# lmb-freiburg/understanding_flow_robustness

Hardware: AMD Instinct MI355X
Metric: attack-iters/s (higher is better)
Workload: dtype f32

## Files before the change

include/ufr_hip.h:

```cpp
#ifndef UFR_HIP_H_
#define UFR_HIP_H_

#include <stdint.h>

#ifdef __cplusplus
extern "C" {
#endif

#define UFR_ABI_VERSION 9

enum { UFR_F32 = 0, UFR_F64 = 1, UFR_F16 = 2 };
enum {
  UFR_OK = 0,
  UFR_EINVAL = -1,
  UFR_EUNSUPPORTED = -2,
  UFR_ELAUNCH = -3
};

typedef void* ufr_stream_t;

int ufr_abi_version(void);
const char* ufr_last_error(void);
int ufr_device_count(void);
const char* ufr_build_manifest(void);
// ... 277 lines not shown
int ufr_resample_u8_vertical(const unsigned char* src, unsigned char* dst, int Hs, int Hd, int W, int C,
                             const int* bounds, const int* kk, int ksize, ufr_stream_t stream);
int ufr_u8_to_tensor(const unsigned char* src, float* dst, int H, int W, int C, int crop_y, int crop_x, int crop_h,
                     int crop_w, float divisor, ufr_stream_t stream);
int ufr_kitti_flow_decode(const unsigned short* src, float* dst, int H, int W, ufr_stream_t stream);

int ufr_host_png_unfilter(const unsigned char* data, unsigned char* out, int rows, int stride, int bpp);

#define UFR_IGEMM_MAX_TAPS 25
typedef struct {
  int ntaps, oy0, ox0;
  long w_off;
  signed char dy[UFR_IGEMM_MAX_TAPS], dx[UFR_IGEMM_MAX_TAPS];
} ufr_igemm_phase;
typedef struct {
  const void* x; long x_plane_stride; int in_chunk0, KC;
  int B, Hi, Wi, in_sy, in_sx;
  const int* in_x0; int in_x0_stride, in_x0_div, in_xw;
  const void* w; long w_plane_stride; int Npad, N;
  int Hr, Wr;
  const int* row_x0; int row_x0_stride, row_x0_div;
  int Ho, Wo, out_sy, out_sx;
  int nphase;
  ufr_igemm_phase phase[4];
  int act; const float* bias; float slope;
  const float* add; int add_chunk0;
  const void* mask; int mask_chunk0;
  void* out_planes; long out_plane_stride; int out_chunk0;
  float* out_f32; int out_f32_chunk0;
  float* tail; int tail_n0, tail_accumulate;
  int splitk; float* ws;
  int products;
  int variant;
  int k_order;
  float* out_rowmajor; long out_ld;
  int planes_chunks, f32_first_chunk;
  int no_reduce;
  int* tickets;
} ufr_igemm_desc;
int ufr_igemm(const ufr_igemm_desc* d, ufr_stream_t stream);
typedef struct {
  int on;
  int row_tiles, col_tiles;
  int full_row_tiles, tail_row_tiles;
  int tail_row0, tail_rows;
  int slices, slice_ktiles, ktiles;
  int workgroups;
  long ws_floats;
  int steps_before, steps_after;
} ufr_igemm_tail_plan_t;
int ufr_igemm_tail_plan(const ufr_igemm_desc* d, int resident_workgroups, ufr_igemm_tail_plan_t* plan);
int ufr_igemm_balanced(const ufr_igemm_desc* d, int resident_workgroups, float* ws, long ws_floats, ufr_stream_t stream);
typedef struct {
  const void* x; long x_plane_stride; int in_chunk0, C;
  const void* gy; long gy_plane_stride; int g_chunk0, N;
  int B, Hi, Wi, Ho, Wo, kh, kw, sy, sx, py, px;
  float* dw;
  float* db;
  int accumulate;
  int splitm; float* ws; long ws_elems;
  int products;
} ufr_igemm_wgrad_desc;
int ufr_igemm_wgrad(const ufr_igemm_wgrad_desc* d, ufr_stream_t stream);
int ufr_igemm_wgrad_dilated(const ufr_igemm_wgrad_desc* d, int dy, int dx, ufr_stream_t stream);
int ufr_igemm_variant_fallbacks(void);
int ufr_igemm_clock_probe(unsigned long long* buf, int capacity_workgroups);
int ufr_rowmajor_to_planes(const float* src, long ld, long rows, int cols, float scale, void* planes, long plane_stride, int chunk0,
                           long plane_rows, ufr_stream_t stream);
int ufr_nchw_to_planes(const float* x, void* planes, long plane_stride, int chunk0, int B, int C, int H, int W,
                       float scale, float slope, const float* bias, ufr_stream_t stream);
int ufr_window_scatter_planes(const float* src, void* planes, long plane_stride, int chunk0, const int* win, int n_win,
                              int N, int C, int Hd, int Wd, int wh, int ww, int level_stride, int margin,
                              ufr_stream_t stream);
int ufr_window_features_planes(const void* c2w, long c2w_stride, const void* c3w, long c3w_stride, void* cat2, long cat2_stride,
                               void* c3a, long c3a_stride, void* c3b, long c3b_stride, float* c3_nchw, float* c3w_nchw,
                               const int* win, int B, int H, int W, int wh, int ww, int m2, int m3, ufr_stream_t stream);
int ufr_chunks_to_nchw(const void* planes, long plane_stride, const float* f32, int chunk0, const void* mask,
                       int mask_chunk0, float* out, int B, int C, int H, int W, float scale, float slope,
                       ufr_stream_t stream);
int ufr_nchw_cat_to_planes(const float* const* srcs, const int* channels, const int* dst_channel0, int nseg, void* planes,
                           long plane_stride, int chunk0, int chunks, int B, int H, int W, ufr_stream_t stream);
int ufr_chunks_to_nchw_cat(const float* g, int chunk0, int chunks, float* const* dsts, const int* channels, const int* src_channel0,
                           int nseg, const float* act0, float pos0, float neg0, int B, int H, int W, ufr_stream_t stream);
int ufr_grad_finalize(const float* g, int g_chunk0, const void* mask, int mask_chunk0, void* out, long out_plane_stride,
                      int out_chunk0, long M, int chunks, float slope, ufr_stream_t stream);

int ufr_conv1_direct(const float* frames_a, const float* frames_b, int Ba, int Bb, int H, int W, const double* mean,
                     const void* wimg, const float* bias, float slope, void* out_planes, long plane_stride, int out_chunk0,
                     ufr_stream_t stream);
int ufr_conv1_pack_planes(const float* frames_a, const float* frames_b, void* planes, long plane_stride, int Ba, int Bb, int H,
                          int W, const double* mean, ufr_stream_t stream);
int ufr_conv1_unpack_grad(const float* G, float* grad_frames, int N, int H, int W, ufr_stream_t stream);
int ufr_unshuffle_pack_planes(const float* x, void* planes, long plane_stride, int N, int C, int H, int W, ufr_stream_t stream);
int ufr_unshuffle_unpack_grad(const float* G, float* grad_x, int N, int C, int H, int W, ufr_stream_t stream);
int ufr_nchw_grad_to_planes(const float* grad, const float* act, void* planes, long plane_stride, int chunk0, int B, int C, int H,
                            int W, float slope, ufr_stream_t stream);
int ufr_window_gather_chunks(const float* src, float* dst, const int* win, int n_win, int N, int N_dst, int chunks, int Hs, int Ws,
                             int wh, int ww, int level_stride, int margin, ufr_stream_t stream);

int ufr_normalize_frames(const float* frames_a, const float* frames_b, float* out, int Ba, int Bb, int C, int H, int W,
                         const double* mean, ufr_stream_t stream);

int ufr_corr_forward_planes_window(const void* f1_planes, const void* f2_planes, long in_plane_stride, void* out_planes,
                                   long out_plane_stride, int out_chunk0, int B, int C, int H, int W, int patch,
                                   int dilation_patch, float scale, float slope, const int* win, int level_stride,
                                   int win_cells, ufr_stream_t stream);

int ufr_corr_forward_planes_changed(const void* f1_planes, const void* f2_planes, long in_plane_stride, void* out_planes,
                                    long out_plane_stride, int out_chunk0, int B, int C, int H, int W, int patch,
                                    int dilation_patch, float scale, float slope, const int* win, int level_stride,
                                    int win_cells_h, int win_cells_w, int margin, ufr_stream_t stream);

int ufr_corr_backward_window_fused(const float* f1, const float* f2, const float* G, int g_chunk0, float g_scale,
                                   const float* G_redir, float* grad_window, int B, int C, int H, int W, int patch,
                                   int dilation_patch, const int* win, int level_stride, int wh, int ww, int margin,
                                   ufr_stream_t stream);

int ufr_corr_forward_planes(const void* f1_planes, const void* f2_planes, long in_plane_stride, void* out_planes,
                            long out_plane_stride, int out_chunk0, int B, int C, int H, int W, int patch,
                            int dilation_patch, float scale, float slope, ufr_stream_t stream);
int ufr_flow_head_planes_forward(const void* planes, long plane_stride, int chunk0, int chunks, const float* wpk, int w_chunks,
                                 const float* bias, float* out, int B, int H, int W, ufr_stream_t stream);
int ufr_flow_head_planes_forward_mfma(const void* planes, long plane_stride, int chunk0, int chunks, const void* wmf, int w_chunks,
                                      const float* bias, float* out, int B, int H, int W, ufr_stream_t stream);
int ufr_flow_head_split_plan(int B, int H, int W, int chunks, int* slices, int* starved, long* partial_floats);
int ufr_flow_head_planes_forward_split(const void* planes, long plane_stride, int chunk0, int chunks, const void* wmf, int w_chunks,
                                       float* partials, long partial_floats, int slices, int B, int H, int W, ufr_stream_t stream);
int ufr_flow_head_split_finish(const float* partials, long partial_floats, int slices, const float* bias, float* flow,
                               const float* up_w, const float* up_bias, void* up_planes, long up_plane_stride, int up_chunk, int B,
                               int H, int W, ufr_stream_t stream);
int ufr_deconv_flow_tail_backward_mfma(const void* grad_planes, long plane_stride, int chunk0, int chunks, const void* wmf,
                                       int w_chunks, float* G, int g_chunks, int out_chunk, int B, int H, int W, ufr_stream_t stream);
int ufr_flow_head_planes_backward(const float* grad_y, const float* wpk, int w_chunks, float* G, int g_chunks, int chunk0, int chunks,
                                  int B, int H, int W, int accumulate, ufr_stream_t stream);
int ufr_flow_head_planes_backward_finalize(const float* grad_y, const float* wpk, int w_chunks, float* G, int g_chunks, int chunk0,
                                           int chunks, int B, int H, int W, int accumulate, const void* mask_planes, void* out_planes,
                                           long out_plane_stride, int fin_chunk0, int fin_chunks, float slope, ufr_stream_t stream);
#define UFR_PF_REGION_BAND 1
#define UFR_PF_REGION_WINDOW 2
int ufr_flow_head_planes_backward_regions(const float* grad_y, const float* wpk, int w_chunks, float* G, int g_chunks, int chunk0,
                                          int chunks, int B, int H, int W, int accumulate, int head_chunks, int region,
                                          const int* origin, int origin_stride, int origin_div, int reg_h, int reg_w, int margin,
// ... 134 lines not shown
```

understanding_flow_robustness_amd/_lib.py:

```python
from __future__ import annotations

import ctypes as C
import os

import torch

_HERE = os.path.dirname(os.path.abspath(__file__))
LIB_PATH = os.environ.get("UFR_HIP_LIB") or os.path.join(_HERE, "lib", "libufr_hip.so")
UFR_F32, UFR_F64, UFR_F16 = 0, 1, 2
ABI_VERSION = 9
_lib = None


class CorrParams(C.Structure):
    _fields_ = [(n, C.c_int) for n in (
        "kH", "kW", "patchH", "patchW", "padH", "padW", "dilationH", "dilationW",
        "dilation_patchH", "dilation_patchW", "dH", "dW")]


UFR_MAX_LEVELS = 8


class Pyramid(C.Structure):
    _fields_ = [("num_levels", C.c_int),
                ("vol", C.c_void_p * UFR_MAX_LEVELS),
                ("grad_vol", C.c_void_p * UFR_MAX_LEVELS),
                ("Hl", C.c_int * UFR_MAX_LEVELS),
                ("Wl", C.c_int * UFR_MAX_LEVELS)]


class AltCorrLevels(C.Structure):
    _fields_ = [("num_levels", C.c_int), ("fmap2", C.c_void_p * 4), ("fmap2_grad", C.c_void_p * 4),
                ("H2", C.c_int * 4), ("W2", C.c_int * 4), ("coord_scale", C.c_float * 4)]


class AltCorrPlaneLevels(C.Structure):
    _fields_ = [("num_levels", C.c_int), ("planes", C.c_void_p * 4), ("plane_stride", C.c_long * 4),
                ("H2", C.c_int * 4), ("W2", C.c_int * 4), ("coord_scale", C.c_float * 4)]


UFR_IGEMM_MAX_TAPS = 25


class IgemmPhase(C.Structure):
    _fields_ = [("ntaps", C.c_int), ("oy0", C.c_int), ("ox0", C.c_int), ("w_off", C.c_long),
                ("dy", C.c_byte * UFR_IGEMM_MAX_TAPS), ("dx", C.c_byte * UFR_IGEMM_MAX_TAPS)]


class IgemmDesc(C.Structure):
    _fields_ = [("x", C.c_void_p), ("x_plane_stride", C.c_long), ("in_chunk0", C.c_int), ("KC", C.c_int),
                ("B", C.c_int), ("Hi", C.c_int), ("Wi", C.c_int), ("in_sy", C.c_int), ("in_sx", C.c_int),
                ("in_x0", C.c_void_p), ("in_x0_stride", C.c_int), ("in_x0_div", C.c_int), ("in_xw", C.c_int),
                ("w", C.c_void_p), ("w_plane_stride", C.c_long), ("Npad", C.c_int), ("N", C.c_int),
                ("Hr", C.c_int), ("Wr", C.c_int),
                ("row_x0", C.c_void_p), ("row_x0_stride", C.c_int), ("row_x0_div", C.c_int),
                ("Ho", C.c_int), ("Wo", C.c_int), ("out_sy", C.c_int), ("out_sx", C.c_int),
                ("nphase", C.c_int),
                ("phase", IgemmPhase * 4),
                ("act", C.c_int), ("bias", C.c_void_p), ("slope", C.c_float),
                ("add", C.c_void_p), ("add_chunk0", C.c_int),
                ("mask", C.c_void_p), ("mask_chunk0", C.c_int),
                ("out_planes", C.c_void_p), ("out_plane_stride", C.c_long), ("out_chunk0", C.c_int),
                ("out_f32", C.c_void_p), ("out_f32_chunk0", C.c_int),
                ("tail", C.c_void_p), ("tail_n0", C.c_int), ("tail_accumulate", C.c_int),
                ("splitk", C.c_int), ("ws", C.c_void_p),
                ("products", C.c_int), ("variant", C.c_int), ("k_order", C.c_int),
                ("out_rowmajor", C.c_void_p), ("out_ld", C.c_long),
                ("planes_chunks", C.c_int), ("f32_first_chunk", C.c_int), ("no_reduce", C.c_int),
                ("tickets", C.c_void_p)]


class IgemmTailPlan(C.Structure):
    _fields_ = [("on", C.c_int), ("row_tiles", C.c_int), ("col_tiles", C.c_int), ("full_row_tiles", C.c_int), ("tail_row_tiles", C.c_int),
                ("tail_row0", C.c_int), ("tail_rows", C.c_int), ("slices", C.c_int), ("slice_ktiles", C.c_int), ("ktiles", C.c_int),
                ("workgroups", C.c_int), ("ws_floats", C.c_long), ("steps_before", C.c_int), ("steps_after", C.c_int)]


UFR_IGEMM_WGRAD_MAX_TAPS = 49


class IgemmWgradDesc(C.Structure):
    _fields_ = [("x", C.c_void_p), ("x_plane_stride", C.c_long), ("in_chunk0", C.c_int), ("C", C.c_int),
                ("gy", C.c_void_p), ("gy_plane_stride", C.c_long), ("g_chunk0", C.c_int), ("N", C.c_int),
                ("B", C.c_int), ("Hi", C.c_int), ("Wi", C.c_int), ("Ho", C.c_int), ("Wo", C.c_int),
                ("kh", C.c_int), ("kw", C.c_int), ("sy", C.c_int), ("sx", C.c_int), ("py", C.c_int), ("px", C.c_int),
                ("dw", C.c_void_p), ("db", C.c_void_p), ("accumulate", C.c_int),
                ("splitm", C.c_int), ("ws", C.c_void_p), ("ws_elems", C.c_long),
                ("products", C.c_int)]


UFR_TRAIN_LOSS_MAX_SCALES = 8


class TrainLossDesc(C.Structure):
    _fields_ = [("gt", C.c_void_p), ("B", C.c_int), ("H", C.c_int), ("W", C.c_int), ("nscale", C.c_int),
                ("pred", C.c_void_p * UFR_TRAIN_LOSS_MAX_SCALES), ("grad", C.c_void_p * UFR_TRAIN_LOSS_MAX_SCALES),
                ("h", C.c_int * UFR_TRAIN_LOSS_MAX_SCALES), ("w", C.c_int * UFR_TRAIN_LOSS_MAX_SCALES),
                ("weight", C.c_double * UFR_TRAIN_LOSS_MAX_SCALES),
                ("kind", C.c_int), ("div_flow", C.c_double),
                ("ws", C.c_void_p), ("ws_elems", C.c_long), ("out", C.c_void_p)]


UFR_RAFT_LOSS_MAX_PREDS = 32


class RaftSequenceLossDesc(C.Structure):
    _fields_ = [("gt", C.c_void_p), ("valid", C.c_void_p), ("B", C.c_int), ("H", C.c_int), ("W", C.c_int), ("npred", C.c_int),
                ("flow", C.c_void_p * UFR_RAFT_LOSS_MAX_PREDS), ("mask", C.c_void_p * UFR_RAFT_LOSS_MAX_PREDS),
                ("grad_flow", C.c_void_p * UFR_RAFT_LOSS_MAX_PREDS), ("grad_mask", C.c_void_p * UFR_RAFT_LOSS_MAX_PREDS),
                ("weight", C.c_double * UFR_RAFT_LOSS_MAX_PREDS),
                ("div_flow", C.c_double), ("max_flow", C.c_double), ("exclude_large", C.c_int),
                ("ws", C.c_void_p), ("ws_elems", C.c_long), ("out", C.c_void_p)]


class AdamwSeg(C.Structure):
    _fields_ = [("p", C.c_void_p), ("g", C.c_void_p), ("m", C.c_void_p), ("v", C.c_void_p), ("n", C.c_long)]


class AdamwHyper(C.Structure):
    _fields_ = [(n, C.c_double) for n in ("lr", "beta1", "beta2", "eps", "weight_decay", "bias1", "bias2")]


class FeatureStatsSeg(C.Structure):
    _fields_ = [("src", C.c_void_p), ("plane_stride", C.c_long), ("pixels", C.c_long), ("kind", C.c_int), ("images", C.c_int),
                ("image0", C.c_int), ("B", C.c_int), ("chunk0", C.c_int), ("channels", C.c_int), ("unleaky", C.c_double),
                ("out_col", C.c_long)]


# ... 29 lines not shown
    "ufr_patch_update": [_vp, _vp, _vp, _vp, _vp, _vp, _vp, _vp, _i, _i, _l, _l, _f, _f, _f, _f, _vp, _vp],
    "ufr_attack_gate": [_vp, _vp, _f, _vp],
    "ufr_gru_gates_forward": [_vp, _vp, _vp, _vp, _i, _i, _i, _l, _vp],
    "ufr_gru_gates_backward": [_vp, _vp, _vp, _vp, _vp, _vp, _i, _i, _i, _l, _vp],
    "ufr_gru_blend_forward": [_vp, _vp, _vp, _vp, _l, _vp],
    "ufr_gru_blend_backward": [_vp, _vp, _vp, _vp, _vp, _vp, _vp, _l, _vp],
    "ufr_flow_loss_ex": [_vp, _vp, _vp, _vp, _i, _i, _i, _i, _f, _vp, _vp, _vp],
    "ufr_universal_update": [_vp, _vp, _vp, _vp, _vp, _vp, _vp, _vp, _i, _i, _f, _f, _f, _f, _i, _i, _i, _i,
                             _i, _vp],
    "ufr_flow_loss": [_vp, _vp, _vp, _vp, _i, _i, _i, _f, _vp, _vp],
    "ufr_flow2_upsampled_loss": [_vp, _f, _vp, _vp, _vp, _i, _i, _i, _i, _f, _vp, _vp],
    "ufr_flow2_upsampled_loss_fast": [_vp, _f, _vp, _vp, _vp, _i, _i, _i, _i, _f, _vp, _vp],
    "ufr_patch_grad_crop": [_vp, _vp, _vp, _vp, _vp, _vp, _vp, _i, _i, _i, _i, _i, _i, _vp],
    "ufr_patch_apply": [_vp, _i, _vp, _vp, _i, _i, _f, _f, _vp, _vp],
    "ufr_patch_grad_crop_window": [_vp, _vp, _vp, _vp, _vp, _vp, _i, _i, _i, _i, _i, _i, _i, _i, _vp],
    "ufr_patch_paste_placed_rect": [_vp, _vp, _vp, _vp, _vp, _vp, _vp, _i, _i, _i, _i, _i, _i, _f, _f, _vp, _vp],
    "ufr_patch_paste_placed": [_vp, _vp, _vp, _vp, _vp, _vp, _vp, _vp, _vp, _i, _i, _i, _i, _i, _i, _f, _f, _vp, _vp],
    "ufr_cone_window": [_vp, _i, _l, _i, _i, _i, C.POINTER(ConeChain), _i, _i, _vp, _vp, _vp],
    "ufr_attack_place": [_vp, _vp, _vp, _vp, _vp, _vp, _vp, _vp, _vp, _vp, _vp, _i, _i, _i, _i, _i, C.POINTER(ConeChain), _i, _i,
                         _vp, _vp, _i, _i, _i, _i, _vp],
    "ufr_attack_load_frames": [_vp, _vp, _vp, _vp, _vp, _vp, _vp, _vp, _vp, _i, _i, _i, _i, _i, _vp],
    "ufr_patch_mask_placed": [_vp, _vp, _vp, _i, _i, _i, _i, _i, _vp],
    "ufr_patch_grad_crop_packed": [_vp, _vp, _vp, _vp, _vp, _vp, _i, _i, _i, _i, _i, _i, _i, _i, _vp],
    "ufr_patch_apply_paste_rect": [_vp, _i, _vp, _vp, _vp, _vp, _vp, _vp, _vp, _vp, _i, _i, _i, _i, _i, _f, _f, _i, _f, _f, _vp, _vp],
    "ufr_window_gather_pair": [_vp, _vp, _vp, _vp, _vp, _i, _i, _i, _i, _i, _i, _vp],
    "ufr_window_features_planes": [_vp, _l, _vp, _l, _vp, _l, _vp, _l, _vp, _l, _vp, _vp, _vp, _i, _i, _i, _i, _i, _i, _i, _vp],
    "ufr_window_gather": [_vp, _vp, _vp, _i, _i, _i, _i, _i, _i, _i, _i, _i, _vp],
    "ufr_window_scatter": [_vp, _vp, _vp, _i, _i, _i, _i, _i, _i, _i, _i, _i, _vp],
    "ufr_conv1_pack_planes": [_vp, _vp, _vp, _l, _i, _i, _i, _i, _vp, _vp],
    "ufr_conv1_unpack_grad": [_vp, _vp, _i, _i, _i, _vp],
    "ufr_nchw_grad_to_planes": [_vp, _vp, _vp, _l, _i, _i, _i, _i, _i, _f, _vp],
    "ufr_window_gather_chunks": [_vp, _vp, _vp, _i, _i, _i, _i, _i, _i, _i, _i, _i, _i, _vp],
    "ufr_normalize_frames": [_vp, _vp, _vp, _i, _i, _i, _i, _i, _vp, _vp],
    "ufr_corr_backward_window_fused": [_vp, _vp, _vp, _i, _f, _vp, _vp, _i, _i, _i, _i, _i, _i, _vp, _i, _i, _i, _i, _vp],
    "ufr_corr_backward_window": [_vp, _vp, _vp, _vp, _vp, _i, _i, _i, _i, _i, _i, _vp, _i, _i, _i, _vp],
    "ufr_bias_leaky_forward": [_vp, _vp, _i, _i, _l, _f, _vp],
    "ufr_leaky_backward": [_vp, _vp, _vp, _l, _f, _vp],
    "ufr_conv3x3_c2_forward": [_vp, _vp, _vp, _vp, _vp, _i, _i, _i, _i, _vp],
    "ufr_conv3x3_c2_backward_data": [_vp, _vp, _vp, _i, _i, _i, _i, _vp],
    "ufr_deconv4x4s2_c2_forward": [_vp, _vp, _vp, _vp, _i, _i, _i, _vp],
    "ufr_deconv4x4s2_c2_backward_data": [_vp, _vp, _vp, _i, _i, _i, _vp],
    "ufr_pwc_warp_forward": [_vp, _vp, _vp, _i, _i, _i, _i, _vp],
    "ufr_pwc_warp_backward": [_vp, _vp, _vp, _vp, _vp, _i, _i, _i, _i, _vp],
    "ufr_pwc_warp_backward_owner": [_vp, _vp, _vp, _vp, _vp, _vp, _l, _i, _i, _i, _i, _vp],
    "ufr_raft_normalize_pair": [_vp, _vp, _vp, _l, _vp],
    "ufr_raft_normalize_pair_backward": [_vp, _vp, _vp, _l, _vp],
    "ufr_raft_fmap_pyramid_forward": [_vp, _vp, _i, _i, _i, _i, _i, _vp],
    "ufr_raft_fmap_pyramid_backward": [_vp, _i, _vp, _i, _i, _i, _i, _vp],
    "ufr_raft_context_split_forward": [_vp, _vp, _vp, _i, _i, _i, _l, _vp],
    "ufr_raft_context_split_backward": [_vp, _vp, _vp, _vp, _vp, _i, _i, _i, _l, _vp],
    "ufr_igemm": [C.POINTER(IgemmDesc), _vp],
    "ufr_igemm_tail_plan": [C.POINTER(IgemmDesc), _i, C.POINTER(IgemmTailPlan)],
    "ufr_igemm_balanced": [C.POINTER(IgemmDesc), _i, _vp, _l, _vp],
    "ufr_igemm_wgrad": [C.POINTER(IgemmWgradDesc), _vp],
    "ufr_igemm_wgrad_dilated": [C.POINTER(IgemmWgradDesc), _i, _i, _vp],
    "ufr_flow_upscale4_forward": [_vp, _vp, _i, _i, _i, _i, _f, _i, _vp],
    "ufr_flow_upscale4_backward": [_vp, _vp, _i, _i, _i, _i, _f, _i, _vp],
    "ufr_fn2_stage_pack": [_vp, _vp, _vp, _vp, _i, _i, _i, _f, _vp],
    "ufr_fn2_stage_unpack_grad": [_vp, _vp, _vp, _vp, _i, _i, _i, _vp],
    "ufr_fn2_stage_finish_grad": [_vp, _vp, _vp, _vp, _vp, _i, _i, _i, _f, _vp],
    "ufr_fn2_fusion_pack": [_vp, _vp, _vp, _vp, _vp, _vp, _i, _i, _i, _vp],
    "ufr_fn2_fusion_unpack_grad": [_vp, _vp, _vp, _vp, _vp, _vp, _vp, _vp, _vp, _i, _i, _i, _vp],
    "ufr_fn2_fusion_finish_grad": [_vp, _vp, _vp, _vp, _vp, _vp, _vp, _i, _i, _i, _vp],
    "ufr_rowmajor_to_planes": [_vp, _l, _l, _i, _f, _vp, _l, _i, _l, _vp],
    "ufr_nchw_to_planes": [_vp, _vp, _l, _i, _i, _i, _i, _i, _f, _f, _vp, _vp],
    "ufr_window_scatter_planes": [_vp, _vp, _l, _i, _vp, _i, _i, _i, _i, _i, _i, _i, _i, _i, _vp],
    "ufr_chunks_to_nchw": [_vp, _l, _vp, _i, _vp, _i, _vp, _i, _i, _i, _i, _f, _f, _vp],
    "ufr_nchw_cat_to_planes": [_vp, _vp, _vp, _i, _vp, _l, _i, _i, _i, _i, _i, _vp],
    "ufr_chunks_to_nchw_cat": [_vp, _i, _i, _vp, _vp, _vp, _i, _vp, _f, _f, _i, _i, _i, _vp],
    "ufr_grad_finalize": [_vp, _i, _vp, _i, _vp, _l, _i, _l, _i, _f, _vp],
    "ufr_flow_head_planes_forward": [_vp, _l, _i, _i, _vp, _i, _vp, _vp, _i, _i, _i, _vp],
    "ufr_flow_head_planes_forward_mfma": [_vp, _l, _i, _i, _vp, _i, _vp, _vp, _i, _i, _i, _vp],
    "ufr_deconv_flow_tail_backward_mfma": [_vp, _l, _i, _i, _vp, _i, _vp, _i, _i, _i, _i, _i, _vp],
    "ufr_flow_head_planes_backward": [_vp, _vp, _i, _vp, _i, _i, _i, _i, _i, _i, _i, _vp],
    "ufr_flow_head_planes_backward_finalize": [_vp, _vp, _i, _vp, _i, _i, _i, _i, _i, _i, _i, _vp, _vp, _l, _i, _i, _f, _vp],
    "ufr_flow_head_planes_backward_regions": [_vp, _vp, _i, _vp, _i, _i, _i, _i, _i, _i, _i, _i, _i, _vp, _i, _i, _i, _i, _i, _vp, _i,
                                              _vp, _vp, _l, _i, _i, _f, _vp],
    "ufr_unshuffle_pack_planes": [_vp, _vp, _l, _i, _i, _i, _i, _vp],
    "ufr_unshuffle_unpack_grad": [_vp, _vp, _i, _i, _i, _i, _vp],
    "ufr_conv3x3s2_c3_planes": [_vp, _vp, _vp, _f, _vp, _l, _i, _i, _i, _i, _i, _vp],
    "ufr_conv3x3_c16_planes": [_vp, _l, _i, _vp, _vp, _f, _vp, _l, _i, _i, _i, _i, _vp],
    "ufr_cm_norm_stats": [_vp, _vp, _vp, _l, _i, _i, _f, _vp],
    "ufr_cm_norm_apply": [_vp, _vp, _vp, _l, _i, _vp, _l, _i, _l, _i, _i, _i, _i, _vp],
    "ufr_cm_norm_stats_apply": [_vp, _vp, _vp, _f, _vp, _l, _i, _vp, _l, _i, _l, _i, _i, _i, _i, _vp],
    "ufr_cm_norm_backward": [_vp, _vp, _vp, _i, _vp, _vp, _vp, _vp, _l, _i, _l, _i, _i, _i, _vp],
    "ufr_cm_masked_copy": [_vp, _vp, _l, _vp, _l, _vp],
    "ufr_raft_flow_patches": [_vp, _vp, _l, _i, _i, _i, _i, _vp],
    "ufr_raft_motion_finish_slabs": [_vp, _i, _i, _i, _vp, _f, _vp, _l, _vp, _l, _i, _vp, _i, _i, _i, _vp],
    "ufr_raft_motion_finish": [_vp, _l, _vp, _l, _i, _vp, _i, _i, _i, _vp],
    "ufr_raft_coords_step": [_vp, _vp, _vp, _vp, _vp, _l, _vp],
    "ufr_grad_finalize_consume": [_vp, _vp, _vp, _l, _l, _i, _f, _vp],
    "ufr_gru_gates_cm_forward": [_vp, _vp, _l, _i, _vp, _l, _i, _l, _i, _vp],
    "ufr_gru_gates_cm_forward_slabs": [_vp, _i, _i, _vp, _vp, _vp, _vp, _l, _i, _vp, _l, _i, _l, _i, _vp],
    "ufr_gru_blend_cm_forward_slabs": [_vp, _i, _i, _vp, _vp, _vp, _vp, _vp, _l, _i, _vp, _l, _i, _l, _i, _vp],
    "ufr_gru_blend_cm_forward": [_vp, _vp, _vp, _l, _i, _vp, _l, _i, _l, _i, _vp],
    "ufr_gru_blend_cm_backward": [_vp, _vp, _vp, _l, _i, _vp, _vp, _l, _i, _vp, _vp, _l, _i, _vp, _vp],
    "ufr_gru_gates_cm_backward": [_vp, _vp, _l, _i, _vp, _vp, _vp, _l, _i, _vp, _l, _i, _i, _vp, _vp],
    "ufr_altcorr_pyramid_forward": [_vp, _vp, _vp, _vp, _i, _i, _i, _i, _i, _f, _vp],
    "ufr_altcorr_pyramid_backward": [_vp, _vp, _vp, _vp, _vp, _vp, _i, _i, _i, _i, _i, _f, _i, _vp],
    "ufr_altcorr_pyramid_backward_cm": [_vp, _vp, _vp, _vp, _vp, _vp, _i, _i, _i, _i, _i, _f, _i, _vp],
    "ufr_upfeat_planes_forward_mfma": [_vp, _l, _i, _i, _vp, _i, _vp, _vp, _i, _i, _i, _vp],
    "ufr_upfeat_planes_backward": [_vp, _vp, _i, _vp, _i, _i, _i, _i, _i, _i, _i, _vp],
    "ufr_flow_up_planes_forward": [_vp, _vp, _vp, _vp, _l, _i, _i, _i, _i, _vp],
    "ufr_flow_head_split_plan": [_i, _i, _i, _i, C.POINTER(C.c_int), C.POINTER(C.c_int), C.POINTER(C.c_long)],
    "ufr_flow_head_planes_forward_split": [_vp, _l, _i, _i, _vp, _i, _vp, _l, _i, _i, _i, _i, _vp],
    "ufr_flow_head_split_finish": [_vp, _l, _i, _vp, _vp, _vp, _vp, _vp, _l, _i, _i, _i, _i, _vp],
    "ufr_flow_up_planes_backward": [_vp, _i, _vp, _vp, _i, _i, _i, _i, _vp],
    "ufr_corr_forward_planes_changed": [_vp, _vp, _l, _vp, _l, _i, _i, _i, _i, _i, _i, _i, _f, _f, _vp, _i, _i, _i, _i, _vp],
    "ufr_corr_forward_planes_window": [_vp, _vp, _l, _vp, _l, _i, _i, _i, _i, _i, _i, _i, _f, _f, _vp, _i, _i, _vp],
    "ufr_corr_forward_planes": [_vp, _vp, _l, _vp, _l, _i, _i, _i, _i, _i, _i, _i, _f, _f, _vp],
    "ufr_convex_upsample_forward": [_vp, _vp, _vp, _i, _i, _i, _vp],
    "ufr_convex_upsample_backward": [_vp, _vp, _vp, _vp, _vp, _vp, _i, _i, _i, _vp],
    "ufr_affine_resample_f64": [_vp, _vp, _i, _i, _i, _i, _i, _d, _d, _d, _d, _d, _d, _i, _vp],
    "ufr_patch_place": [_vp, _vp, _vp, _i, _i, _i, _vp, _vp, _vp, _i, _i, _i, _i, _vp],
    "ufr_patch_crop_f64": [_vp, _vp, _vp, _i, _i, _i, _i, _i, _i, _i, _vp],
    "ufr_resample_u8_horizontal": [_vp, _vp, _i, _i, _i, _i, _i, _vp, _vp, _i, _vp],
    "ufr_resample_u8_vertical": [_vp, _vp, _i, _i, _i, _i, _vp, _vp, _i, _vp],
    "ufr_u8_to_tensor": [_vp, _vp, _i, _i, _i, _i, _i, _i, _i, _f, _vp],
    "ufr_kitti_flow_decode": [_vp, _vp, _i, _i, _vp],
    "ufr_host_png_unfilter": [_vp, _vp, _i, _i, _i],
    "ufr_igemm_clock_probe": [_vp, _i],
    "ufr_altcorr_planes_prepare": [_vp, _vp, _l, _l, _i, _vp],
    "ufr_altcorr_planes_forward": [_vp, _l, C.POINTER(AltCorrPlaneLevels), _vp, _vp, _i, _i, _i, _i, _i, _f, _vp],
    "ufr_conv1_direct": [_vp, _vp, _i, _i, _i, _i, _vp, _vp, _vp, _f, _vp, _l, _i, _vp],
    "ufr_train_loss": [C.POINTER(TrainLossDesc), _vp],
    "ufr_raft_sequence_loss": [C.POINTER(RaftSequenceLossDesc), _vp],
    "ufr_grad_norm": [C.POINTER(AdamwSeg), _i, _f, _vp, _l, _vp, _vp],
    "ufr_adamw_step": [C.POINTER(AdamwSeg), _i, C.POINTER(AdamwHyper), _vp, _vp],
    "ufr_sweep_paste": [_vp, _vp, _vp, _vp, _vp, _vp, _vp, _vp, _i, _i, _i, _i, _i, _f, _f, C.POINTER(ConeChain), _i, _i, _vp, _vp, _vp],
    "ufr_sweep_metrics": [_vp, _vp, _vp, _vp, _vp, _i, _i, _i, _i, _i, _i, _i, _i, _vp, _l, _vp, _i, _i, _vp],
    "ufr_eval_paste": [_vp, _vp, _vp, _vp, _vp, _vp, _vp, _vp, _vp, _vp, _i, _i, _i, _i, _i, _f, _f, _vp],
    "ufr_eval_metrics": [_vp, _vp, _vp, _vp, _vp, _vp, _vp, _vp, _i, _i, _i, _i, _i, _i, _i, _i, _vp, _l, _vp, _i, _i, _vp],
    "ufr_flow_to_image": [_vp, _vp, _vp, _vp, _i, _i, _i, _vp, _l, _vp],
    "ufr_eval_blend_gt": [_vp, _vp, _vp, _vp, _vp, _vp, _vp, _i, _i, _i, _i, _i, _i, _i, _i, _vp],
    "ufr_sweep_blend_gt": [_vp, _vp, _vp, _vp, _vp, _i, _i, _i, _i, _i, _i, _i, _i, _vp],
    "ufr_viz_ranges": [_vp, _vp, _vp, _vp, _vp, _i, _i, _i, _i, _i, _vp, _l, _vp, _vp],
    "ufr_viz_strip": [_vp, _vp, _vp, _vp, _vp, _vp, _vp, _vp, _i, _i, _i, _i, _i, _vp],
    "ufr_global_apply": [_vp, _vp, _vp, _vp, _vp, _vp, _i, _i, _i, _i, _f, _f, _vp],
    "ufr_global_metrics": [_vp, _vp, _vp, _vp, _vp, _i, _i, _i, _i, _i, _i, _i, _i, _vp, _l, _vp, _i, _i, _vp],
    "ufr_validation_pad": [_vp, _vp, _vp, _vp, _i, _i, _i, _i, _i, _i, _i, _i, _vp],
    "ufr_validation_metrics": [_vp, _vp, _vp, _i, _i, _i, _i, _i, _i, _i, _i, _vp, _l, _vp, _i, _i, _vp],
    "ufr_forward_interpolate": [_vp, _vp, _i, _i, _i, _vp],
    "ufr_forward_interpolate_sliced": [_vp, _vp, _i, _i, _i, _i, _vp],
    "ufr_flow_encode": [_vp, _vp, _i, _i, _i, _i, _i, _i, _i, _i, _vp],
    "ufr_feature_stats": [C.POINTER(FeatureStatsSeg), _i, _vp, _l, _vp, _i, _l, _l, _vp],
    "ufr_abs_sums": [_vp, _vp, _l, _vp, _l, _vp, _vp],
    "ufr_momentum_update": [_vp, _vp, _vp, _vp, _vp, _vp, _vp, _vp, _vp, _vp, _i, _i, _f, _f, _f, _f, _f, _f, _i, _i, _vp],
    "ufr_diverse_table_check": [_vp, _i, _i, _i],
    "ufr_diverse_forward": [_vp, _vp, _vp, _vp, _vp, _vp, _i, _i, _i, _i, _vp, _i, _vp, _vp, _vp, _l, _vp],
    "ufr_diverse_backward": [_vp, _vp, _vp, _vp, _i, _i, _i, _vp, _i, _vp, _vp],
    "ufr_step_advance": [_vp, _vp],
}
DIVERSE_COLS = 8
PLAIN = {"ufr_abi_version": (C.c_int, []), "ufr_last_error": (C.c_char_p, []),
         "ufr_device_count": (C.c_int, []), "ufr_build_manifest": (C.c_char_p, []),
         "ufr_igemm_variant_fallbacks": (C.c_int, []),
         "ufr_conv3x3_c2_workspace_floats": (C.c_long, [_i, _i, _i, _i]),
         "ufr_cm_norm_workspace_doubles": (C.c_long, [_l, _i, _i]),
         "ufr_resample2d_backward_workspace_bytes": (C.c_long, [_i, _i, _i]),
         "ufr_pwc_warp_backward_workspace_bytes": (C.c_long, [_i, _i, _i]),
         "ufr_altcorr_pyramid_workspace_bytes": (C.c_long, [_i, _i, _i, _i, _i, _i]),
         "ufr_train_loss_workspace_doubles": (C.c_long, [_i, _i, C.POINTER(C.c_int), C.POINTER(C.c_int)]),
         "ufr_raft_sequence_loss_workspace_doubles": (C.c_long, [_i, _i, _i, _i]),
         "ufr_grad_norm_partials": (C.c_long, [C.POINTER(AdamwSeg), _i]),
         "ufr_sweep_metrics_workspace_doubles": (C.c_long, [_i]),
         "ufr_eval_metrics_workspace_doubles": (C.c_long, [_i]),
         "ufr_flow_to_image_workspace_floats": (C.c_long, [_i]),
         "ufr_viz_workspace_floats": (C.c_long, [_i]),
         "ufr_global_metrics_workspace_doubles": (C.c_long, [_i]),
         "ufr_validation_metrics_workspace_doubles": (C.c_long, [_i, _i, _i]),
         "ufr_feature_stats_workspace_doubles": (C.c_long, [C.POINTER(FeatureStatsSeg), _i]),
         "ufr_abs_sums_workspace_doubles": (C.c_long, [_l]),
         "ufr_diverse_workspace_doubles": (C.c_long, [_i, _i, _i, _i])}


def lib():
    global _lib
    if _lib is None:
        if not os.path.exists(LIB_PATH):
            raise RuntimeError(
                f"{LIB_PATH} not found: build it with `python -c 'import __graft_entry__ as g; "
                "g.build()'` or `make -C understanding_flow_robustness_amd/csrc` (hipcc, gfx950). "
                "There is no CPU fallback.")
        handle = C.CDLL(LIB_PATH)
        for name, args in SIGNATURES.items():
            fn = getattr(handle, name)
            fn.argtypes, fn.restype = args, C.c_int
        for name, (res, args) in PLAIN.items():
            fn = getattr(handle, name)
            fn.argtypes, fn.restype = args, res
        if handle.ufr_abi_version() != ABI_VERSION:
            raise RuntimeError(f"{LIB_PATH} has ABI version {handle.ufr_abi_version()}, these bindings are written for "
                               f"{ABI_VERSION}: rebuild it (`make -C understanding_flow_robustness_amd/csrc`)")
        verify_build(handle.ufr_build_manifest().decode("ascii", "replace"))
        _lib = handle
    return _lib


_CSRC = os.path.join(_HERE, "csrc")
_HEADER = os.path.join(os.path.dirname(_HERE), "include", "ufr_hip.h")


def source_checksums(csrc: str = _CSRC, header: str = _HEADER) -> dict:
    import hashlib
    shared = b""
    for name in sorted(n.encode() for n in os.listdir(csrc) if n.endswith(".h")):
        with open(os.path.join(csrc, name.decode()), "rb") as f:
            shared += f.read()
    with open(header, "rb") as f:
# ... 255 lines not shown
```

understanding_flow_robustness_amd/csrc/conv1_direct.hip:

```cpp
#include <atomic>

#include "ufr_common.h"

namespace {

using ufr::dev::bf16x8;
using ufr::dev::f32x4;
using ufr::dev::split3;
typedef __attribute__((ext_vector_type(4))) __bf16 bf16x4;

constexpr int TY = 8, TX = 32;
constexpr int RY = 2 * TY + 5, RX = 2 * TX + 5;
constexpr int LX = 72;
constexpr int PLANE_B = RY * LX * 8;
constexpr int BUF_B = 3 * PLANE_B;
constexpr int PX_PER_THREAD = (RY * RX + 511) / 512;
__device__ constexpr int PROD_W[6] = {2, 0, 1, 1, 0, 0};
__device__ constexpr int PROD_X[6] = {0, 2, 1, 0, 1, 0};

struct Conv1Args {
  const float* fa; const float* fb; int Ba, N, H, W;
  const double* mean;
  const __bf16* wimg;
  const float* bias; float slope;
  __bf16* out; long plane_stride; int out_chunk0;
  int tiles_x, tiles_y, tiles;
};

template <bool BUF_>
__global__ __launch_bounds__(512) __attribute__((amdgpu_waves_per_eu(2, 2))) void conv1_direct_kernel(const Conv1Args a) {
  extern __shared__ __attribute__((aligned(16))) unsigned char lds[];
  const int tid = threadIdx.x, lane = tid & 63, wave = __builtin_amdgcn_readfirstlane(tid >> 6);
  const int q = wave & 3, half = wave >> 2;
  const int li = lane & 15, g = lane >> 4;
  const int Hh = a.H >> 1, Wh = a.W >> 1;
  const long M = (long)a.N * Hh * Wh;

  for (int i = tid; i < 2 * BUF_B / 16; i += 512) reinterpret_cast<uint4*>(lds)[i] = make_uint4(0, 0, 0, 0);
  bf16x8 wf[7][3];
#pragma unroll
  for (int ky = 0; ky < 7; ++ky)
#pragma unroll
    for (int p = 0; p < 3; ++p)
      wf[ky][p] = *reinterpret_cast<const bf16x8*>(a.wimg + (((long)p * 7 + ky) * 64 + q * 16 + li) * 32 + g * 8);
  float bias4[4];
#pragma unroll
  for (int r = 0; r < 4; ++r) bias4[r] = a.bias[q * 16 + g * 4 + r];
  const double m0 = a.mean[0], m1 = a.mean[1], m2 = a.mean[2];
  __amdgpu_buffer_rsrc_t rsrc = __builtin_amdgcn_make_buffer_rsrc(a.out, 0, BUF_ ? (int)(6L * a.plane_stride) : 0, 0x00020000);

  float pre[PX_PER_THREAD][3];
  unsigned pre_ok = 0;
  auto tile_coords = [&](int t, int& n, int& Y0, int& X0) {
    const int tx = t % a.tiles_x, r = t / a.tiles_x;
    n = r / a.tiles_y;
    Y0 = (r - n * a.tiles_y) * TY;
    X0 = tx * TX;
  };
  auto fetch = [&](int t) {
    int n, Y0, X0;
    tile_coords(t, n, Y0, X0);
    const float* img = n < a.Ba ? a.fa + (long)n * 3 * a.H * a.W : a.fb + (long)(n - a.Ba) * 3 * a.H * a.W;
    const long HW = (long)a.H * a.W;
    pre_ok = 0;
#pragma unroll
    for (int i = 0; i < PX_PER_THREAD; ++i) {
      const int idx = tid + 512 * i, ry = idx / RX, rx = idx - ry * RX;
      const int iy = 2 * Y0 - 3 + ry, ix = 2 * X0 - 3 + rx;
      const bool ok = idx < RY * RX && (unsigned)iy < (unsigned)a.H && (unsigned)ix < (unsigned)a.W;
      const long o = (long)iy * a.W + ix;
      pre[i][0] = ok ? img[o] : 0.f;
      pre[i][1] = ok ? img[o + HW] : 0.f;
      pre[i][2] = ok ? img[o + 2 * HW] : 0.f;
      pre_ok |= ok ? 1u << i : 0u;
    }
  };
  auto stage = [&](int buf) {
    unsigned char* base = lds + buf * BUF_B;
#pragma unroll
    for (int i = 0; i < PX_PER_THREAD; ++i) {
      const int idx = tid + 512 * i;
      if (idx >= RY * RX) continue;
      const int ry = idx / RX, rx = idx - ry * RX;
      const bool ok = (pre_ok >> i) & 1u;
      const float v0 = ok ? (float)((double)pre[i][0] - m0) : 0.f;
      const float v1 = ok ? (float)((double)pre[i][1] - m1) : 0.f;
      const float v2 = ok ? (float)((double)pre[i][2] - m2) : 0.f;
      bf16x4 p0, p1, p2;
      __bf16 x, y, z;
// ... 12 lines not shown
  if (t >= a.tiles) return;
  fetch(t);
  __syncthreads();
  stage(0);
  int tn = t + gridDim.x;
  if (tn < a.tiles) fetch(tn);
  __syncthreads();

  for (int it = 0; t < a.tiles; ++it, t = tn, tn += gridDim.x) {
    const int buf = it & 1;
    int n, Y0, X0;
    tile_coords(t, n, Y0, X0);
    const unsigned char* src = lds + buf * BUF_B;
    const unsigned char* base = src + ((2 * half * 4) * LX + 2 * (li + g)) * 8;
    bf16x8 xf[3][3];
    auto read_step = [&](int s, bf16x8 (&dst)[3]) {
      const int pt = s / 7, ky = s - 7 * pt;
      const unsigned char* px = base + ((2 * (pt >> 1) + ky) * LX + 2 * ((pt & 1) * 16)) * 8;
#pragma unroll
      for (int p = 0; p < 3; ++p) dst[p] = *reinterpret_cast<const bf16x8*>(px + p * PLANE_B);
    };
    read_step(0, xf[0]);
    read_step(1, xf[1]);
    float vkeep[4] = {0.f, 0.f, 0.f, 0.f};
    auto epilogue = [&](int pt, const f32x4 (&acc)[4]) {
      float v[4];
#pragma unroll
      for (int r = 0; r < 4; ++r) {
        v[r] = (acc[0][r] + acc[1][r]) + (acc[2][r] + acc[3][r]) + bias4[r];
        v[r] = v[r] > 0.f ? v[r] : v[r] * a.slope;
      }
      if (!(pt & 1)) {
#pragma unroll
        for (int r = 0; r < 4; ++r) vkeep[r] = v[r];
        return;
      }
      const bool even = !(g & 1);
      float out8[8];
#pragma unroll
      for (int r = 0; r < 4; ++r) {
        const float got = __shfl_xor(even ? v[r] : vkeep[r], 16);
        out8[r] = even ? vkeep[r] : got;
        out8[4 + r] = even ? got : v[r];
      }
      bf16x8 o0, o1, o2;
#pragma unroll
      for (int r = 0; r < 8; ++r) {
        __bf16 b0, b1, b2;
        split3(out8[r], b0, b1, b2);
        o0[r] = b0; o1[r] = b1; o2[r] = b2;
      }
      const int yy = half * 4 + (pt >> 1);
      const int y = Y0 + yy, x = X0 + (even ? 0 : 16) + li;
      const long m = ((long)n * Hh + y) * Wh + x;
      const long e = ((long)(a.out_chunk0 + (q >> 1)) * M + m) * 32 + (q & 1) * 16 + (g & 2) * 4;
      const bool live = y < Hh && x < Wh;
      if constexpr (BUF_) {
        const unsigned off = live ? (unsigned)(e * 2) : 0x80000000u;
        typedef __attribute__((ext_vector_type(4))) unsigned u32x4;
        __builtin_amdgcn_raw_buffer_store_b128(__builtin_bit_cast(u32x4, o0), rsrc, off, 0, 0);
        __builtin_amdgcn_raw_buffer_store_b128(__builtin_bit_cast(u32x4, o1), rsrc, off, (unsigned)(a.plane_stride * 2), 0);
        __builtin_amdgcn_raw_buffer_store_b128(__builtin_bit_cast(u32x4, o2), rsrc, off, (unsigned)(a.plane_stride * 4), 0);
      } else if (live) {
        __bf16* o = a.out + e;
        *reinterpret_cast<bf16x8*>(o) = o0;
        *reinterpret_cast<bf16x8*>(o + a.plane_stride) = o1;
        *reinterpret_cast<bf16x8*>(o + 2 * a.plane_stride) = o2;
      }
    };
    f32x4 acc_prev[4];
#pragma unroll
    for (int pt = 0; pt < 8; ++pt) {
      f32x4 acc[4];
#pragma unroll
      for (int c = 0; c < 4; ++c) acc[c] = f32x4{0.f, 0.f, 0.f, 0.f};
      if (pt > 0) epilogue(pt - 1, acc_prev);
#pragma unroll
      for (int ky = 0; ky < 7; ++ky) {
        const int s = pt * 7 + ky;
        if (s + 2 < 56) read_step(s + 2, xf[(s + 2) % 3]);
#pragma unroll
        for (int tp = 0; tp < 6; ++tp) {
          const int c = (ky * 6 + tp) & 3;
          acc[c] = __builtin_amdgcn_mfma_f32_16x16x32_bf16(wf[ky][PROD_W[tp]], xf[s % 3][PROD_X[tp]], acc[c], 0, 0, 0);
        }
      }
#pragma unroll
      for (int i = 0; i < 42; ++i) {
        __builtin_amdgcn_sched_group_barrier(0x008, 1, 0);
        __builtin_amdgcn_sched_group_barrier(0x002, 2, 0);
        if (i & 1) __builtin_amdgcn_sched_group_barrier(0x100, 1, 0);
      }
      __builtin_amdgcn_sched_barrier(0);
#pragma unroll
      for (int c = 0; c < 4; ++c) acc_prev[c] = acc[c];
    }
    epilogue(7, acc_prev);
    if (tn < a.tiles) {
      stage(buf ^ 1);
      if (tn + (int)gridDim.x < a.tiles) fetch(tn + gridDim.x);
    }
    __syncthreads();
  }
}

}

extern "C" int ufr_conv1_direct(const float* frames_a, const float* frames_b, int Ba, int Bb, int H, int W, const double* mean,
                                const void* wimg, const float* bias, float slope, void* out_planes, long plane_stride,
                                int out_chunk0, ufr_stream_t stream) {
  UFR_REQUIRE(frames_a && mean && wimg && bias && out_planes && (frames_b || Bb == 0), "conv1 direct: null pointer");
  UFR_REQUIRE(Ba > 0 && Bb >= 0 && H > 0 && W > 0 && !(H & 1) && !(W & 1) && plane_stride > 0 && out_chunk0 >= 0, "conv1 direct: bad shape");
  Conv1Args a;
  a.fa = frames_a; a.fb = frames_b; a.Ba = Ba; a.N = Ba + Bb; a.H = H; a.W = W; a.mean = mean;
  a.wimg = static_cast<const __bf16*>(wimg); a.bias = bias; a.slope = slope;
  a.out = static_cast<__bf16*>(out_planes); a.plane_stride = plane_stride; a.out_chunk0 = out_chunk0;
  a.tiles_x = ((W >> 1) + TX - 1) / TX; a.tiles_y = ((H >> 1) + TY - 1) / TY;
  const long tiles = (long)a.N * a.tiles_x * a.tiles_y;
  UFR_REQUIRE(tiles < (1L << 30) && (long)a.N * (H >> 1) * (W >> 1) < (1L << 30), "conv1 direct: too many pixels");
  a.tiles = (int)tiles;
  int dev = 0;
  if (hipGetDevice(&dev) != hipSuccess || dev < 0 || dev >= 64) return ufr::fail(UFR_ELAUNCH, "conv1 direct: no current device");
  static std::atomic<bool> raised[64] = {};
  if (!raised[dev].load(std::memory_order_acquire)) {
    hipError_t e = ufr::ensure_dynamic_lds(reinterpret_cast<const void*>(conv1_direct_kernel<true>), 2 * BUF_B);
    if (e == hipSuccess) e = ufr::ensure_dynamic_lds(reinterpret_cast<const void*>(conv1_direct_kernel<false>), 2 * BUF_B);
    if (e != hipSuccess) return ufr::fail(UFR_ELAUNCH, "conv1 direct: %s", hipGetErrorString(e));
    raised[dev].store(true, std::memory_order_release);
  }
  const int grid = (int)(tiles < ufr::kNumCU ? tiles : ufr::kNumCU);
  if (6L * plane_stride < 0x7fffffffL) conv1_direct_kernel<true><<<grid, 512, 2 * BUF_B, ufr::as_stream(stream)>>>(a);
  else conv1_direct_kernel<false><<<grid, 512, 2 * BUF_B, ufr::as_stream(stream)>>>(a);
  return ufr::launched("conv1_direct_kernel");
}
```

understanding_flow_robustness_amd/csrc/igemm.hip:

```cpp
#include <atomic>
#include <cstdlib>

#include "ufr_common.h"

namespace {

using ufr::dev::bf16x8;
using ufr::dev::f32x4;
using ufr::dev::glds16;
using ufr::dev::split3;
typedef __attribute__((ext_vector_type(4))) unsigned u32x4;

constexpr int BM = 128, BN = 128, BK = 32;
__device__ constexpr int PROD_A[6] = {2, 0, 1, 1, 0, 0};
__device__ constexpr int PROD_B[6] = {0, 2, 1, 0, 1, 0};

struct RowGeom {
  int B, Hr, Wr, M;
  const int* row_x0;
  int row_x0_stride, row_x0_div;
  int Ho, Wo, out_sy, out_sx;
};

struct Epilogue {
  const float* bias; float slope; int act;
  const float* add; int add_chunk0;
  const __bf16* mask; int mask_chunk0;
  __bf16* out_planes; long out_plane_stride; int out_chunk0;
  float* out_f32; int out_f32_chunk0;
  int planes_chunks, f32_first_chunk;
  float* out_rm; long out_ld;
  float* tail; int tail_n0, tail_acc;
  long Mout; int N, Nchunks32;
  int nostore;
};

__device__ __forceinline__ void epilogue_store(const Epilogue& e, long pout, int n, float v) {
  if (n >= e.Nchunks32 * 32) return;
  if (e.tail && n >= e.tail_n0) {
    float* tp = e.tail + ((long)((n - e.tail_n0) >> 5) * e.Mout + pout) * 32 + (n & 31);
    *tp = (n < e.N ? v : 0.f) + (e.tail_acc ? *tp : 0.f);
    return;
  }
  const long cm = ((long)(n >> 5) * e.Mout + pout) * 32 + (n & 31);
  if (e.act) {
    if (e.add) v += e.add[(long)e.add_chunk0 * e.Mout * 32 + cm];
    v += (n < e.N) ? e.bias[n] : 0.f;
    v = v > 0.f ? v : v * e.slope;
  } else {
    if (e.add) v += e.add[(long)e.add_chunk0 * e.Mout * 32 + cm];
    if (e.mask) v = ((float)e.mask[(long)e.mask_chunk0 * e.Mout * 32 + cm] > 0.f) ? v : v * e.slope;
  }
  if (n >= e.N) v = 0.f;
  if (e.out_rm && n < e.N) e.out_rm[pout * e.out_ld + n] = v;
  if (e.out_f32 && (n >> 5) >= e.f32_first_chunk) e.out_f32[(long)e.out_f32_chunk0 * e.Mout * 32 + cm] = v;
// ... 77 lines not shown
    bf16x8 q0, q1, q2;
#pragma unroll
    for (int j = 0; j < 8; ++j) {
      __bf16 x, y, z;
      split3(v[j], x, y, z);
      q0[j] = x; q1[j] = y; q2[j] = z;
    }
    __bf16* o = e.out_planes + (long)e.out_chunk0 * e.Mout * 32 + cm;
    if (e.nostore) {
      asm volatile("" ::"v"(q0), "v"(q1), "v"(q2), "v"(o));
      return;
    }
    *reinterpret_cast<bf16x8*>(o) = q0;
    *reinterpret_cast<bf16x8*>(o + e.out_plane_stride) = q1;
    *reinterpret_cast<bf16x8*>(o + 2 * e.out_plane_stride) = q2;
  }
}

__device__ __forceinline__ void xcd_tile(int swz, int& bx, int& by, int& bz) {
  bx = blockIdx.x; by = blockIdx.y; bz = blockIdx.z;
  if (!swz) return;
  const int nx = gridDim.x, nxy = nx * gridDim.y, n = nxy * gridDim.z;
  const int orig = (bz * gridDim.y + by) * nx + bx;
  const int q = n / 8, r = n % 8, xcd = orig % 8, idx = orig / 8;
  const int w = (xcd < r ? xcd * (q + 1) : r * (q + 1) + (xcd - r) * q) + idx;
  bz = w % gridDim.z;
  const int rem = w / gridDim.z;
  by = rem / nx;
  bx = rem - by * nx;
}

struct Phase {
  int ntaps, oy0, ox0;
  long w_off;
  int dyx[UFR_IGEMM_MAX_TAPS];
  int run[UFR_IGEMM_MAX_TAPS];
};

struct Args {
  const __bf16* x; long x_plane_stride; int in_chunk0, KC;
  int Hi, Wi, in_sy, in_sx;
  const int* in_x0; int in_x0_stride, in_x0_div, in_xw;
  const __bf16* w; long w_plane_stride; int Npad;
  RowGeom g;
  Epilogue e;
  int nphase, splitk, xcd;
  int korder;
  int per_k, sk[4], zoff[4];
  float* ws;
  int* tickets;
  int skip_out;
  int tl_S, tl_full, tl_nt, tl_rt0, tl_row0, tl_rows, tl_per_k;
  Phase ph[4];
};

__device__ __forceinline__ int xcd_before(int m, int x) { return (m >> 3) * x + min(m & 7, x); }
__device__ __forceinline__ bool tail_tile(const Args& a, int& bx, int& by, int& bz) {
  const int orig = blockIdx.x, x = orig & 7;
  const bool tail = orig >= a.tl_full;
  const int lo = tail ? a.tl_full : 0, hi = tail ? (int)gridDim.x : a.tl_full;
  const int w = xcd_before(hi, x) - xcd_before(lo, x) + (orig >> 3) - ((lo + 7 - x) >> 3);
  if (!tail) {
    bz = 0;
    by = w / a.tl_nt;
    bx = w - by * a.tl_nt;
    return false;
  }
  bz = w % a.tl_S;
  const int rem = w / a.tl_S, rt = rem / a.tl_nt;
  by = a.tl_rt0 + rt;
  bx = rem - rt * a.tl_nt;
  return true;
}

__device__ __forceinline__ void sum_slabs(const float* src, long sstride, int S, float (&v)[8]) {
#pragma unroll
  for (int j = 0; j < 8; ++j) v[j] = 0.f;
  int s = 0;
  for (; s + 8 <= S; s += 8) {
    float4 lo[8], hi[8];
#pragma unroll
    for (int u = 0; u < 8; ++u) {
      lo[u] = *reinterpret_cast<const float4*>(src + (s + u) * sstride);
      hi[u] = *reinterpret_cast<const float4*>(src + (s + u) * sstride + 4);
    }
#pragma unroll
    for (int u = 0; u < 8; ++u) {
      v[0] += lo[u].x; v[1] += lo[u].y; v[2] += lo[u].z; v[3] += lo[u].w; v[4] += hi[u].x; v[5] += hi[u].y; v[6] += hi[u].z; v[7] += hi[u].w;
    }
  }
  if (S - s >= 5) {
    float4 lo[7], hi[7];
#pragma unroll
    for (int u = 0; u < 7; ++u) {
      const int su = min(s + u, S - 1);
      lo[u] = *reinterpret_cast<const float4*>(src + su * sstride);
      hi[u] = *reinterpret_cast<const float4*>(src + su * sstride + 4);
    }
#pragma unroll
    for (int u = 0; u < 7; ++u)
      if (s + u < S) {
        v[0] += lo[u].x; v[1] += lo[u].y; v[2] += lo[u].z; v[3] += lo[u].w; v[4] += hi[u].x; v[5] += hi[u].y; v[6] += hi[u].z; v[7] += hi[u].w;
      }
    s = S;
  }
  for (; s + 4 <= S; s += 4) {
    float4 lo[4], hi[4];
#pragma unroll
    for (int u = 0; u < 4; ++u) {
      lo[u] = *reinterpret_cast<const float4*>(src + (s + u) * sstride);
      hi[u] = *reinterpret_cast<const float4*>(src + (s + u) * sstride + 4);
    }
#pragma unroll
    for (int u = 0; u < 4; ++u) {
      v[0] += lo[u].x; v[1] += lo[u].y; v[2] += lo[u].z; v[3] += lo[u].w; v[4] += hi[u].x; v[5] += hi[u].y; v[6] += hi[u].z; v[7] += hi[u].w;
    }
  }
  for (; s < S; ++s) {
    const float4 lo = *reinterpret_cast<const float4*>(src + s * sstride), hi = *reinterpret_cast<const float4*>(src + s * sstride + 4);
    v[0] += lo.x; v[1] += lo.y; v[2] += lo.z; v[3] += lo.w; v[4] += hi.x; v[5] += hi.y; v[6] += hi.z; v[7] += hi.w;
  }
}

template <int NPL, int MT, int WGR, int BNT>
__device__ __forceinline__ void igemm_write_out(const Args& a, const Phase& ph, f32x4 (&acc)[MT][4], float* lds_f32, int* flag, int z, int phase,
                                                int tile_id, int bm0, int bm, int bn0, int bn, int wrow, int wcol, int lane, int wave,
                                                bool tail_slice = false) {
  if (a.skip_out) {
    float keep = 0.f;
#pragma unroll
    for (int m = 0; m < MT; ++m)
#pragma unroll
      for (int n = 0; n < 4; ++n) keep += acc[m][n][0] + acc[m][n][1] + acc[m][n][2] + acc[m][n][3];
    if (keep == 1.2345678e-30f && a.ws) a.ws[0] = keep;
    return;
  }
  if (a.splitk > 1 || tail_slice) {
    float* slab = a.ws + (tail_slice ? (long)z * a.tl_rows - a.tl_row0 : (long)z * a.g.M) * a.Npad;
#pragma unroll
    for (int m = 0; m < MT; ++m)
#pragma unroll
      for (int j = 0; j < 4; ++j) {
        const int row = bm + wrow + m * 16 + (lane >> 4) * 4 + j;
        if (row < a.g.M) {
#pragma unroll
          for (int n = 0; n < 4; ++n) slab[(long)row * a.Npad + bn + wcol + n * 16 + (lane & 15)] = acc[m][n][j];
        }
      }
    if (!a.tickets) return;
    asm volatile("s_waitcnt vmcnt(0)" ::: "memory");
    __syncthreads();
    if (threadIdx.x == 0) {
      __builtin_amdgcn_fence(__ATOMIC_RELEASE, "agent");
      asm volatile("s_waitcnt vmcnt(0)" ::: "memory");
      const int S = a.sk[phase];
      const int t = __hip_atomic_fetch_add(a.tickets + tile_id, 1, __ATOMIC_RELAXED, __HIP_MEMORY_SCOPE_AGENT);
      const int last = t == S - 1;
      if (last) {
        __hip_atomic_store(a.tickets + tile_id, 0, __ATOMIC_RELAXED, __HIP_MEMORY_SCOPE_AGENT);
        __builtin_amdgcn_fence(__ATOMIC_ACQUIRE, "agent");
        asm volatile("s_waitcnt vmcnt(0)" ::: "memory");
      }
      *flag = last;
    }
    __syncthreads();
    if (!*flag) return;
    const float* base = a.ws + (long)a.zoff[phase] * a.g.M * a.Npad;
    const long sstride = (long)a.g.M * a.Npad;
    const int S = a.sk[phase];
    for (int it = threadIdx.x; it < WGR * (BNT / 8); it += blockDim.x) {
      const int r = it / (BNT / 8), n0 = bn0 + (it - r * (BNT / 8)) * 8, row = bm0 + r;
      if (row >= a.g.M || n0 >= a.e.Nchunks32 * 32) continue;
      float v[8];
      sum_slabs(base + (long)row * a.Npad + n0, sstride, S, v);
      epilogue_store8(a.e, out_pixel(a.g, row, ph.oy0, ph.ox0), n0, v);
    }
    return;
  }
  {
    constexpr int TS = 68;
    float* tw = lds_f32 + wave * (32 * TS);
#pragma unroll
    for (int pass = 0; pass < MT / 2; ++pass) {
      __syncthreads();
#pragma unroll
      for (int mm = 0; mm < 2; ++mm)
#pragma unroll
        for (int n = 0; n < 4; ++n)
#pragma unroll
          for (int j = 0; j < 4; ++j)
            tw[(mm * 16 + (lane >> 4) * 4 + j) * TS + n * 16 + (lane & 15)] = acc[pass * 2 + mm][n][j];
      __syncthreads();
#pragma unroll
      for (int it = 0; it < 4; ++it) {
        const int item = it * 64 + lane, r = item >> 3, g8 = item & 7;
        const int row = bm + wrow + pass * 32 + r;
        if (row < a.g.M) {
          const float4 lo = *reinterpret_cast<const float4*>(tw + r * TS + g8 * 8), hi = *reinterpret_cast<const float4*>(tw + r * TS + g8 * 8 + 4);
          float v[8] = {lo.x, lo.y, lo.z, lo.w, hi.x, hi.y, hi.z, hi.w};
          epilogue_store8(a.e, out_pixel(a.g, row, ph.oy0, ph.ox0), bn + wcol + g8 * 8, v);
        }
      }
    }
  }
}

__device__ __attribute__((aligned(64))) unsigned ufr_zero_page[16];

__device__ unsigned long long* ufr_clock_probe_buf = nullptr;
__device__ int ufr_clock_probe_cap = 0;


struct TileWalk {
  int tx, ty, z, phase, ks, kt0, kt1;
  bool tail_slice;
  __device__ __forceinline__ int tile_id() const { return (phase * gridDim.y + ty) * gridDim.x + tx; }
};
template <bool TAIL_ = false>
__device__ __forceinline__ TileWalk tile_walk(const Args& a) {
  TileWalk t;
  t.tail_slice = false;
  if (TAIL_ && a.tl_S) t.tail_slice = tail_tile(a, t.tx, t.ty, t.z);
  else xcd_tile(a.xcd, t.tx, t.ty, t.z);
  t.phase = 0;
#pragma unroll
  for (int p = 1; p < 4; ++p)
    if (p < a.nphase && t.z >= a.zoff[p]) t.phase = p;
  t.ks = t.z - a.zoff[t.phase];
  const int per_k = t.tail_slice ? a.tl_per_k : a.per_k;
  t.kt0 = t.ks * per_k;
  t.kt1 = min(a.ph[t.phase].ntaps * a.KC, t.kt0 + per_k);
  return t;
}

struct Cell {
  int yb, xb, xlo, xhi;
  long ibase;
};
__device__ __forceinline__ Cell cell_geometry(const Args& a, long cell, int xr_override) {
  const bool live = cell >= 0 && cell < a.g.M;
  const GridCell c = grid_cell(a.g, live ? (int)cell : 0);
  const int xg = (xr_override >= 0 ? xr_override : c.xr) + band_x0(a.g, c.b);
  Cell o;
  o.yb = live ? c.yr * a.in_sy : -(1 << 20);
  o.xb = xg * a.in_sx;
  o.ibase = (long)c.b * a.Hi * a.Wi;
  o.xlo = a.in_x0 ? a.in_x0[c.b * a.in_x0_stride] / a.in_x0_div : 0;
  o.xhi = a.in_x0 ? min(a.Wi, o.xlo + a.in_xw) : a.Wi;
  o.xlo = max(o.xlo, 0);
  return o;
}
__device__ __forceinline__ bool tap_pixel(const Args& a, const Cell& c, int dyo, int dxo, int& pix) {
  const int yi = c.yb + dyo, xi = c.xb + dxo;
  pix = yi * a.Wi + xi;
  return (unsigned)yi < (unsigned)a.Hi && xi >= c.xlo && xi < c.xhi;
}

template <int APT, int NPL, int IMG_ROWS, bool BUF_>
struct ActStager {
  Cell cell[APT];
  bool ok[APT];
  long aoff[APT];
  unsigned voff[APT], rowbase[APT];
  __amdgpu_buffer_rsrc_t rsrc;
  const __bf16 *gx, *xk;
  long xkoff, cstride;
  int tap, kc;

  __device__ __forceinline__ void init(const Args& a, const Phase& ph, int bm, int srow0, int csw, int kt0) {
    cstride = (long)a.g.B * a.Hi * a.Wi * 32;
#pragma unroll
    for (int i = 0; i < APT; ++i) {
      cell[i] = cell_geometry(a, bm + srow0 + 64 * i, -1);
      rowbase[i] = (unsigned)(cell[i].ibase * 64 + csw * 16);
    }
    gx = a.x + (long)a.in_chunk0 * cstride + csw * 8;
    tap = a.korder ? kt0 % ph.ntaps : kt0 / a.KC;
    kc = a.korder ? kt0 / ph.ntaps : kt0 - tap * a.KC;
    xk = gx + (long)kc * cstride;
    rsrc = __builtin_amdgcn_make_buffer_rsrc(const_cast<__bf16*>(a.x), 0, (int)min(6L * a.x_plane_stride, 0x7fffffffL), 0x00020000);
    xkoff = (long)(a.in_chunk0 + kc) * cstride;
  }
  __device__ __forceinline__ void set_tap(const Args& a, const Phase& ph, int t) {
    const int dyx = ph.dyx[t], dyo = (int)(short)(dyx & 0xffff), dxo = dyx >> 16;
#pragma unroll
    for (int i = 0; i < APT; ++i) {
      int pix;
      ok[i] = tap_pixel(a, cell[i], dyo, dxo, pix);
      if (BUF_) voff[i] = ok[i] ? rowbase[i] + (unsigned)pix * 64u : 0x80000000u;
      else aoff[i] = ok[i] ? (cell[i].ibase + (long)pix) * 32 : 0;
    }
  }
  __device__ __forceinline__ void stage(const Args& a, const Phase& ph, __bf16* lds, int wave) {
#pragma unroll
    for (int i = 0; i < APT; ++i)
#pragma unroll
      for (int p = 0; p < NPL; ++p) {
        __bf16* dst = lds + p * (IMG_ROWS * BK) + (64 * i + wave * 16) * BK;
        if constexpr (BUF_) {
          typedef __attribute__((address_space(3))) void* lds_void;
          __builtin_amdgcn_raw_ptr_buffer_load_lds(rsrc, (lds_void)dst, 16, (int)voff[i], (unsigned)((xkoff + p * a.x_plane_stride) * 2), 0, 0);
        } else {
          glds16(ok[i] ? xk + aoff[i] + p * a.x_plane_stride : reinterpret_cast<const __bf16*>(ufr_zero_page), dst);
        }
      }
    if (a.korder) {
      if (++tap == ph.ntaps) {
        tap = 0;
        xk += cstride;
        xkoff += cstride;
      }
      set_tap(a, ph, tap);
    } else {
      xk += cstride;
      xkoff += cstride;
      if (++kc == a.KC) {
        kc = 0;
        xk = gx;
        xkoff = (long)a.in_chunk0 * cstride;
        if (++tap < ph.ntaps) set_tap(a, ph, tap);
      }
    }
  }
};

template <int BN_, int NPL>
__device__ __forceinline__ void stage_weights(const __bf16* wp, long w_plane_stride, __bf16* lds, int wave) {
#pragma unroll
  for (int i = 0; i < BN_ / 64; ++i)
#pragma unroll
    for (int p = 0; p < NPL; ++p)
      glds16(wp + p * w_plane_stride + (long)(64 * i) * BK, lds + p * (BN_ * BK) + (64 * i + wave * 16) * BK);
}

template <int MT>
__device__ __forceinline__ void zero_acc(f32x4 (&acc)[MT][4]) {
#pragma unroll
  for (int m = 0; m < MT; ++m)
#pragma unroll
    for (int n = 0; n < 4; ++n) acc[m][n] = f32x4{0.f, 0.f, 0.f, 0.f};
}
__device__ __forceinline__ int frag_offset(int lane) {
  const int frow = lane & 15;
  return frow * BK + ((((lane >> 4)) ^ ((frow >> 1) & 3)) << 3);
}
template <int NPL, int MT, int FIRST>
__device__ __forceinline__ void mfma_products(const bf16x8 (&fa)[NPL][MT], const bf16x8 (&fb)[4][NPL], f32x4 (&acc)[MT][4]) {
#pragma unroll
  for (int n = 0; n < 4; ++n)
#pragma unroll
    for (int t = FIRST; t < 6; ++t)
#pragma unroll
      for (int m = 0; m < MT; ++m)
        acc[m][n] = __builtin_amdgcn_mfma_f32_16x16x32_bf16(fa[PROD_A[t]][m], fb[n][PROD_B[t]], acc[m][n], 0, 0, 0);
}

template <int BM_, int BN_, bool PIPE_ = false, bool BUF_ = false, int NP_ = 6>
__global__ __launch_bounds__(256) __attribute__((amdgpu_waves_per_eu(PIPE_ ? 2 : (BM_ == 64 ? 4 : 3), PIPE_ ? 2 : (BM_ == 64 ? 4 : 3)))) void igemm_glds_kernel(const Args a) {
  static_assert(!(PIPE_ && BUF_), "the buffer-resource form exists for the single-stage kernel");
  static_assert(NP_ == 6 || NP_ == 3 || NP_ == 1, "six, three or one product");
  constexpr int NPL = NP_ == 6 ? 3 : (NP_ == 3 ? 2 : 1), FIRST = 6 - NP_;
  constexpr int MT = (BN_ == 128 && BM_ == 128) ? 4 : 2;
  constexpr int APT = BM_ / 64;
  constexpr int STAGE = NPL * (BM_ + BN_) * BK;
  constexpr int EPI = 4 * 32 * 68 * 2;
  __shared__ __attribute__((aligned(16))) __bf16 lds_static[PIPE_ ? 8 : (STAGE > EPI ? STAGE : EPI)];
  extern __shared__ __attribute__((aligned(16))) __bf16 lds_dynamic[];
  __bf16* lds_all = PIPE_ ? lds_dynamic : lds_static;
  __bf16 (*ldsA)[BM_ * BK] = reinterpret_cast<__bf16 (*)[BM_ * BK]>(lds_all);
  __bf16 (*ldsB)[BN_ * BK] = reinterpret_cast<__bf16 (*)[BN_ * BK]>(lds_all + NPL * BM_ * BK);
  const int tid = threadIdx.x, lane = tid & 63, wave = __builtin_amdgcn_readfirstlane(tid >> 6);
  const int wrow = BN_ == 128 ? (wave >> 1) * (BM_ / 2) : wave * 32, wcol = BN_ == 128 ? (wave & 1) * 64 : 0;
  const TileWalk wk = tile_walk(a);
  const int bm = wk.ty * BM_, bn = wk.tx * BN_, kt0 = wk.kt0, kt1 = wk.kt1;
  const Phase& ph = a.ph[wk.phase];

  const int srow0 = tid >> 2, sch = tid & 3;
  const int csw = sch ^ ((srow0 >> 1) & 3);
  ActStager<APT, NPL, BM_, BUF_> act;
  act.init(a, ph, bm, srow0, csw, kt0);
  const __bf16* wp = a.w + ph.w_off + ((long)kt0 * a.Npad + bn + srow0) * BK + csw * 8;
  const long wstep = (long)a.Npad * BK;
  auto stage_A = [&](int img) { act.stage(a, ph, (BUF_ ? lds_static : lds_all) + img, wave); };
  auto stage_B = [&]() {
    stage_weights<BN_, NPL>(wp, a.w_plane_stride, &ldsB[0][0], wave);
    wp += wstep;
  };
  auto stage_tile = [&]() {
    stage_A(0);
    stage_B();
  };

  f32x4 acc[MT][4];
  zero_acc(acc);
  const int foff = frag_offset(lane);

  if (kt0 < kt1) act.set_tap(a, ph, act.tap);
  if constexpr (PIPE_) {
    if (kt0 < kt1) {
      stage_A(0);
      stage_B();
    }
    for (int kt = kt0; kt < kt1; ++kt) {
      const int cur = (kt - kt0) & 1;
      asm volatile("s_waitcnt vmcnt(0)" ::: "memory");
      __builtin_amdgcn_s_barrier();
      __builtin_amdgcn_s_setprio(2);
      const __bf16* sA = lds_all + (cur ? STAGE : 0);
      bf16x8 fa[NPL][MT], fb[4][NPL];
#pragma unroll
      for (int p = 0; p < NPL; ++p) {
#pragma unroll
        for (int m = 0; m < MT; ++m) fa[p][m] = *reinterpret_cast<const bf16x8*>(sA + p * (BM_ * BK) + (wrow + m * 16) * BK + foff);
#pragma unroll
        for (int n = 0; n < 4; ++n) fb[n][p] = *reinterpret_cast<const bf16x8*>(&ldsB[p][(wcol + n * 16) * BK + foff]);
      }
      if (kt + 1 < kt1) stage_A(cur ? 0 : STAGE);
      asm volatile("s_waitcnt lgkmcnt(0)" ::: "memory");
      __builtin_amdgcn_s_barrier();
      if (kt + 1 < kt1) stage_B();
      __builtin_amdgcn_s_setprio(0);
      mfma_products<NPL, MT, FIRST>(fa, fb, acc);
    }
  } else
  for (int kt = kt0; kt < kt1; ++kt) {
    __syncthreads();
    stage_tile();
    __syncthreads();
    bf16x8 fa[NPL][MT];
#pragma unroll
    for (int p = 0; p < NPL; ++p)
#pragma unroll
      for (int m = 0; m < MT; ++m)
        fa[p][m] = *reinterpret_cast<const bf16x8*>(&ldsA[p][(wrow + m * 16) * BK + foff]);
#pragma unroll
    for (int n = 0; n < 4; ++n) {
      bf16x8 fb[NPL];
#pragma unroll
      for (int p = 0; p < NPL; ++p) fb[p] = *reinterpret_cast<const bf16x8*>(&ldsB[p][(wcol + n * 16) * BK + foff]);
#pragma unroll
      for (int t = FIRST; t < 6; ++t)
#pragma unroll
        for (int m = 0; m < MT; ++m)
          acc[m][n] = __builtin_amdgcn_mfma_f32_16x16x32_bf16(fa[PROD_A[t]][m], fb[PROD_B[t]], acc[m][n], 0, 0, 0);
    }
  }
  static_assert(PIPE_ ? 4 * 32 * 68 * 4 <= STAGE * 2 : true, "epilogue staging does not fit");
  igemm_write_out<NPL, MT, BM_, BN_>(a, ph, acc, reinterpret_cast<float*>(lds_all), reinterpret_cast<int*>(lds_all), wk.z, wk.phase,
                                     wk.tile_id(), bm, bm, bn, bn, wrow, wcol, lane, wave);
}
constexpr int PIPE_LDS_BYTES = (3 * (128 + 128) * BK + 3 * 128 * BK) * 2;

constexpr int PP_IMG = 3 * 128 * BK;
constexpr int pp_lds_bytes(int bn) { return (4 * PP_IMG + 2 * 3 * bn * BK) * 2; }

template <int BN_, bool BUF_ = false, int NP_ = 6>
__global__ __launch_bounds__(512) __attribute__((amdgpu_waves_per_eu(2, 2))) void igemm_pp_kernel(const Args a) {
  static_assert(NP_ == 6 || NP_ == 3 || NP_ == 1, "six, three or one product");
  constexpr int NPL = NP_ == 6 ? 3 : (NP_ == 3 ? 2 : 1), FIRST = 6 - NP_;
  constexpr int MT = BN_ == 128 ? 4 : 2;
  constexpr int PP_IMG_B = 3 * BN_ * BK;
  extern __shared__ __attribute__((aligned(16))) __bf16 lds_pp[];
  unsigned long long* const probe = ufr_clock_probe_buf;
  const unsigned long long probe_c0 = probe ? __builtin_amdgcn_s_memtime() : 0, probe_r0 = probe ? __builtin_amdgcn_s_memrealtime() : 0;
  const int tid = threadIdx.x & 255, lane = tid & 63;
  const int wave = __builtin_amdgcn_readfirstlane(tid >> 6);
  const int grp = __builtin_amdgcn_readfirstlane(threadIdx.x >> 8);
  const int wrow = BN_ == 128 ? (wave >> 1) * 64 : wave * 32, wcol = BN_ == 128 ? (wave & 1) * 64 : 0;
  const TileWalk wk = tile_walk<true>(a);
  const int bm = wk.ty * 256 + grp * 128, bn = wk.tx * BN_;
  const Phase& ph = a.ph[wk.phase];
  const int nk = max(wk.kt1 - wk.kt0, 0);

  const int srow0 = tid >> 2, sch = tid & 3;
  const int csw = sch ^ ((srow0 >> 1) & 3);
  ActStager<2, NPL, 128, BUF_> act;
  act.init(a, ph, bm, srow0, csw, wk.kt0);
  const __bf16* wp = a.w + ph.w_off + ((long)wk.kt0 * a.Npad + bn + srow0) * BK + csw * 8;
  const long wstep = (long)a.Npad * BK;
  const int imgA0 = grp * 2 * PP_IMG, imgB0 = 4 * PP_IMG;
  auto stage_A = [&](int img) { act.stage(a, ph, lds_pp + img, wave); };
  auto stage_B = [&](int img) {
    stage_weights<BN_, NPL>(wp, a.w_plane_stride, lds_pp + img, wave);
    wp += wstep;
  };

  f32x4 acc[MT][4];
  zero_acc(acc);
  const int foff = frag_offset(lane);

  if (nk > 0) {
    act.set_tap(a, ph, act.tap);
    stage_A(imgA0);
    if (grp == 0) stage_B(imgB0);
  }
  if (grp == 1) {
    asm volatile("s_waitcnt vmcnt(0)" ::: "memory");
    __builtin_amdgcn_s_barrier();
  }
  const unsigned long long probe_c2 = probe ? __builtin_amdgcn_s_memtime() : 0;
  for (int i = 0; i < nk; ++i) {
    const int cur = i & 1;
    asm volatile("s_waitcnt vmcnt(0)" ::: "memory");
    __builtin_amdgcn_s_barrier();
    __builtin_amdgcn_s_setprio(2);
    const __bf16* sA = lds_pp + imgA0 + cur * PP_IMG;
    const __bf16* sB = lds_pp + imgB0 + cur * PP_IMG_B;
    bf16x8 fa[NPL][MT], fb[4][NPL];
#pragma unroll
    for (int p = 0; p < NPL; ++p) {
#pragma unroll
      for (int m = 0; m < MT; ++m) fa[p][m] = *reinterpret_cast<const bf16x8*>(sA + p * (128 * BK) + (wrow + m * 16) * BK + foff);
#pragma unroll
      for (int n = 0; n < 4; ++n) fb[n][p] = *reinterpret_cast<const bf16x8*>(sB + p * (BN_ * BK) + (wcol + n * 16) * BK + foff);
    }
    if (i + 1 < nk) {
      stage_A(imgA0 + (cur ^ 1) * PP_IMG);
      if (grp == 0) stage_B(imgB0 + (cur ^ 1) * PP_IMG_B);
    }
    asm volatile("s_waitcnt lgkmcnt(0)" ::: "memory");
    __builtin_amdgcn_s_setprio(0);
    __builtin_amdgcn_s_barrier();
    mfma_products<NPL, MT, FIRST>(fa, fb, acc);
  }
  if (grp == 0) __builtin_amdgcn_s_barrier();
  const unsigned long long probe_c3 = probe ? __builtin_amdgcn_s_memtime() : 0;
  static_assert(4 * 32 * 68 * 4 <= 2 * PP_IMG * 2, "epilogue staging does not fit a group's activation images");
  igemm_write_out<NPL, MT, 256, BN_>(a, ph, acc, reinterpret_cast<float*>(lds_pp + imgA0), reinterpret_cast<int*>(lds_pp), wk.z, wk.phase,
                                     wk.tile_id(), wk.ty * 256, bm, bn, bn, wrow, wcol, lane, wave, wk.tail_slice);
  if (probe && threadIdx.x == 0) {
    const int wg = (blockIdx.z * gridDim.y + blockIdx.y) * gridDim.x + blockIdx.x;
    if (wg < ufr_clock_probe_cap) {
      unsigned long long* o = probe + 8L * wg;
      o[0] = probe_c0; o[1] = __builtin_amdgcn_s_memtime(); o[2] = probe_r0; o[3] = __builtin_amdgcn_s_memrealtime();
      o[4] = probe_c2; o[5] = probe_c3; o[6] = __builtin_amdgcn_s_getreg((4 << 0) | (0 << 6) | (31 << 11)); o[7] = (unsigned long long)nk;
    }
  }
}

constexpr int PP3_ROWS = 144;
constexpr int PP3_IMG = 3 * PP3_ROWS * BK;
constexpr int pp3_lds_bytes(int bn) { return (4 * PP3_IMG + 2 * 3 * bn * BK) * 2; }

template <int BN_>
__global__ __launch_bounds__(512) __attribute__((amdgpu_waves_per_eu(2, 2))) void igemm_pp3_kernel(const Args a) {
  constexpr int NPL = 3, MT = BN_ == 128 ? 4 : 2, PP_IMG_B = 3 * BN_ * BK;
  extern __shared__ __attribute__((aligned(16))) __bf16 lds_pp[];
  const int tid = threadIdx.x & 255, lane = tid & 63, wave = __builtin_amdgcn_readfirstlane(tid >> 6);
  const int grp = __builtin_amdgcn_readfirstlane(threadIdx.x >> 8);
  const int wrow = BN_ == 128 ? (wave >> 1) * 64 : wave * 32, wcol = BN_ == 128 ? (wave & 1) * 64 : 0;
  const TileWalk wk = tile_walk(a);
  const int bm = wk.ty * 256 + grp * 128, bn = wk.tx * BN_;
  const Phase& ph = a.ph[wk.phase];
  const int ntaps = ph.ntaps, kt0 = wk.kt0;
  const int nk = max(wk.kt1 - kt0, 0);
  const long cstride = (long)a.g.B * a.Hi * a.Wi * 32;
  const int Wr = a.g.Wr;

  const int srow0 = tid >> 2, sch = tid & 3;
  const int csw = sch ^ ((srow0 >> 1) & 3);
  const int xrow = lane >> 2, cswx = sch ^ ((xrow >> 1) & 3);
  Cell cg[3];
  cg[0] = cell_geometry(a, (long)bm + srow0, -1);
  cg[1] = cell_geometry(a, (long)bm + srow0 + 64, -1);
  const int grow0 = bm / Wr;
  if (xrow < 2) {
    cg[2] = cell_geometry(a, (long)bm + 128 + xrow, -1);
  } else {
    const int e = (xrow - 2) >> 1, w = (xrow - 2) & 1;
    const long rowcell = (long)(grow0 + e) * Wr;
    cg[2] = cell_geometry(a, rowcell < a.g.M ? rowcell : -1, Wr + w);
  }
  const __bf16* gx = a.x + (long)a.in_chunk0 * cstride + csw * 8;
  const __bf16* gxx = a.x + (long)a.in_chunk0 * cstride + cswx * 8;
  const __bf16* zero = reinterpret_cast<const __bf16*>(ufr_zero_page);
  const __bf16* wp = a.w + ph.w_off + ((long)kt0 * a.Npad + bn + srow0) * BK + csw * 8;
  const long wstep = (long)a.Npad * BK;

  const int imgA0 = grp * 2 * PP3_IMG, imgB0 = 4 * PP3_IMG;
  auto stage_A = [&](int img, int kc, int tap) {
    const int dyx = ph.dyx[tap], dyo = (int)(short)(dyx & 0xffff), dxo = (dyx >> 16) - (ph.run[tap] & 3) * a.in_sx;
    const long coff = (long)kc * cstride;
// ... 126 lines not shown
    bf16x8 wr[9][3];
    const __bf16* wl = a.w + ph.w_off + ((long)kc * 9 * a.Npad + nt * 16 + pi) * BK + kgrp * 8;
#pragma unroll
    for (int tt = 0; tt < 9; ++tt)
#pragma unroll
      for (int p = 0; p < 3; ++p) wr[tt][p] = *reinterpret_cast<const bf16x8*>(wl + (long)p * a.w_plane_stride + (long)tt * a.Npad * BK);
    asm volatile("s_waitcnt vmcnt(0)" ::: "memory");
    __syncthreads();
#pragma unroll
    for (int tt = 0; tt < 9; ++tt) {
      const int dyx = ph.dyx[tt], dy = (int)(short)(dyx & 0xffff), dx = dyx >> 16;
#pragma unroll
      for (int m = 0; m < MTW; ++m) {
        const int g = pg * MTW + m;
        const int hp = ((g >> 1) + dy + 1) * HW_ + 16 * (g & 1) + pi + dx + 1;
        const int off = hp * BK + ((kgrp ^ ((hp >> 1) & 3)) << 3);
        bf16x8 fa[3];
#pragma unroll
        for (int p = 0; p < 3; ++p) fa[p] = *reinterpret_cast<const bf16x8*>(sH + p * (HROWS * BK) + off);
#pragma unroll
        for (int q = 0; q < 6; ++q) acc[m] = __builtin_amdgcn_mfma_f32_16x16x32_bf16(fa[PROD_A[q]], wr[tt][PROD_B[q]], acc[m], 0, 0, 0);
      }
    }
  }
  constexpr int TS = 20;
  __syncthreads();
  float* tw = reinterpret_cast<float*>(lds_d33) + wave * (MTW * 16 * TS);
#pragma unroll
  for (int m = 0; m < MTW; ++m)
#pragma unroll
    for (int j = 0; j < 4; ++j) tw[(m * 16 + kgrp * 4 + j) * TS + pi] = acc[m][j];
  __syncthreads();
  const int G8 = NT == 1 ? max(2, a.e.Nchunks32 * 4) : 2;
  for (int it = lane; it < MTW * 16 * G8; it += 64) {
    const int r = it / G8, g8 = it - r * G8, g = pg * MTW + (r >> 4);
    const int y = y0 + (g >> 1), x = x0 + 16 * (g & 1) + (r & 15);
    if (y < H && x < W) {
      float v[8] = {0.f, 0.f, 0.f, 0.f, 0.f, 0.f, 0.f, 0.f};
      if (g8 < 2) {
        const float4 lo = *reinterpret_cast<const float4*>(tw + r * TS + g8 * 8), hi = *reinterpret_cast<const float4*>(tw + r * TS + g8 * 8 + 4);
        v[0] = lo.x; v[1] = lo.y; v[2] = lo.z; v[3] = lo.w; v[4] = hi.x; v[5] = hi.y; v[6] = hi.z; v[7] = hi.w;
      }
      epilogue_store8(a.e, ((long)b * H + y) * W + x, nt * 16 + g8 * 8, v);
    }
  }
}

template <int NT>
constexpr int d33_lds_bytes() {
  constexpr int HROWS = ((6 * 34 + 15) / 16) * 16, stage = 3 * HROWS * BK * 2, epi = 4 * (2 * NT) * 16 * 20 * 4;
  return stage > epi ? stage : epi;
}

__global__ __launch_bounds__(256) void igemm_reduce_kernel(const Args a) {
  const int n8 = a.Npad / 8;
  const int rows = a.tl_S ? a.tl_rows : a.g.M, row0 = a.tl_S ? a.tl_row0 : 0;
  const long total = (long)a.nphase * rows * n8;
  for (long i = (long)blockIdx.x * blockDim.x + threadIdx.x; i < total; i += (long)gridDim.x * blockDim.x) {
    const int n0 = (int)(i % n8) * 8;
    const long rest = i / n8;
    const int r = (int)(rest % rows), row = row0 + r, phase = (int)(rest / rows);
    if (n0 >= a.e.Nchunks32 * 32) continue;
    float v[8];
    sum_slabs(a.ws + ((long)a.zoff[phase] * rows + r) * a.Npad + n0, (long)rows * a.Npad, a.tl_S ? a.tl_S : a.sk[phase], v);
    epilogue_store8(a.e, out_pixel(a.g, row, a.ph[phase].oy0, a.ph[phase].ox0), n0, v);
  }
}

}

extern "C" int ufr_igemm_clock_probe(unsigned long long* buf, int capacity_workgroups) {
  UFR_REQUIRE((buf == nullptr) == (capacity_workgroups == 0) && capacity_workgroups >= 0, "igemm clock probe: buffer and capacity disagree");
  if (hipMemcpyToSymbol(HIP_SYMBOL(ufr_clock_probe_cap), &capacity_workgroups, sizeof(int)) != hipSuccess ||
      hipMemcpyToSymbol(HIP_SYMBOL(ufr_clock_probe_buf), &buf, sizeof(buf)) != hipSuccess)
    return ufr::fail(UFR_ELAUNCH, "igemm clock probe: %s", hipGetErrorString(hipGetLastError()));
  return UFR_OK;
}

namespace {
std::atomic<int> g_variant_fallbacks{0};
}
extern "C" int ufr_igemm_variant_fallbacks(void) { return g_variant_fallbacks.load(); }

namespace {
template <int BM_, int BN_, int NP_>
void launch_glds(const Args& a, dim3 grid, bool use_buf, hipStream_t st) {
  if (use_buf) igemm_glds_kernel<BM_, BN_, false, true, NP_><<<grid, 256, 0, st>>>(a);
  else if constexpr (NP_ == 6) igemm_glds_kernel<BM_, BN_><<<grid, 256, 0, st>>>(a);
}
template <int NP_>
void launch_pp(const Args& a, dim3 grid, bool use_buf, hipStream_t st) {
  if (use_buf) igemm_pp_kernel<128, true, NP_><<<grid, 512, pp_lds_bytes(128), st>>>(a);
  else if constexpr (NP_ == 6) igemm_pp_kernel<128><<<grid, 512, pp_lds_bytes(128), st>>>(a);
}

template <int NP_>
int launch_tiles(const Args& a, const ufr_igemm_desc* d, const ufr_igemm_tail_plan_t* tp, int variant, int nz, bool use_buf, hipStream_t st) {
  const long M = a.g.M;
  const int bn = d->Npad % BN == 0 ? BN : 64;
  const dim3 grid(d->Npad / bn, (unsigned)((M + BM - 1) / BM), nz);
  if constexpr (NP_ != 6) UFR_REQUIRE(use_buf, "igemm: the reduced-product forms need activation planes below 2 GB");
  if (NP_ == 6 && variant == 7 && d->k_order && (d->in_sx == 1 || d->in_sx == 2) && d->Wr >= 22) {
    const dim3 gpp(d->Npad / bn, (unsigned)((M + 255) / 256), nz);
    if (bn == BN) igemm_pp3_kernel<128><<<gpp, 512, pp3_lds_bytes(128), st>>>(a);
    else igemm_pp3_kernel<64><<<gpp, 512, pp3_lds_bytes(64), st>>>(a);
  } else if (variant == 4 && bn == BN) {
    launch_glds<64, 128, NP_>(a, dim3(d->Npad / BN, (unsigned)((M + 63) / 64), nz), use_buf, st);
  } else if ((variant == 6 || variant == 7 || (NP_ != 6 && variant == 5)) && bn == BN) {
    if constexpr (NP_ != 6) {
      const hipError_t e = ufr::ensure_dynamic_lds(reinterpret_cast<const void*>(igemm_pp_kernel<128, true, NP_>), pp_lds_bytes(128));
      if (e != hipSuccess) return ufr::fail(UFR_ELAUNCH, "igemm: %s", hipGetErrorString(e));
    }
    launch_pp<NP_>(a, tp ? dim3(tp->workgroups) : dim3(d->Npad / BN, (unsigned)((M + 255) / 256), nz), use_buf, st);
  } else if (NP_ == 6 && variant == 5 && bn == BN) {
    igemm_glds_kernel<128, 128, true><<<grid, 256, PIPE_LDS_BYTES, st>>>(a);
  } else if (bn == BN) {
    launch_glds<128, 128, NP_>(a, grid, use_buf, st);
  } else {
    launch_glds<128, 64, NP_>(a, grid, use_buf, st);
  }
  return UFR_OK;
}

int igemm_run(const ufr_igemm_desc* d, const ufr_igemm_tail_plan_t* tp, float* tws, ufr_stream_t stream) {
  UFR_REQUIRE(d, "igemm: null descriptor");
  UFR_REQUIRE(d->x && d->w, "igemm: null operand");
  UFR_REQUIRE(d->B > 0 && d->Hi > 0 && d->Wi > 0 && d->Hr > 0 && d->Wr > 0 && d->Ho > 0 && d->Wo > 0, "igemm: bad grid");
  UFR_REQUIRE(d->KC > 0 && d->in_chunk0 >= 0 && d->N > 0 && d->Npad % 64 == 0 && d->Npad >= d->N, "igemm: bad channel counts");
  UFR_REQUIRE(d->in_sy > 0 && d->in_sx > 0 && d->out_sy > 0 && d->out_sx > 0, "igemm: bad strides");
  UFR_REQUIRE(d->nphase >= 1 && d->nphase <= 4 && d->splitk >= 1 && d->splitk <= 64, "igemm: bad phase / split count");
  UFR_REQUIRE(d->products == 6 || d->products == 3 || d->products == 1, "igemm: products must be 6, 3 or 1");
  UFR_REQUIRE(d->splitk == 1 || d->ws, "igemm: split-K needs a workspace");
  UFR_REQUIRE(!d->no_reduce || (d->splitk > 1 && d->nphase == 1), "igemm: no_reduce is for single-phase split-K launches");
  UFR_REQUIRE(d->out_planes || d->out_f32 || d->out_rowmajor, "igemm: no output");
  UFR_REQUIRE(!d->out_rowmajor || (d->out_ld >= d->N && d->N % 8 == 0 && d->out_ld % 4 == 0), "igemm: bad row-major output");
  UFR_REQUIRE(!d->act || d->bias, "igemm: the forward epilogue needs the bias");
  UFR_REQUIRE(d->planes_chunks >= 0 && d->f32_first_chunk >= 0 && ((d->planes_chunks == 0 && d->f32_first_chunk == 0) || (d->out_planes && d->out_f32)),
              "igemm: planes_chunks / f32_first_chunk need both outputs");
  UFR_REQUIRE(!d->tail || (d->tail_n0 > 0 && d->tail_n0 % 32 == 0 && d->tail_n0 < d->N), "igemm: bad tail column");
  UFR_REQUIRE(!d->row_x0 || (d->row_x0_div > 0), "igemm: bad band divisor");
  UFR_REQUIRE(!d->in_x0 || (d->in_x0_div > 0 && d->in_xw > 0), "igemm: bad input band");
  const long M = (long)d->B * d->Hr * d->Wr;
  UFR_REQUIRE(M < (1L << 30) && (long)d->B * d->Hi * d->Wi < (1L << 30) && (long)d->B * d->Ho * d->Wo < (1L << 30),
              "igemm: too many pixels");
  UFR_REQUIRE((d->Hr - 1) * d->out_sy + 1 <= d->Ho && (d->row_x0 || (d->Wr - 1) * d->out_sx + 1 <= d->Wo),
              "igemm: the row grid does not fit the output grid");
  Args a;
  a.x = static_cast<const __bf16*>(d->x); a.x_plane_stride = d->x_plane_stride; a.in_chunk0 = d->in_chunk0; a.KC = d->KC;
  a.Hi = d->Hi; a.Wi = d->Wi; a.in_sy = d->in_sy; a.in_sx = d->in_sx;
  a.in_x0 = d->in_x0; a.in_x0_stride = d->in_x0_stride; a.in_x0_div = d->in_x0_div; a.in_xw = d->in_xw;
  a.w = static_cast<const __bf16*>(d->w); a.w_plane_stride = d->w_plane_stride; a.Npad = d->Npad;
  a.g.B = d->B; a.g.Hr = d->Hr; a.g.Wr = d->Wr; a.g.M = (int)M;
  a.g.row_x0 = d->row_x0; a.g.row_x0_stride = d->row_x0_stride; a.g.row_x0_div = d->row_x0_div;
  a.g.Ho = d->Ho; a.g.Wo = d->Wo; a.g.out_sy = d->out_sy; a.g.out_sx = d->out_sx;
  a.e.bias = d->bias; a.e.slope = d->slope; a.e.act = d->act;
  a.e.add = d->add; a.e.add_chunk0 = d->add_chunk0;
  a.e.mask = static_cast<const __bf16*>(d->mask); a.e.mask_chunk0 = d->mask_chunk0;
  a.e.out_planes = static_cast<__bf16*>(d->out_planes); a.e.out_plane_stride = d->out_plane_stride; a.e.out_chunk0 = d->out_chunk0;
  a.e.out_f32 = d->out_f32; a.e.out_f32_chunk0 = d->out_f32_chunk0;
  a.e.out_rm = d->out_rowmajor; a.e.out_ld = d->out_ld;
  a.e.planes_chunks = d->planes_chunks > 0 ? d->planes_chunks : (1 << 30); a.e.f32_first_chunk = d->f32_first_chunk;
  a.e.tail = d->tail; a.e.tail_n0 = d->tail_n0; a.e.tail_acc = d->tail_accumulate;
  a.e.Mout = (long)d->B * d->Ho * d->Wo; a.e.N = d->N; a.e.Nchunks32 = (d->N + 31) / 32;
  a.nphase = d->nphase; a.splitk = d->splitk; a.ws = d->ws;
  a.tickets = (d->splitk > 1 && !d->no_reduce) ? d->tickets : nullptr;
  static const int skip_out = [] { const char* e = getenv("UFR_IGEMM_DEBUG_SKIP_EPILOGUE"); return e ? atoi(e) : 0; }();
  a.skip_out = skip_out == 1;
  a.e.nostore = skip_out == 2;
  a.tl_S = a.tl_full = a.tl_nt = a.tl_rt0 = a.tl_row0 = a.tl_rows = a.tl_per_k = 0;
  if (tp) {
    a.tl_S = tp->slices; a.tl_full = tp->full_row_tiles * tp->col_tiles; a.tl_nt = tp->col_tiles; a.tl_rt0 = tp->full_row_tiles;
    a.tl_row0 = tp->tail_row0; a.tl_rows = tp->tail_rows; a.tl_per_k = tp->slice_ktiles;
    a.ws = tws;
  }
  a.xcd = 1;
  a.korder = d->k_order ? 1 : 0;
  for (int z = 0; z < 4; ++z) {
    const ufr_igemm_phase& p = d->phase[z < d->nphase ? z : 0];
    UFR_REQUIRE(p.ntaps >= 1 && p.ntaps <= UFR_IGEMM_MAX_TAPS && p.w_off >= 0, "igemm: bad phase %d", z);
    UFR_REQUIRE(p.oy0 >= 0 && p.oy0 < d->out_sy && p.ox0 >= 0 && p.ox0 < d->out_sx, "igemm: bad phase offset");
    UFR_REQUIRE(p.w_off + (long)p.ntaps * d->KC * d->Npad * BK <= d->w_plane_stride, "igemm: phase %d weights out of range", z);
    a.ph[z].ntaps = p.ntaps; a.ph[z].oy0 = p.oy0; a.ph[z].ox0 = p.ox0; a.ph[z].w_off = p.w_off;
    for (int t = 0; t < UFR_IGEMM_MAX_TAPS; ++t)
      a.ph[z].dyx[t] = t < p.ntaps ? (int)(((unsigned)(int)p.dy[t] & 0xffffu) | ((unsigned)(int)p.dx[t] << 16)) : 0;
    for (int t = 0; t < UFR_IGEMM_MAX_TAPS; ++t) a.ph[z].run[t] = 1 << 4;
    for (int t = 0; t < p.ntaps;) {
      int len = 1, dir = 0;
      while (len < 3 && t + len < p.ntaps && p.dy[t + len] == p.dy[t]) {
        const int step = p.dx[t + len] - p.dx[t + len - 1];
        if ((step != d->in_sx && step != -d->in_sx) || (dir && step != dir)) break;
        dir = step;
        ++len;
      }
      int dmin = p.dx[t];
      for (int i = 1; i < len; ++i) dmin = p.dx[t + i] < dmin ? p.dx[t + i] : dmin;
      for (int i = 0; i < len; ++i) a.ph[z].run[t + i] = ((p.dx[t + i] - dmin) / d->in_sx) | (i << 2) | (len << 4);
      t += len;
    }
  }
  int ktmax = 0, nz = 0;
  for (int z = 0; z < d->nphase; ++z) ktmax = a.ph[z].ntaps * d->KC > ktmax ? a.ph[z].ntaps * d->KC : ktmax;
  a.per_k = (ktmax + d->splitk - 1) / d->splitk;
  for (int z = 0; z < 4; ++z) {
    a.zoff[z] = nz;
    a.sk[z] = z < d->nphase ? (a.ph[z].ntaps * d->KC + a.per_k - 1) / a.per_k : 0;
    nz += a.sk[z];
  }
  hipStream_t st = ufr::as_stream(stream);
  const int variant = d->variant ? d->variant : 2;
  UFR_REQUIRE(variant == 2 || variant == 4 || variant == 5 || variant == 6 || variant == 7 || variant == 8, "igemm: unknown kernel variant %d",
              d->variant);
  const bool use_buf = 6L * d->x_plane_stride < 0x7fffffffL;
  int dev = 0;
  if (hipGetDevice(&dev) != hipSuccess || dev < 0 || dev >= 64) return ufr::fail(UFR_ELAUNCH, "igemm: no current device");
  static std::atomic<bool> raised[64] = {};
  if (!raised[dev].load(std::memory_order_acquire)) {
    hipError_t e = ufr::ensure_dynamic_lds(reinterpret_cast<const void*>(igemm_pp_kernel<128>), pp_lds_bytes(128));
    if (e == hipSuccess) e = ufr::ensure_dynamic_lds(reinterpret_cast<const void*>(igemm_pp_kernel<128, true>), pp_lds_bytes(128));
    if (e == hipSuccess) e = ufr::ensure_dynamic_lds(reinterpret_cast<const void*>(igemm_glds_kernel<128, 128, true>), PIPE_LDS_BYTES);
    if (e == hipSuccess) e = ufr::ensure_dynamic_lds(reinterpret_cast<const void*>(igemm_pp3_kernel<128>), pp3_lds_bytes(128));
    if (e == hipSuccess) e = ufr::ensure_dynamic_lds(reinterpret_cast<const void*>(igemm_pp3_kernel<64>), pp3_lds_bytes(64));
    if (e != hipSuccess) return ufr::fail(UFR_ELAUNCH, "igemm: %s", hipGetErrorString(e));
    raised[dev].store(true, std::memory_order_release);
  }
  bool d33 = variant == 8 && d->nphase == 1 && d->phase[0].ntaps == 9 && d->in_sx == 1 && d->in_sy == 1 && d->out_sx == 1 && d->out_sy == 1 &&
             d->Hr == d->Hi && d->Wr == d->Wi && d->Ho == d->Hi && d->Wo == d->Wi && !d->row_x0 && !d->in_x0 && d->splitk == 1 && !d->tail &&
             !d->out_rowmajor && d->k_order && d->N <= 64 && d->products == 6;
  for (int t = 0; d33 && t < 9; ++t)
    d33 = d->phase[0].dy[t] >= -1 && d->phase[0].dy[t] <= 1 && d->phase[0].dx[t] >= -1 && d->phase[0].dx[t] <= 1;
  if ((variant == 8 && !d33) || (variant == 7 && !(d->k_order && (d->in_sx == 1 || d->in_sx == 2) && d->Wr >= 22 && d->products == 6)))
    g_variant_fallbacks.fetch_add(1);
  if (d33) {
    const int nt = d->N <= 16 ? 1 : (d->N <= 32 ? 2 : 4);
    const int tiles = d->B * ((d->Hi + 3) / 4) * ((d->Wi + 31) / 32);
    hipError_t e = hipSuccess;
#define UFR_D33(NT_)                                                                                                  \
    e = ufr::ensure_dynamic_lds(reinterpret_cast<const void*>(igemm_d33_kernel<NT_>), d33_lds_bytes<NT_>());          \
    if (e == hipSuccess) igemm_d33_kernel<NT_><<<tiles, 256, d33_lds_bytes<NT_>(), st>>>(a)
    if (nt == 1) { UFR_D33(1); } else if (nt == 2) { UFR_D33(2); } else { UFR_D33(4); }
#undef UFR_D33
    if (e != hipSuccess) return ufr::fail(UFR_ELAUNCH, "igemm (direct 3 x 3): %s", hipGetErrorString(e));
    return ufr::launched("igemm_d33_kernel");
  }
  int rc = d->products == 6 ? launch_tiles<6>(a, d, tp, variant, nz, use_buf, st)
                            : (d->products == 3 ? launch_tiles<3>(a, d, tp, variant, nz, use_buf, st) : launch_tiles<1>(a, d, tp, variant, nz, use_buf, st));
  if (rc == UFR_OK) rc = ufr::launched("igemm_kernel");
  if (rc != UFR_OK || (!tp && (d->splitk == 1 || d->no_reduce || a.tickets))) return rc;
  const long total = tp ? (long)tp->tail_rows * (d->Npad / 8) : (long)d->nphase * M * (d->Npad / 8);
  igemm_reduce_kernel<<<ufr::stream_grid(total, 256), 256, 0, st>>>(a);
  return ufr::launched("igemm_reduce_kernel");
}
}

extern "C" int ufr_igemm(const ufr_igemm_desc* d, ufr_stream_t stream) { return igemm_run(d, nullptr, nullptr, stream); }

extern "C" int ufr_igemm_tail_plan(const ufr_igemm_desc* d, int resident_workgroups, ufr_igemm_tail_plan_t* plan) {
  UFR_REQUIRE(d && plan, "igemm tail plan: null argument");
  UFR_REQUIRE(resident_workgroups >= 0 && resident_workgroups <= (1 << 20), "igemm tail plan: bad resident workgroup count");
  UFR_REQUIRE(d->B > 0 && d->Hr > 0 && d->Wr > 0 && d->KC > 0 && d->Npad > 0 && d->Npad % 64 == 0 && d->nphase >= 1 && d->nphase <= 4,
              "igemm tail plan: bad descriptor");
  const long M = (long)d->B * d->Hr * d->Wr;
  UFR_REQUIRE(M < (1L << 30), "igemm tail plan: too many pixels");
  UFR_REQUIRE(d->phase[0].ntaps >= 1 && d->phase[0].ntaps <= UFR_IGEMM_MAX_TAPS && (long)d->phase[0].ntaps * d->KC < (1L << 24),
              "igemm tail plan: bad phase");
  *plan = ufr_igemm_tail_plan_t{};
  const int R = resident_workgroups ? resident_workgroups : 256;
  const int Mt = (int)((M + 255) / 256), ktiles = d->phase[0].ntaps * d->KC;
  plan->row_tiles = Mt; plan->ktiles = ktiles;
  plan->full_row_tiles = Mt;
  if (d->Npad % 128 != 0 || d->nphase != 1 || d->variant != 6 || d->products != 6 || d->tickets || d->no_reduce || d->tail || d->splitk > 1)
    return UFR_OK;
  const int Nt = d->Npad / 128;
  plan->col_tiles = Nt;
  const long T = (long)Mt * Nt;
  const long q = T / R;
  plan->steps_before = (int)((T + R - 1) / R) * (ktiles + 6);
  plan->steps_after = plan->steps_before;
  if (q == 0 || T % R == 0) return UFR_OK;
  const int full = (int)(q * R / Nt), tail_rt = Mt - full;
  const long tail_tiles = (long)tail_rt * Nt;
  long S = R / tail_tiles;
  if (S > ktiles / 8) S = ktiles / 8;
  if (S > 8) S = 8;
  if (S < 2) return UFR_OK;
  const int per = (int)((ktiles + S - 1) / S);
  const int after = (int)q * (ktiles + 6) + (per + 6) + 10;
  if (after > plan->steps_before) return UFR_OK;
  plan->on = 1;
  plan->full_row_tiles = full; plan->tail_row_tiles = tail_rt;
  plan->tail_row0 = full * 256; plan->tail_rows = (int)(M - (long)full * 256);
  plan->slices = (int)S; plan->slice_ktiles = per;
  plan->workgroups = (int)((long)full * Nt + tail_tiles * S);
  plan->ws_floats = S * (long)plan->tail_rows * d->Npad;
  plan->steps_after = after;
  return UFR_OK;
}

extern "C" int ufr_igemm_balanced(const ufr_igemm_desc* d, int resident_workgroups, float* ws, long ws_floats, ufr_stream_t stream) {
  UFR_REQUIRE(d, "igemm: null descriptor");
  UFR_REQUIRE(resident_workgroups >= 0, "igemm (balanced): bad resident workgroup count");
  int R = resident_workgroups, dev = 0;
  if (!R && (hipGetDevice(&dev) != hipSuccess || hipDeviceGetAttribute(&R, hipDeviceAttributeMultiprocessorCount, dev) != hipSuccess || R < 1))
    return ufr::fail(UFR_ELAUNCH, "igemm (balanced): no current device");
  ufr_igemm_tail_plan_t plan;
  const int rc = ufr_igemm_tail_plan(d, R, &plan);
  if (rc != UFR_OK) return rc;
  UFR_REQUIRE(!plan.on || (ws && ws_floats >= plan.ws_floats), "igemm (balanced): workspace of %ld floats needed, %ld given", plan.ws_floats,
// ... 4 lines not shown
```

understanding_flow_robustness_amd/flownetc_engine.py:

```python
from __future__ import annotations

import os

import torch
from ._lib import engine_cache as _engine_cache

from . import _lib as L
from . import igemm as ig

_HEADS = ((6, 1024), (5, 1026), (4, 770), (3, 386), (2, 194))


def pf_split_plan(B: int, H: int, W: int, chunks: int):
    import ctypes
    slices, starved, floats = ctypes.c_int(0), ctypes.c_int(0), ctypes.c_long(0)
    L.check(L.lib().ufr_flow_head_split_plan(int(B), int(H), int(W), int(chunks), ctypes.byref(slices), ctypes.byref(starved),
                                             ctypes.byref(floats)), "predict_flow split plan")
    return slices.value, bool(starved.value), floats.value


def _pack_flow_head(weight: torch.Tensor) -> torch.Tensor:
    cin = weight.shape[1]
    chunks = ig.pad32(cin) // 32
    w = torch.zeros(2, chunks * 32, 9, dtype=torch.float32, device=weight.device)
    w[:, :cin] = weight.detach().float().reshape(2, cin, 9)
    return w.view(2, chunks, 32, 9).permute(1, 3, 0, 2).contiguous()


def _pack_flow_head_mfma(weight: torch.Tensor) -> torch.Tensor:
    cin = weight.shape[1]
    chunks = ig.pad32(cin) // 32
    w = torch.zeros(chunks * 32, 32, dtype=torch.float32, device=weight.device)
    w[:cin, :18] = weight.detach().float().reshape(2, cin, 9).permute(1, 2, 0).reshape(cin, 18)
    wn = w.view(chunks, 32, 32).permute(0, 2, 1).contiguous()
    planes = ig._split3(wn).view(3, chunks, 32, 32).permute(1, 0, 2, 3).contiguous()
    return planes


def _pack_flow_tail_mfma(weight2: torch.Tensor) -> torch.Tensor:
    cout = weight2.shape[1]
    chunks = ig.pad32(cout) // 32
    w = torch.zeros(chunks * 32, 32, dtype=torch.float32, device=weight2.device)
    w[:cout] = weight2.detach().float().reshape(2, cout, 16).permute(1, 2, 0).reshape(cout, 32)
    wn = w.view(chunks, 32, 32).permute(0, 2, 1).contiguous()
    return ig._split3(wn).view(3, chunks, 32, 32).permute(1, 0, 2, 3).contiguous()


_TILE = {7: (128, 768)}
_WINDOW_TILE = {**_TILE, 4: (128, 768)}
_PLAN = dict(min_ktiles=16, tile=_TILE)


class FlowNetCHeadEngine:
    def __init__(self, net, B: int, H: int, W: int, device):
        if H % 64 or W % 64:
            raise ValueError("FlowNetC head engine: frame sides must be multiples of 64")
        L.lib()
        self.net, self.B, self.H, self.W, self.dev = net, int(B), int(H), int(W), torch.device(device)
        g = {s: (H // s, W // s) for s in (4, 8, 16, 32, 64)}
        self.grid = g
        P = lambda s, chunks: ig.Planes(B, g[s][0], g[s][1], chunks, self.dev)
        G = lambda s, chunks: ig.GradSum(B, g[s][0], g[s][1], chunks, self.dev)
        self.siamese = hasattr(net, "conv_redir")
        self.c3a_p, self.c3b_p = (P(8, 8), P(8, 8)) if self.siamese else (None, None)
        self.in31, self.cat3, self.cat2 = P(8, 15 if self.siamese else 8), P(8, 13), P(4, 7)
        self.c4a, self.cat4 = P(16, 16), P(16, 25)
        self.c5a, self.cat5 = P(32, 16), P(32, 33)
        self.c6a, self.c6 = P(64, 32), P(64, 32)
        f32 = dict(dtype=torch.float32, device=self.dev)
        self.flow = {k: torch.zeros(B, 2, *g[2 ** k], **f32) for k in (6, 5, 4, 3, 2)}
        self.G_cat2, self.G_cat3, self.G_cat4, self.G_cat5 = G(4, 7), G(8, 13), G(16, 25), G(32, 33)
        self.G_c6, self.G_in31, self.G_c3a = G(64, 32), G(8, 15 if self.siamese else 8), G(8, 8)
        self.gz_cat2, self.gz_cat3, self.gz_cat4, self.gz_cat5 = P(4, 7), P(8, 13), P(16, 25), P(32, 33)
        self.gz_c6, self.gz_c6a, self.gz_c5a, self.gz_c4a = P(64, 32), P(64, 32), P(32, 16), P(16, 16)
        self.gz_in31 = P(8, 15) if self.siamese else None
        self.g_flow = {k: torch.zeros(B, 2, *g[2 ** k], **f32) for k in (6, 5, 4, 3)}
        self.g_corr = torch.zeros(B, 21, 21, *g[8], **f32)
        self.g_c2a = torch.zeros(B, 128, *g[4], **f32)
        self.g_c3a, self.g_c3a_redir, self.g_c3b = (torch.zeros(B, 256, *g[8], **f32) for _ in range(3))
        self.c3_nchw = torch.zeros(2 * B, 256, *g[8], **f32)
        self._prefix = None
        self.flow_out, self.flow_scale = self.flow[2], float(getattr(net, "div_flow", 20.0))
        self._wprefixes, self._wprefix = {}, None
        self._win_m3 = 0
        self._build_launches()

    def _conv(self, name):
        return getattr(self.net, name)[0]

    def _bias(self, conv):
        if conv.bias is None:
            return torch.zeros(conv.out_channels, dtype=torch.float32, device=self.dev)
        return conv.bias.detach().float().contiguous()

    def _stem_layers(self):
        from .plane_graph import stem_stages
        return [(name, block[0], lvl) for lvl, stage in enumerate(stem_stages(self.net), 1) for name, block in stage]

    def _build_launches(self):
        net, g = self.net, self.grid
        queue = ig.LaunchQueue(self.dev, **_PLAN)

        def plan(wi, x, in_chunk0, rows, out_hw, **kw):
            kw.setdefault("variant", self._variant_for(wi))
            return queue.add(wi, x, in_chunk0, rows, out_hw, **kw)

        self._pipe_variant = {"0": 2, "5": 5}.get(os.environ.get("UFR_IGEMM_PIPE", "6"), 6)
# ... 46 lines not shown
        self.ws = queue.build()
        self.fwd = {k: h.launch for k, h in fwd.items()}
        self.plain = {}
        self.bwd = {k: self._with_tail(("full", k), h.launch, h.args, h.kw, h.S) for k, h in bwd.items()}
        self._plans = {("fwd", k): (*h.args, h.S, h.kw) for k, h in fwd.items()}
        self._plans.update({("bwd", k): (*h.args, h.S, h.kw) for k, h in bwd.items()})
        self._band, self.fwd_band, self.bwd_band = None, {}, {}
        self.bwd_band_wide, self.bwd_rest, self._band_plans, self._pf_band, self._split_w = {}, {}, {}, {}, {}
        self.pf_w = {k: _pack_flow_head(getattr(net, f"predict_flow{k}").weight) for k, _ in _HEADS}
        self.pf_wm = {k: _pack_flow_head_mfma(getattr(net, f"predict_flow{k}").weight) for k, _ in _HEADS}
        self.pf_b = {k: getattr(net, f"predict_flow{k}").bias.detach().float().contiguous() for k, _ in _HEADS}
        self.up = {k: getattr(net, f"upsampled_flow{k}_to_{k - 1}") for k in (6, 5, 4, 3)}
        self.up_w = {k: m.weight.detach().float().contiguous() for k, m in self.up.items()}
        self.up_b = {k: (m.bias.detach().float().contiguous() if m.bias is not None else None) for k, m in self.up.items()}
        self.pf_src = {6: (self.c6, 32), 5: (self.cat5, 33), 4: (self.cat4, 25), 3: (self.cat3, 13), 2: (self.cat2, 7)}
        self.pf_G = {6: self.G_c6, 5: self.G_cat5, 4: self.G_cat4, 3: self.G_cat3, 2: self.G_cat2}
        self.up_dst = {6: (self.cat5, 32), 5: (self.cat4, 24), 4: (self.cat3, 12), 3: (self.cat2, 6)}
        self.up_G = {6: (self.G_cat5, 32), 5: (self.G_cat4, 24), 4: (self.G_cat3, 12), 3: (self.G_cat2, 6)}
        self.pf_split, floats = {}, 0
        for k in (6, 5, 4, 3):
            src, chunks = self.pf_src[k]
            slices, starved, n = pf_split_plan(self.B, src.H, src.W, chunks)
            if starved:
                self.pf_split[k] = (slices, n)
                floats = max(floats, n)
        self.pf_partials = torch.empty(max(floats, 1), dtype=torch.float32, device=self.dev)
        self._pf_pending = None
        self.pf_ran = {}

    def _with_tail(self, key, plain, args, kw, S, resident=None):
        self.plain.pop(key, None)
        if S != 1 and resident is None:
            return plain
        wi, x, c0, rows, out_hw = args
        launch = ig.make_launch(wi, x, c0, rows, out_hw, ws=self.ws, balance=True, resident=resident, **kw)
        if launch.tail_plan is None:
            return plain
        self.plain[key] = plain
        return launch

    def tail_launches(self):
        tables = {"full": self.bwd, "band": self.bwd_band, "rest": self.bwd_rest}
        return [(tag, name, tables[tag][name].tail_plan) for tag, name in sorted(self.plain)]

    def _variant_for(self, wi):
        return self._pipe_variant if wi.Npad % 128 == 0 else 2

    def _build_prefix(self):
        B, dev = self.B, self.dev
        H, W = self.H, self.W
        layers = self._stem_layers()
        wis = [None] + [ig.conv_forward_weights(conv.weight, conv.stride[0], conv.padding[0]) for _, conv, _ in layers[1:]]
        scratch = {}

        def level_buffer(lvl, slot, chunks):
            if (lvl, slot) not in scratch:
                scratch[(lvl, slot)] = ig.Planes(B, H >> lvl, W >> lvl, chunks, dev)
            return scratch[(lvl, slot)]
        halves = {}
        for h, taps in (("a", {2: self.cat2, 3: self.c3a_p}), ("b", {3: self.c3b_p})):
            outs = []
            for i, (_, conv, lvl) in enumerate(layers):
                later = sum(1 for _, _, l in layers[i + 1:] if l == lvl)
                outs.append(taps[lvl] if later == 0 and lvl in taps else level_buffer(lvl, later % 2, ig.pad32(conv.out_channels) // 32))
            chain = []
            for i in range(1, len(layers)):
                name, conv, lvl = layers[i]
                launch = ig.make_launch(wis[i], outs[i - 1], 0, (H >> lvl, W >> lvl), (H >> lvl, W >> lvl), out_planes=outs[i],
                                        out_chunk0=0, bias=self._bias(conv), variant=self._variant_for(wis[i]))
                chain.append((name, launch, wis[i]))
            conv1 = layers[0][1]
            P = dict(c1=outs[0], layers=chain, b1=self._bias(conv1), w1=conv1.weight.detach())
            P.update({name: launch for name, launch, _ in chain})
            P.update({name + "_wi": wi for name, _, wi in chain})
            P.update(self._conv1_launch(B, H, W, outs[0]))
            halves[h] = P
        self._prefix = halves

    def _conv1_launch(self, n: int, H: int, W: int, c1: ig.Planes) -> dict:
        conv1 = self._stem_layers()[0][1]
        bias = self._bias(conv1)
        if os.environ.get("UFR_CONV1_DIRECT", "1") != "0":
            return dict(direct=dict(wimg=ig.conv1_direct_weights(conv1.weight), bias=bias, c1=c1, n=n, hw=(H, W),
                                    gflop=2.0 * n * (H // 2) * (W // 2) * 147 * 64 / 1e9))
        packed = ig.Planes(n, H // 2 + 3, W // 2 + 2, 1, self.dev)
        wi = ig.conv1_packed_weights(conv1.weight)
        launch = ig.make_launch(wi, packed, 0, (H // 2, W // 2), (H // 2, W // 2), out_planes=c1, bias=bias, variant=2)
        return dict(packed=packed, conv1=launch, conv1_wi=wi)

    def _conv1(self, P: dict, a: torch.Tensor, b: torch.Tensor | None):
        a = a.contiguous()
        L.require_hip(a, "frames")
        nb = 0 if b is None else int(b.shape[0])
        mean = self.net._mean64.reshape(-1).contiguous()
        D = P.get("direct")
        if D is not None:
            c1 = D["c1"]
            L.check(L.lib().ufr_conv1_direct(L.ptr(a), L.ptr(b.contiguous()) if b is not None else None, int(a.shape[0]), nb,
                                             int(a.shape[2]), int(a.shape[3]), L.ptr(mean), L.ptr(D["wimg"]), L.ptr(D["bias"]),
                                             float(ig.LEAKY), L.ptr(c1.t), c1.plane_stride, 0, L.stream()), "conv1 direct")
            return
        pk = P["packed"]
        L.check(L.lib().ufr_conv1_pack_planes(L.ptr(a), L.ptr(b.contiguous()) if b is not None else None, L.ptr(pk.t),
                                              pk.plane_stride, int(a.shape[0]), nb, int(a.shape[2]), int(a.shape[3]),
                                              L.ptr(mean), L.stream()), "conv1 pack")
        P["conv1"]()

    def prefix_full(self, frames_a: torch.Tensor, frames_b: torch.Tensor):
        if self._prefix is None:
            self._build_prefix()
        B = self.B

        def chain(h, frames, out):
            P = self._prefix[h]
            self._conv1(P, frames, None)
            for _, launch, _ in P["layers"]:
                launch()
            (self.c3a_p if h == "a" else self.c3b_p).to_nchw(256, 0, out=out)
        chain("a", frames_a, self.c3_nchw[:B])
        chain("b", frames_b, self.c3_nchw[B:])
        self._c3a, self._c3b = self.c3_nchw[:B], self.c3_nchw[B:]

    def load_prefix_features(self, c2_all: torch.Tensor, c3_all: torch.Tensor):
        B = self.B
        self.cat2.load_nchw(c2_all[:B].contiguous(), 0)
        self.c3_nchw.copy_(c3_all[:2 * B])
        self._c3a, self._c3b = self.c3_nchw[:B], self.c3_nchw[B:]
        self.c3a_p.load_nchw(self._c3a, 0)
        self.c3b_p.load_nchw(self._c3b, 0)

    def scatter_window_features(self, c2_w: torch.Tensor, c3_w: torch.Tensor, win: torch.Tensor, wh: int, ww: int, m2: int, m3: int):
        lib, B, st = L.lib(), self.B, L.stream()
        h4, w4 = self.grid[4]
        h8, w8 = self.grid[8]
        self._win_m3 = int(m3)
        L.check(lib.ufr_window_scatter_planes(L.ptr(c2_w), L.ptr(self.cat2.t), self.cat2.plane_stride, 0, L.ptr(win), B, B, 128,
                                              h4, w4, wh // 4, ww // 4, 4, m2, st), "window -> planes (conv2)")
        for k, dst in ((0, self.c3a_p), (1, self.c3b_p)):
            L.check(lib.ufr_window_scatter_planes(L.ptr(c3_w[k * B:]), L.ptr(dst.t), dst.plane_stride, 0, L.ptr(win), B, B, 256,
                                                  h8, w8, wh // 8, ww // 8, 8, m3, st), "window -> planes (conv3)")
        L.check(lib.ufr_window_scatter(L.ptr(c3_w), L.ptr(self.c3_nchw), L.ptr(win), B, 2 * B, 256, h8, w8, wh // 8, ww // 8, 8,
                                       m3, st), "window -> nchw (conv3)")

    def _build_window_prefix(self, wh: int, ww: int):
        B2, dev = 2 * self.B, self.dev
        f32 = dict(dtype=torch.float32, device=dev)
        h2, w2, h4, w4, h8, w8 = wh // 2, ww // 2, wh // 4, ww // 4, wh // 8, ww // 8
        layers = self._stem_layers()
        n = len(layers)
        tap2 = max(i for i, (_, _, lvl) in enumerate(layers) if lvl == 2)
        acts = [ig.Planes(B2, wh >> lvl, ww >> lvl, ig.pad32(conv.out_channels) // 32, dev) for _, conv, lvl in layers]
        gz = [ig.Planes(B2, wh >> lvl, ww >> lvl, ig.pad32(conv.out_channels) // 32, dev) for _, conv, lvl in layers]
        G_p = ig.GradSum(B2, h2 + 3, w2 + 2, 1, dev)
# ... 510 lines not shown
        stage("corr", corr, lambda v: self.in31.load_nchw(v, 1, slope=ig.LEAKY))
        stage("conv_redir", self.fwd["conv_redir"], lambda v: self.in31.load_nchw(v, 0))
        stage("conv3_1", self.fwd["conv3_1"], lambda v: self.cat3.load_nchw(v, 0))
        for name in ("conv4", "conv4_1", "conv5", "conv5_1", "conv6", "conv6_1"):
            self.fwd[name]()
        self._pf_forward(6, defer=True)
        for k in (5, 4, 3, 2):
            self._up_forward(k + 1)
            self.fwd[f"deconv{k}"]()
            self._pf_forward(k, defer=True)
        return self.flow[2]


def _unleaky(x: torch.Tensor, slope: float) -> torch.Tensor:
    s = torch.tensor(slope, dtype=torch.float32, device=x.device)
    y0 = x / s
    best, found = y0.clone(), x >= 0
    bits = y0.view(torch.int32)
    for d in (-2, -1, 0, 1, 2):
        cand = (bits + d).view(torch.float32)
        ok = ~found & (cand * s == x)
        best = torch.where(ok, cand, best)
        found = found | ok
    return torch.where(x < 0, best, x)


class _EngineHead(torch.autograd.Function):

    @staticmethod
    def forward(ctx, c2a, c3a, c3b, engine, band):
        ctx.engine, ctx.band = engine, band
        engine.generation = ctx.generation = getattr(engine, "generation", 0) + 1
        ctx.static, ctx.static_grads = L.static_ok(), L.static_grads_ok()
        flow2 = engine.forward(c2a.contiguous(), c3a.contiguous(), c3b.contiguous() if c3b is not None else None, band)
        return flow2.detach() if ctx.static else flow2.clone()

    @staticmethod
    def backward(ctx, g_flow2):
        if ctx.engine.generation != ctx.generation:
            raise RuntimeError("FlowNetC head engine: another forward of this network (same batch and frame size) ran before this "
                               "backward; its activations are gone.  Call backward() before the next forward, or set "
                               "UFR_ENGINE=0 for interleaved forwards")
        g2a, g3a, g3b = ctx.engine.backward(g_flow2.contiguous(), ctx.band, fused_window=False)
        if ctx.static_grads:
            return g2a, g3a, g3b, None, None
        return (g2a.clone() if g2a is not None else None, g3a.clone() if g3a is not None else None,
                g3b.clone() if g3b is not None else None, None, None)


def _weights_stamp(net):
    return tuple((p.data_ptr(), p._version) for p in net.parameters())


def get_engine(net, B: int, H: int, W: int, device) -> FlowNetCHeadEngine:
    key = (int(B), int(H), int(W), str(torch.device(device)))
    cache = _engine_cache(net, "_ufr_head_engines")
    stamp = _weights_stamp(net)
    eng = cache.get(key)
    if eng is None or eng.weights_stamp != stamp:
        eng = cache[key] = FlowNetCHeadEngine(net, B, H, W, device)
        eng.weights_stamp = stamp
    return eng


def engine_head(net, c2a, c3a, c3b, band=None):
    B, _, h4, w4 = c2a.shape
    return _EngineHead.apply(c2a, c3a, c3b, get_engine(net, B, h4 * 4, w4 * 4, c2a.device), band)
```

understanding_flow_robustness_amd/igemm.py:

```python
from __future__ import annotations

import ctypes as C

import os
import threading

import torch

from . import _lib as L

LEAKY = 0.1


def pad32(c: int) -> int:
    return (c + 31) // 32 * 32


def pad128(c: int) -> int:
    return (c + 127) // 128 * 128


def pad_n(c: int) -> int:
    p64, p128 = (c + 63) // 64 * 64, pad128(c)
    return p64 if p64 * 4 <= p128 * 3 else p128


class Planes:

    def __init__(self, B, H, W, chunks, device):
        self.B, self.H, self.W, self.chunks = int(B), int(H), int(W), int(chunks)
        self.M = self.B * self.H * self.W
        self.t = torch.zeros(3, self.chunks, self.M, 32, dtype=torch.bfloat16, device=device)
        self.plane_stride = self.chunks * self.M * 32

    def load_nchw(self, x: torch.Tensor, chunk0: int = 0, scale: float = 1.0, slope: float = 1.0, bias: torch.Tensor | None = None):
        L.require_hip(x, "x")
        B, Cn, H, W = x.shape
        if (B, H, W) != (self.B, self.H, self.W) or chunk0 + pad32(Cn) // 32 > self.chunks or x.dtype != torch.float32:
            raise RuntimeError("Planes.load_nchw: shape mismatch")
        L.check(L.lib().ufr_nchw_to_planes(L.ptr(x), L.ptr(self.t), self.plane_stride, int(chunk0), B, Cn, H, W,
                                           float(scale), float(slope), L.ptr(bias) if bias is not None else None, L.stream()),
                "nchw -> planes")
        return self

    def load_rowmajor(self, src: torch.Tensor, chunk0: int = 0, scale: float = 1.0):
        L.require_hip(src, "src", contiguous=False)
        if src.dim() != 2 or (src.stride(1) != 1 and src.shape[1] != 1) or src.dtype != torch.float32 or src.shape[0] != self.M or chunk0 + pad32(src.shape[1]) // 32 > self.chunks:
            raise RuntimeError("Planes.load_rowmajor: shape mismatch")
        L.check(L.lib().ufr_rowmajor_to_planes(L.ptr(src), src.stride(0), src.shape[0], src.shape[1], float(scale), L.ptr(self.t),
                                               self.plane_stride, int(chunk0), self.M, L.stream()), "row-major -> planes")
        return self

    def to_nchw(self, Cn: int, chunk0: int = 0, out: torch.Tensor | None = None) -> torch.Tensor:
        if out is None:
            out = torch.empty(self.B, Cn, self.H, self.W, dtype=torch.float32, device=self.t.device)
        L.check(L.lib().ufr_chunks_to_nchw(L.ptr(self.t), self.plane_stride, None, int(chunk0), None, 0, L.ptr(out), self.B, Cn,
                                           self.H, self.W, 1.0, 1.0, L.stream()), "planes -> nchw")
        return out


class GradSum:

    def __init__(self, B, H, W, chunks, device):
        self.B, self.H, self.W, self.chunks = int(B), int(H), int(W), int(chunks)
        self.M = self.B * self.H * self.W
        self.t = torch.zeros(self.chunks, self.M, 32, dtype=torch.float32, device=device)

    def to_nchw(self, Cn: int, chunk0: int = 0, mask: Planes | None = None, mask_chunk0: int = 0, scale: float = 1.0,
                slope: float = LEAKY, out: torch.Tensor | None = None) -> torch.Tensor:
        if out is None:
            out = torch.empty(self.B, Cn, self.H, self.W, dtype=torch.float32, device=self.t.device)
        L.check(L.lib().ufr_chunks_to_nchw(None, 0, L.ptr(self.t), int(chunk0), L.ptr(mask.t) if mask is not None else None,
                                           int(mask_chunk0), L.ptr(out), self.B, Cn, self.H, self.W, float(scale), float(slope),
                                           L.stream()), "gradient sum -> nchw")
        return out


class WeightImage:

    def __init__(self, planes, offsets, phases, N, Npad, KC, geometry, C=None):
        self.planes, self.offsets, self.phases = planes, offsets, phases
        self.N, self.Npad, self.KC = N, Npad, KC
        self.C = C if C is not None else KC * 32
        self.geometry = geometry
        self.k_order = K_ORDER

    def flops(self, rows: int) -> float:
        return 2.0 * rows * sum(len(t) for _, _, t in self.phases) * self.C * self.N


def _split3(w: torch.Tensor) -> torch.Tensor:
    w = w.reshape(-1).float()
    p0 = w.to(torch.bfloat16)
    r1 = w - p0.float()
    p1 = r1.to(torch.bfloat16)
    p2 = (r1 - p1.float()).to(torch.bfloat16)
    return torch.stack((p0, p1, p2)).contiguous()


K_ORDER = 1


def _pack(mats, device):
    images, offsets, total = [], [], 0
    N, _, Cn = mats[0].shape
    npad, cpad = pad_n(N), pad32(Cn)
# ... 94 lines not shown
                for c in range(3):
                    for p in range(2):
                        for q in range(2):
                            ky, kx = 2 * a - 1 + p, 4 * b2 - 1 + 2 * j + q
                            if 0 <= ky < 7 and 0 <= kx < 7:
                                mat[j * 12 + (c * 2 + p) * 2 + q, a * 2 + b2, :] = w[:, c, ky, kx]
    taps = [(-a, -2 * b2) for a in range(4) for b2 in range(2)]
    planes, offsets, n, npad, KC, _ = _pack([mat], weight.device)
    return WeightImage(planes, offsets, [(0, 0, taps)], n, npad, KC, dict(in_s=1, out_s=1), C=147.0 * N / (8.0 * 24.0))


def conv_backward_weights(weight: torch.Tensor, stride: int, padding, dilation: int = 1) -> WeightImage:
    N, Cn, kh, kw = weight.shape
    ph, pw = _pair(padding)
    w = weight.detach().float()
    if stride == 1:
        mat = w.permute(1, 2, 3, 0).reshape(Cn, kh * kw, N)
        taps = [(ph - ky * dilation, pw - kx * dilation) for ky in range(kh) for kx in range(kw)]
        planes, offsets, n, npad, KC, cr = _pack([mat], weight.device)
        return WeightImage(planes, offsets, [(0, 0, taps)], n, npad, KC, dict(in_s=1, out_s=1), cr)
    k, padding = kh, ph
    if kh != kw or ph != pw:
        raise NotImplementedError("data gradient of a strided convolution: square kernels only")
    if stride != 2 or dilation != 1:
        raise NotImplementedError("data gradient: stride 1 (any dilation) or 2")
    phases = _deconv_phases(k, padding)
    mats = [torch.stack([w[:, :, ky, kx].t() for ky, kx, _, _ in taps], dim=1) for _, _, taps in phases]
    planes, offsets, n, npad, KC, cr = _pack(mats, weight.device)
    return WeightImage(planes, offsets, [(oy, ox, [(dy, dx) for _, _, dy, dx in taps]) for oy, ox, taps in phases], n, npad, KC,
                       dict(in_s=1, out_s=2), cr)


def deconv_forward_weights(weight: torch.Tensor, padding: int) -> WeightImage:
    cin, cout, k, _ = weight.shape
    w = weight.detach().float()
    phases = _deconv_phases(k, padding)
    mats = [torch.stack([w[:, :, ky, kx].t() for ky, kx, _, _ in taps], dim=1) for _, _, taps in phases]
    planes, offsets, n, npad, KC, cr = _pack(mats, weight.device)
    return WeightImage(planes, offsets, [(oy, ox, [(dy, dx) for _, _, dy, dx in taps]) for oy, ox, taps in phases], n, npad, KC,
                       dict(in_s=1, out_s=2), cr)


def deconv_backward_weights(weight: torch.Tensor, padding: int) -> WeightImage:
    cin, cout, k, _ = weight.shape
    w = weight.detach().float()
    mat = w.permute(0, 2, 3, 1).reshape(cin, k * k, cout)
    taps = [(ky - padding, kx - padding) for ky in range(k) for kx in range(k)]
    planes, offsets, n, npad, KC, cr = _pack([mat], weight.device)
    return WeightImage(planes, offsets, [(0, 0, taps)], n, npad, KC, dict(in_s=2, out_s=1), cr)


class Launch:

    def __init__(self, desc, keep, tail_plan=None, resident=0, tail_ws=None):
        self.desc, self._keep = desc, keep
        self.tail_plan, self._resident, self._tail_ws = tail_plan, int(resident), tail_ws

    def __call__(self):
        if self.tail_plan is not None:
            L.check(L.lib().ufr_igemm_balanced(C.byref(self.desc), self._resident, L.ptr(self._tail_ws), self._tail_ws.numel(), L.stream()),
                    "igemm (balanced)")
            return
        L.check(L.lib().ufr_igemm(C.byref(self.desc), L.stream()), "igemm")

    def algorithmic_bytes(self) -> float:
        d = self.desc
        rows = d.B * d.Hr * d.Wr
        pix_in = min(d.B * d.Hi * d.Wi, rows * d.in_sy * d.in_sx)
        taps = sum(d.phase[z].ntaps for z in range(d.nphase))
        out_el = rows * d.nphase * ((d.tail_n0 if d.tail else d.N) + 31) // 32 * 32
        b = pix_in * d.KC * 32 * 6 + taps * d.KC * d.Npad * 32 * 6
        b += out_el * ((4 if d.add else 0) + (2 if d.mask else 0))
        nch = out_el // (rows * d.nphase * 32)
        pl = min(nch, d.planes_chunks) if d.planes_chunks else nch
        b += rows * d.nphase * 32 * ((6 * pl if d.out_planes else 0) + (4 * (nch - min(nch, d.f32_first_chunk)) if d.out_f32 else 0))
        if d.tail:
            b += rows * (d.N - d.tail_n0) * 4
        return float(b)


_TUNING = None
FUSE_REDUCE = os.environ.get("UFR_IGEMM_FUSE_REDUCE", "0") == "1"
class _ProductsStack(threading.local):
    def __init__(self):
        self.stack = [6]


_PRODUCTS = _ProductsStack()


def current_products() -> int:
    return _PRODUCTS.stack[-1]


class products:
    def __init__(self, n: int):
        if n not in (6, 3, 1):
            raise ValueError("igemm.products: 6, 3 or 1")
        self.n = n

    def __enter__(self):
        _PRODUCTS.stack.append(self.n)

    def __exit__(self, *exc):
        _PRODUCTS.stack.pop()


RECORD = None


def launch_signature(wi: "WeightImage", M: int, kw: dict, rows=None) -> str:
    out = ("slabs" if kw.get("no_reduce") else "rowmajor" if kw.get("out_rowmajor") is not None else
           ("planes" if kw.get("out_planes") is not None else "") + ("f32" if kw.get("out_f32") is not None else ""))
    out += ("+add" if kw.get("add") is not None else "") + ("+mask" if kw.get("mask") is not None else "") + ("+tail" if kw.get("tail") is not None else "")
    taps = "-".join(str(len(t)) for _, _, t in wi.phases)
    grid = f"_g{int(rows[0])}x{int(rows[1])}" if rows is not None else ""
    return f"M{M}_N{wi.Npad}_KC{wi.KC}_t{taps}_s{wi.geometry['in_s']}{wi.geometry['out_s']}_{out}{grid}"


def _tuning_table() -> dict:
    global _TUNING
    if _TUNING is None:
        _TUNING = {}
        path = os.environ.get("UFR_IGEMM_TUNING_FILE") or os.path.join(os.path.dirname(os.path.abspath(__file__)), "igemm_tuning.json")
        if os.environ.get("UFR_IGEMM_TUNING", "1") != "0" and os.path.exists(path):
            import json
            with open(path) as f:
                raw = json.load(f)
            if raw.get("_arch", "gfx950") == "gfx950":
                _TUNING = {k: tuple(v) for k, v in raw.items() if not k.startswith("_")}
    return _TUNING


def variant_fallbacks() -> int:
    return int(L.lib().ufr_igemm_variant_fallbacks())


def tuned(wi: "WeightImage", M: int, kw: dict, variant: int, splitk: int, rows=None):
    table, sig = _tuning_table(), launch_signature(wi, M, kw)
    if rows is not None and launch_signature(wi, M, kw, rows) in table:
        return table[launch_signature(wi, M, kw, rows)]
    if sig in table:
        return table[sig]
    head, _, out = sig.rpartition("_")
    twin = out.replace("+add", "") if "+add" in out else (out.replace("+mask", "+add+mask") if "+mask" in out else
                                                         (out.replace("+tail", "+add+tail") if "+tail" in out else out + "+add"))
    return table.get(f"{head}_{twin}", (variant, splitk))


def make_launch(wi: WeightImage, x: Planes, in_chunk0: int, rows_hw, out_hw, *, out_planes: Planes | None = None,
                out_chunk0: int = 0, out_f32: GradSum | None = None, out_f32_chunk0: int = 0, bias: torch.Tensor | None = None,
                add: GradSum | None = None, add_chunk0: int = 0, mask: Planes | None = None, mask_chunk0: int = 0,
                slope: float = LEAKY, splitk: int = 1, ws: torch.Tensor | None = None, row_band=None, in_band=None,
                products: int | None = None, variant: int = 0, tail: GradSum | None = None, tail_n0: int = 0, tail_chunk0: int = 0,
                tail_accumulate: bool = False, out_rowmajor=None, planes_chunks: int = 0, f32_first_chunk: int = 0,
                no_reduce: bool = False, fuse_reduce: bool | None = None, balance: bool = False, resident: int | None = None) -> Launch:
    if RECORD is not None:
        RECORD.append(dict(wi=wi, x=x, in_chunk0=in_chunk0, rows=tuple(rows_hw), out_hw=tuple(out_hw), splitk=splitk, variant=variant,
                           kw=dict(out_planes=out_planes, out_chunk0=out_chunk0, out_f32=out_f32, out_f32_chunk0=out_f32_chunk0, bias=bias,
                                   add=add, add_chunk0=add_chunk0, mask=mask, mask_chunk0=mask_chunk0, slope=slope, row_band=row_band,
                                   in_band=in_band, tail=tail, tail_n0=tail_n0, tail_chunk0=tail_chunk0, tail_accumulate=tail_accumulate,
                                   out_rowmajor=out_rowmajor, planes_chunks=planes_chunks, f32_first_chunk=f32_first_chunk,
                                   no_reduce=no_reduce)))
    d = L.IgemmDesc()
    d.x, d.x_plane_stride, d.in_chunk0, d.KC = x.t.data_ptr(), x.plane_stride, int(in_chunk0), wi.KC
    if in_chunk0 + wi.KC > x.chunks:
        raise RuntimeError("igemm: the reduced chunks leave the input buffer")
    d.B, d.Hi, d.Wi = x.B, x.H, x.W
    d.in_sy = d.in_sx = int(wi.geometry["in_s"])
    if in_band is not None:
        d.in_x0, d.in_x0_stride, d.in_x0_div, d.in_xw = in_band[0].data_ptr(), int(in_band[1]), int(in_band[2]), int(in_band[3])
    d.w, d.w_plane_stride, d.Npad, d.N = wi.planes.data_ptr(), wi.planes.stride(0), wi.Npad, wi.N
    d.Hr, d.Wr = int(rows_hw[0]), int(rows_hw[1])
    if row_band is not None:
        d.row_x0, d.row_x0_stride, d.row_x0_div = row_band[0].data_ptr(), int(row_band[1]), int(row_band[2])
    d.Ho, d.Wo = int(out_hw[0]), int(out_hw[1])
    d.out_sy = d.out_sx = int(wi.geometry["out_s"])
    d.nphase = len(wi.phases)
    for z, ((oy0, ox0, taps), off) in enumerate(zip(wi.phases, wi.offsets)):
        ph = d.phase[z]
        if len(taps) > L.UFR_IGEMM_MAX_TAPS:
            raise RuntimeError("igemm: too many taps")
        ph.ntaps, ph.oy0, ph.ox0, ph.w_off = len(taps), oy0, ox0, off
        for t, (dy, dx) in enumerate(taps):
            ph.dy[t], ph.dx[t] = dy, dx
    Mout = x.B * d.Ho * d.Wo
    nch = pad32(wi.N) // 32
    if tail is not None:
        if tail_n0 % 32 or not 0 < tail_n0 < wi.N or tail.M != Mout or tail_chunk0 + (wi.N - tail_n0 + 31) // 32 > tail.chunks:
            raise RuntimeError("igemm: tail geometry")
        d.tail, d.tail_n0 = tail.t.data_ptr() + int(tail_chunk0) * tail.M * 32 * 4, int(tail_n0)
        d.tail_accumulate = 1 if tail_accumulate else 0
        nch = tail_n0 // 32
    keep = [wi, x, bias, add, mask, out_planes, out_f32, ws, row_band, in_band, tail]
    if bias is not None:
        d.act, d.bias = 1, bias.data_ptr()
    d.slope = float(slope)
    if add is not None:
        if add.M != Mout or add_chunk0 + nch > add.chunks:
            raise RuntimeError("igemm: addend geometry")
        d.add, d.add_chunk0 = add.t.data_ptr(), int(add_chunk0)
    if mask is not None:
        if mask.M != Mout or mask_chunk0 + nch > mask.chunks:
            raise RuntimeError("igemm: mask geometry")
        d.mask, d.mask_chunk0 = mask.t.data_ptr(), int(mask_chunk0)
    if out_planes is not None:
        if out_planes.M != Mout or out_chunk0 + nch > out_planes.chunks:
            raise RuntimeError("igemm: output plane geometry")
        d.out_planes, d.out_plane_stride, d.out_chunk0 = out_planes.t.data_ptr(), out_planes.plane_stride, int(out_chunk0)
    if out_f32 is not None:
        if out_f32.M != Mout or out_f32_chunk0 + nch > out_f32.chunks:
            raise RuntimeError("igemm: fp32 output geometry")
        d.out_f32, d.out_f32_chunk0 = out_f32.t.data_ptr(), int(out_f32_chunk0)
    if out_rowmajor is not None:
        rm, rm_off, ld = out_rowmajor
        if rm.dtype != torch.float32 or wi.N % 8 or ld < wi.N or ld % 4 or rm_off % 4 or rm.numel() < rm_off + (Mout - 1) * ld + wi.N:
            raise RuntimeError("igemm: row-major output geometry")
        d.out_rowmajor, d.out_ld = rm.data_ptr() + 4 * int(rm_off), int(ld)
        keep.append(rm)
    if planes_chunks or f32_first_chunk:
        if out_planes is None or out_f32 is None:
            raise RuntimeError("igemm: planes_chunks / f32_first_chunk need both outputs")
        d.planes_chunks, d.f32_first_chunk = int(planes_chunks), int(f32_first_chunk)
    d.splitk = int(splitk)
    if splitk > 1:
        need = d.nphase * splitk * x.B * d.Hr * d.Wr * wi.Npad
        if ws is None or ws.numel() < need or ws.dtype != torch.float32:
            raise RuntimeError(f"igemm: split-K workspace of {need} floats needed")
        d.ws = ws.data_ptr()
    d.no_reduce = 1 if (no_reduce and splitk > 1) else 0
    if splitk > 1 and not d.no_reduce and (FUSE_REDUCE if fuse_reduce is None else fuse_reduce):
        tickets = torch.zeros(d.nphase * (-(-(x.B * d.Hr * d.Wr) // 64)) * (wi.Npad // 64), dtype=torch.int32, device=x.t.device)
        d.tickets = tickets.data_ptr()
        keep.append(tickets)
    d.products = int(current_products() if products is None else products)
    d.k_order = int(wi.k_order)
    d.variant = int(variant)
    if balance:
        R = int(resident) if resident else resident_workgroups(x.t.device)
        plan = tail_plan(d, R)
        if plan.on:
            tws = ws if (ws is not None and ws.dtype == torch.float32 and ws.numel() >= plan.ws_floats) else \
                torch.empty(plan.ws_floats, dtype=torch.float32, device=x.t.device)
            return Launch(d, keep + [tws], tail_plan=plan, resident=R, tail_ws=tws)
    return Launch(d, keep)


def resident_workgroups(device) -> int:
    device = torch.device(device)
    return int(torch.cuda.get_device_properties(device).multi_processor_count) if device.type == "cuda" else 256


def tail_plan(desc, resident: int = 0) -> "L.IgemmTailPlan":
    plan = L.IgemmTailPlan()
    L.check(L.lib().ufr_igemm_tail_plan(C.byref(desc), int(resident), C.byref(plan)), "igemm tail plan")
    return plan


def splitk_for(M: int, Npad: int, ktiles: int, phases: int = 1, target: int = 768, phase_ktiles=None, bm: int = 128,
               min_ktiles: int = 16) -> int:
    tiles_mn = -(-M // bm) * (Npad // (128 if Npad % 128 == 0 else 64))
    if phase_ktiles is not None and len(set(phase_ktiles)) > 1:
        best, best_cost = 1, None
        s = 1
        while s <= 16:
            per = -(-max(phase_ktiles) // s)
            if s > 1 and per < min(8, min_ktiles):
                break
            wgs = tiles_mn * sum(-(-k // per) for k in phase_ktiles)
            cost = -(-wgs // target) * (per + 6) + (10 if s > 1 else 0)
            if best_cost is None or cost < best_cost:
                best, best_cost = s, cost
            s *= 2
        return best
    tiles = tiles_mn * phases
    s = 1
    while tiles * s * 2 <= target and ktiles // (s * 2) >= min_ktiles and s < 32:
        s *= 2
    return s


_TILE = {4: (64, 1024), 5: (128, 512), 6: (256, 256), 7: (256, 256)}


def tile_rows_and_slots(Npad: int, variant: int, override=None):
    if override and variant in override:
        return override[variant]
    if Npad % 128:
        return (256, 256) if variant == 7 else (128, 768)
    return _TILE.get(variant, (128, 768))


def plan_splitk(wi: "WeightImage", M: int, kw: dict, *, min_ktiles: int, rows=None, tile=None, tune: bool = True, phases=None,
                ktiles=None):
    variant = kw.get("variant", 0)
    bm, target = tile if isinstance(tile, tuple) else tile_rows_and_slots(wi.Npad, variant, tile)
    pk = [len(t) * wi.KC for _, _, t in wi.phases] if ktiles is None else None
    S = splitk_for(M, wi.Npad, max(pk) if pk else ktiles, len(wi.phases) if phases is None else phases, phase_ktiles=pk, bm=bm,
# ... 133 lines not shown
```

understanding_flow_robustness_amd/patch_attack.py:

```python
from __future__ import annotations

import ctypes as C
import os
from argparse import Namespace

import numpy as np
import torch
from ._lib import engine_cache as _engine_cache

from . import _lib as L
from .flownets.utils_model import predict_flow

LOSS_THRESHOLD = 0.1
CLAMP_BOUND = 2.0


def _pixel_range(flownet: str):
    return (0.0, 1.0) if any(k in flownet for k in ("FlowNetC", "FlowNetS", "FlowNet2", "RAFT", "PWC")) else (-1.0, 1.0)


class ShardedExchange:

    def __init__(self, group=None):
        import torch.distributed as dist
        self.dist, self.group = dist, group
        self.world = dist.get_world_size(group) if dist.is_initialized() else 1
        self.rank = dist.get_rank(group) if dist.is_initialized() else 0

    def __call__(self, packed: torch.Tensor) -> torch.Tensor:
        if self.world > 1:
            self.dist.all_reduce(packed, op=self.dist.ReduceOp.SUM, group=self.group)
        return packed

    def gather(self, rows_local: torch.Tensor, rows_all: torch.Tensor) -> torch.Tensor:
        if self.world > 1:
            self.dist.all_gather_into_tensor(rows_all, rows_local, group=self.group)
        return rows_all


class PatchAttackStep:

    def __init__(self, flow_net, args, batch, height, width, device="cuda:0", shared_patch=True,
                 exchange: ShardedExchange | None = None, use_graph=True, warmup=3, use_cone=None, patch_hw=None,
                 sum_groups=1, skip_unread=True, corr_changed=True, tail_split=True, tail_resident=None):
        L.lib()
        self.net, self.args = flow_net, args
        self.skip_unread = bool(skip_unread)
        self.corr_changed = bool(corr_changed)
        self.tail_split, self.tail_resident = bool(tail_split), tail_resident
        self.B, self.H, self.W = batch, height, width
        self.dev = torch.device(device)
        self.shared = shared_patch
        self.exchange = exchange
        self.world = exchange.world if exchange is not None else 1
        if self.world > 1 and not shared_patch:
            raise ValueError("per-sample patches need no exchange; shard them as independent replicas")
        self.placed = patch_hw is not None
        if shared_patch and batch * self.world > 1 and not self.placed:
            raise ValueError("one patch behind several pairs is defined in patch coordinates: pass patch_hw=(ph, pw) "
                             "and load() a [1,3,ph,pw] patch / mask with per-pair origins (SURVEY.md 8e)")
        if self.placed and not shared_patch:
            raise ValueError("patch_hw: per-sample patches stay canvas-sized like the reference's")
        self.groups = int(sum_groups)
        if self.groups < 1 or batch % self.groups or (self.groups > 1 and not self.placed):
            raise ValueError("sum_groups must divide the pairs of a patch-coordinate step")
        self.lo, self.hi = _pixel_range(args.flownet)
        self.kind = 1 if getattr(args, "l2", False) else 0
        self.alpha = float(getattr(args, "alpha", 0.0))
        self.step = 0.5 * float(args.lr)
        self.CHW = 3 * height * width
        f32 = dict(dtype=torch.float32, device=self.dev)
        pb = 1 if shared_patch else batch
        self.tgt = torch.zeros(batch, 3, height, width, **f32)
        self.ref = torch.zeros_like(self.tgt)
        self._mask_canvas = None if self.placed else torch.zeros_like(self.tgt)
        self._mask_stale = self.placed
        if self.placed:
            ph, pw = (int(v) for v in patch_hw)
            if not (0 < ph <= height and 0 < pw <= width):
                raise ValueError("patch_hw does not fit the frame")
            self.ph, self.pw, self.n_p = ph, pw, 3 * ph * pw
            self.patch = torch.zeros(1, 3, ph, pw, **f32)
            self.mask_p = torch.zeros(1, 3, ph, pw, **f32)
            self.origins = torch.zeros(batch, 2, dtype=torch.int32, device=self.dev)
            self.origins_host = None
            self.rows_local = torch.zeros(self.groups, self.n_p + 1, **f32)
            self.rows_all = torch.zeros(self.world * self.groups, self.n_p + 1, **f32) if self.world > 1 else self.rows_local
            self.loss_local = torch.zeros(1, **f32)
            self.loss_cur = torch.zeros(1, **f32)
        else:
            self.patch = torch.zeros(pb, 3, height, width, **f32)
            self.loss_cur = torch.zeros(1, **f32)
            self.loss_local = self.loss_cur
        self.patch_init = torch.zeros_like(self.patch)
        self.target = torch.zeros(batch, 2, height, width, **f32)
        self.adv_tgt = torch.zeros_like(self.tgt).requires_grad_(True)
        self.adv_ref = torch.zeros_like(self.tgt).requires_grad_(True)
        self.g_flow = torch.zeros_like(self.target)
        self.loss_ws = torch.zeros(L.LOSS_PARTIALS, **f32)
        self._fused_loss = (batch * -(-(height // 4) // 16) * -(-(width // 4) // 16) <= L.LOSS_PARTIALS
                            and height % 4 == 0 and width % 4 == 0)
        self.g_flow2 = torch.zeros(batch, 2, height // 4, width // 4, **f32)
# ... 51 lines not shown
                                         self.CHW, self.step, CLAMP_BOUND, self.lo, self.hi,
                                         L.ptr(self.state), L.stream()), "patch update")

    def _crop(self, g_tgt, g_ref):
        L.check(L.lib().ufr_patch_grad_crop(L.ptr(g_tgt), L.ptr(g_ref), L.ptr(self.mask_p), L.ptr(self.origins), None,
                                            L.ptr(self.loss_local), L.ptr(self.rows_local), self.B, self.H, self.W,
                                            self.ph, self.pw, self.groups, L.stream()), "patch grad crop")

    def _apply(self):
        if self._rect_paste:
            return self._apply_rect()
        L.check(L.lib().ufr_patch_apply(L.ptr(self.rows_all), self.rows_all.shape[0], L.ptr(self.patch),
                                        L.ptr(self.loss_cur), self.ph, self.pw, self.step, CLAMP_BOUND,
                                        L.ptr(self.state), L.stream()), "patch apply")
        self._paste(do_clamp=True, gate=True)

    def _apply_rect(self):
        L.check(L.lib().ufr_patch_apply_paste_rect(
            L.ptr(self.rows_all), self.rows_all.shape[0], L.ptr(self.patch), L.ptr(self.loss_cur), L.ptr(self.tgt), L.ptr(self.ref),
            L.ptr(self.mask_p), L.ptr(self.origins), L.ptr(self.adv_tgt), L.ptr(self.adv_ref), self.B, self.H, self.W, self.ph,
            self.pw, self.step, CLAMP_BOUND, 1, self.lo, self.hi, L.ptr(self.state), L.stream()), "patch apply + rect paste")

    def _mask_extent(self):
        m = self.mask.amax(dim=1) != 0
        rows, cols = m.any(dim=2).cpu(), m.any(dim=1).cpu()
        ext = lambda v: max([int(r.nonzero().max() - r.nonzero().min()) + 1 if bool(r.any()) else 0 for r in v] + [1])
        eh, ew = ext(rows), ext(cols)
        if self.world > 1:
            both = torch.tensor([eh, ew], dtype=torch.float32, device=self.dev)
            self.exchange.dist.all_reduce(both, op=self.exchange.dist.ReduceOp.MAX, group=self.exchange.group)
            eh, ew = (int(v) for v in both.tolist())
        return eh, ew

    def _setup_cone(self):
        spec, B, H, W = self.cone, self.B, self.H, self.W
        eh, ew = self._mask_extent()
        wh, ww = spec.window_size(eh, H), spec.window_size(ew, W)
        self.graph = self.graph_b = self.graph_next = self.graph_b_next = None
        if self._warmup < 0:
            self._warmup = 1
        if wh * ww * 2 > H * W:
            self.cone = None
            return
        self.win_hw = (wh, ww)
        f32 = dict(dtype=torch.float32, device=self.dev)
        self.xw = torch.zeros(2 * B, 3, wh, ww, **f32).requires_grad_(True)
        self.eng = self.eng_kind = None
        if getattr(self.net, "engine_available", None) is not None and self.net.engine_available(H, W, self.dev):
            self.eng_kind = getattr(self.net, "ENGINE", "flownetc")
            if self.eng_kind == "pwc":
                from .pwc_engine import get_engine
            else:
                from .flownetc_engine import get_engine
            self.eng = get_engine(self.net, B, H, W, self.dev)
            self.eng.flow_out.requires_grad_(True)
            self._wp_hold = self.eng.window_prefix(wh, ww)
        self.taps = []
        with torch.no_grad(), L.shape_probe():
            feats = self.net.encode(torch.zeros(2, 3, spec.total_stride * 2, spec.total_stride * 2, **f32))
        for t, m, fr, f in zip(spec.taps, spec.tap_margins(), spec.frames, feats):
            ls = spec.level_stride(t)
            n = B * fr
            full = None if self.eng is not None else torch.zeros(n, f.shape[1], H // ls, W // ls, **f32).requires_grad_(True)
            gwin = torch.zeros(n, f.shape[1], wh // ls, ww // ls, **f32)
            self.taps.append((ls, m, n, full, gwin))
        if not self.placed:
            self.g_tgt_full = torch.zeros_like(self.tgt)
            self.g_ref_full = torch.zeros_like(self.tgt)
        self._chain = spec.to_c()
        self.band, reach = None, getattr(self.net, "BAND_REACH", None)
        if reach is not None and os.environ.get("UFR_BAND", "1") != "0":
            from .band_conv import Band, corr_band_width
            bw = -(-(ww + 2 * reach + 31) // 32) * 32
            if W % 32 != 0 or bw * 4 > W * 3:
                bw = 0
            self._band_reach = reach
            self.band = Band(torch.zeros(B, 8, dtype=torch.int32, device=self.dev), bw, cone_win=self.win,
                             cone_hw=(wh, ww))
            if bw and corr_band_width(ww) <= bw:
                self.band.corr_width = corr_band_width(ww)
            if self.tail_resident:
                self.band.tail_resident = int(self.tail_resident)
            if bw and os.environ.get("UFR_INCREMENTAL", "1") != "0":
                self.band.inc_layers = tuple(getattr(self.net, "INCREMENTAL_LAYERS", ()))

    def _win_copy(self, fn, src, dst, n, c, hf, wf, ls, margin):
        wh, ww = self.win_hw
        L.check(fn(L.ptr(src), L.ptr(dst), L.ptr(self.win), self.B, n, c, hf, wf, wh // ls, ww // ls, ls, margin,
                   L.stream()), "window copy")

    def _cone_refresh(self, prefix_features=None):
        lib = L.lib()
        wh, ww = self.win_hw
        L.check(lib.ufr_cone_window(L.ptr(self.mask), self.B, self.CHW, 3, self.H, self.W, C.byref(self._chain),
                                    wh, ww, L.ptr(self.win), L.ptr(self.state[3:]), L.stream()), "cone window")
        if not self.placed:
            self.g_tgt_full.zero_(); self.g_ref_full.zero_()
        if self.band is not None and self.band.width:
            start = torch.div(self.win[:, 1] - self._band_reach, 32, rounding_mode="floor") * 32
            self.band.win[:, 1] = start.clamp(0, self.W - self.band.width)
            if self.band.corr_width:
                from .band_conv import corr_band_origin
                self.band.win[:, 2] = corr_band_origin(self.win[:, 1], self.band.corr_width, self.W)
        self._cone_prefix(prefix_features)

    def _cone_prefix(self, prefix_features=None):
        if self.eng is not None:
# ... 432 lines not shown
```

Baseline: 1560.

## Store stride-2 conv prefix activations in a parity-split plane layout

Adds a parity-split layout in which each image's pixels are grouped by (y&1, x&1) into four quarter planes. conv1 can write its output in this layout, and the following stride-2 implicit-GEMM launches can read or write it, so every tap of a stride-2 conv reads a contiguous quarter plane instead of striding across full rows. It is enabled by default for the FlowNetC engine prefix. This adds kernel template variants and new validation paths, and restricts parity buffers to a single stride-2, band-free, non-balanced launch.

```diff
diff --git a/include/ufr_hip.h b/include/ufr_hip.h
--- a/include/ufr_hip.h
+++ b/include/ufr_hip.h
@@ -353,6 +353,17 @@
 int ufr_igemm_tail_plan(const ufr_igemm_desc* d, int resident_workgroups, ufr_igemm_tail_plan_t* plan);
 int ufr_igemm_balanced(const ufr_igemm_desc* d, int resident_workgroups, float* ws, long ws_floats, ufr_stream_t stream);
 typedef struct {
+  int in_hp, in_wp; long in_pixels;
+  int out_hp, out_wp; long out_pixels;
+  int ntaps;
+  int q[UFR_IGEMM_MAX_TAPS], dy[UFR_IGEMM_MAX_TAPS], dx[UFR_IGEMM_MAX_TAPS];
+  int rows[UFR_IGEMM_MAX_TAPS], cols[UFR_IGEMM_MAX_TAPS];
+} ufr_igemm_parity_plan_t;
+int ufr_igemm_parity(const ufr_igemm_desc* d, int in_parity, int out_parity, ufr_stream_t stream);
+int ufr_igemm_parity_plan(const ufr_igemm_desc* d, int in_parity, int out_parity, ufr_igemm_parity_plan_t* plan);
+int ufr_igemm_parity_tap(const ufr_igemm_parity_plan_t* plan, int tap, int b, int y, int x, long* pixel);
+long ufr_parity_pixel(int H, int W, int b, int y, int x);
+typedef struct {
   const void* x; long x_plane_stride; int in_chunk0, C;
   const void* gy; long gy_plane_stride; int g_chunk0, N;
   int B, Hi, Wi, Ho, Wo, kh, kw, sy, sx, py, px;
@@ -389,6 +400,9 @@
 int ufr_conv1_direct(const float* frames_a, const float* frames_b, int Ba, int Bb, int H, int W, const double* mean,
                      const void* wimg, const float* bias, float slope, void* out_planes, long plane_stride, int out_chunk0,
                      ufr_stream_t stream);
+int ufr_conv1_direct_parity(const float* frames_a, const float* frames_b, int Ba, int Bb, int H, int W, const double* mean,
+                            const void* wimg, const float* bias, float slope, void* out_planes, long plane_stride, int out_chunk0,
+                            int out_parity, ufr_stream_t stream);
 int ufr_conv1_pack_planes(const float* frames_a, const float* frames_b, void* planes, long plane_stride, int Ba, int Bb, int H,
                           int W, const double* mean, ufr_stream_t stream);
 int ufr_conv1_unpack_grad(const float* G, float* grad_frames, int N, int H, int W, ufr_stream_t stream);
diff --git a/understanding_flow_robustness_amd/_lib.py b/understanding_flow_robustness_amd/_lib.py
--- a/understanding_flow_robustness_amd/_lib.py
+++ b/understanding_flow_robustness_amd/_lib.py
@@ -74,6 +74,13 @@
     _fields_ = [("on", C.c_int), ("row_tiles", C.c_int), ("col_tiles", C.c_int), ("full_row_tiles", C.c_int), ("tail_row_tiles", C.c_int),
                 ("tail_row0", C.c_int), ("tail_rows", C.c_int), ("slices", C.c_int), ("slice_ktiles", C.c_int), ("ktiles", C.c_int),
                 ("workgroups", C.c_int), ("ws_floats", C.c_long), ("steps_before", C.c_int), ("steps_after", C.c_int)]
+
+
+class IgemmParityPlan(C.Structure):
+    _fields_ = [("in_hp", C.c_int), ("in_wp", C.c_int), ("in_pixels", C.c_long),
+                ("out_hp", C.c_int), ("out_wp", C.c_int), ("out_pixels", C.c_long), ("ntaps", C.c_int),
+                ("q", C.c_int * UFR_IGEMM_MAX_TAPS), ("dy", C.c_int * UFR_IGEMM_MAX_TAPS), ("dx", C.c_int * UFR_IGEMM_MAX_TAPS),
+                ("rows", C.c_int * UFR_IGEMM_MAX_TAPS), ("cols", C.c_int * UFR_IGEMM_MAX_TAPS)]
 
 
 UFR_IGEMM_WGRAD_MAX_TAPS = 49
@@ -209,6 +216,9 @@
     "ufr_igemm": [C.POINTER(IgemmDesc), _vp],
     "ufr_igemm_tail_plan": [C.POINTER(IgemmDesc), _i, C.POINTER(IgemmTailPlan)],
     "ufr_igemm_balanced": [C.POINTER(IgemmDesc), _i, _vp, _l, _vp],
+    "ufr_igemm_parity": [C.POINTER(IgemmDesc), _i, _i, _vp],
+    "ufr_igemm_parity_plan": [C.POINTER(IgemmDesc), _i, _i, C.POINTER(IgemmParityPlan)],
+    "ufr_igemm_parity_tap": [C.POINTER(IgemmParityPlan), _i, _i, _i, _i, C.POINTER(C.c_long)],
     "ufr_igemm_wgrad": [C.POINTER(IgemmWgradDesc), _vp],
     "ufr_igemm_wgrad_dilated": [C.POINTER(IgemmWgradDesc), _i, _i, _vp],
     "ufr_flow_upscale4_forward": [_vp, _vp, _i, _i, _i, _i, _f, _i, _vp],
@@ -280,6 +290,7 @@
     "ufr_altcorr_planes_prepare": [_vp, _vp, _l, _l, _i, _vp],
     "ufr_altcorr_planes_forward": [_vp, _l, C.POINTER(AltCorrPlaneLevels), _vp, _vp, _i, _i, _i, _i, _i, _f, _vp],
     "ufr_conv1_direct": [_vp, _vp, _i, _i, _i, _i, _vp, _vp, _vp, _f, _vp, _l, _i, _vp],
+    "ufr_conv1_direct_parity": [_vp, _vp, _i, _i, _i, _i, _vp, _vp, _vp, _f, _vp, _l, _i, _i, _vp],
     "ufr_train_loss": [C.POINTER(TrainLossDesc), _vp],
     "ufr_raft_sequence_loss": [C.POINTER(RaftSequenceLossDesc), _vp],
     "ufr_grad_norm": [C.POINTER(AdamwSeg), _i, _f, _vp, _l, _vp, _vp],
@@ -312,6 +323,7 @@
 PLAIN = {"ufr_abi_version": (C.c_int, []), "ufr_last_error": (C.c_char_p, []),
          "ufr_device_count": (C.c_int, []), "ufr_build_manifest": (C.c_char_p, []),
          "ufr_igemm_variant_fallbacks": (C.c_int, []),
+         "ufr_parity_pixel": (C.c_long, [_i, _i, _i, _i, _i]),
          "ufr_conv3x3_c2_workspace_floats": (C.c_long, [_i, _i, _i, _i]),
          "ufr_cm_norm_workspace_doubles": (C.c_long, [_l, _i, _i]),
          "ufr_resample2d_backward_workspace_bytes": (C.c_long, [_i, _i, _i]),
diff --git a/understanding_flow_robustness_amd/csrc/conv1_direct.hip b/understanding_flow_robustness_amd/csrc/conv1_direct.hip
--- a/understanding_flow_robustness_amd/csrc/conv1_direct.hip
+++ b/understanding_flow_robustness_amd/csrc/conv1_direct.hip
@@ -1,5 +1,6 @@
 #include <atomic>
 
+#include "parity_layout.h"
 #include "ufr_common.h"
 
 namespace {
@@ -27,14 +28,15 @@
   int tiles_x, tiles_y, tiles;
 };
 
-template <bool BUF_>
+template <bool BUF_, bool PAR_ = false>
 __global__ __launch_bounds__(512) __attribute__((amdgpu_waves_per_eu(2, 2))) void conv1_direct_kernel(const Conv1Args a) {
   extern __shared__ __attribute__((aligned(16))) unsigned char lds[];
   const int tid = threadIdx.x, lane = tid & 63, wave = __builtin_amdgcn_readfirstlane(tid >> 6);
   const int q = wave & 3, half = wave >> 2;
   const int li = lane & 15, g = lane >> 4;
   const int Hh = a.H >> 1, Wh = a.W >> 1;
-  const long M = (long)a.N * Hh * Wh;
+  const int Hp = ufr::parity::half_up(Hh), Wp = ufr::parity::half_up(Wh);
+  const long M = PAR_ ? 4L * a.N * Hp * Wp : (long)a.N * Hh * Wh;
 
   for (int i = tid; i < 2 * BUF_B / 16; i += 512) reinterpret_cast<uint4*>(lds)[i] = make_uint4(0, 0, 0, 0);
   bf16x8 wf[7][3];
@@ -153,7 +155,7 @@
       }
       const int yy = half * 4 + (pt >> 1);
       const int y = Y0 + yy, x = X0 + (even ? 0 : 16) + li;
-      const long m = ((long)n * Hh + y) * Wh + x;
+      const long m = PAR_ ? ufr::parity::pixel(Hp, Wp, n, y, x) : ((long)n * Hh + y) * Wh + x;
       const long e = ((long)(a.out_chunk0 + (q >> 1)) * M + m) * 32 + (q & 1) * 16 + (g & 2) * 4;
       const bool live = y < Hh && x < Wh;
       if constexpr (BUF_) {
@@ -207,11 +209,14 @@
 
 }
 
-extern "C" int ufr_conv1_direct(const float* frames_a, const float* frames_b, int Ba, int Bb, int H, int W, const double* mean,
-                                const void* wimg, const float* bias, float slope, void* out_planes, long plane_stride,
-                                int out_chunk0, ufr_stream_t stream) {
+extern "C" int ufr_conv1_direct_parity(const float* frames_a, const float* frames_b, int Ba, int Bb, int H, int W, const double* mean,
+                                       const void* wimg, const float* bias, float slope, void* out_planes, long plane_stride,
+                                       int out_chunk0, int out_parity, ufr_stream_t stream) {
   UFR_REQUIRE(frames_a && mean && wimg && bias && out_planes && (frames_b || Bb == 0), "conv1 direct: null pointer");
   UFR_REQUIRE(Ba > 0 && Bb >= 0 && H > 0 && W > 0 && !(H & 1) && !(W & 1) && plane_stride > 0 && out_chunk0 >= 0, "conv1 direct: bad shape");
+  UFR_REQUIRE(out_parity == 0 || out_parity == 1, "conv1 direct: the output layout is 0 (plain) or 1 (parity-split)");
+  UFR_REQUIRE(!out_parity || (out_chunk0 + 2) * 4L * (Ba + Bb) * ufr::parity::half_up(H >> 1) * ufr::parity::half_up(W >> 1) * 32 <= plane_stride,
+              "conv1 direct: the output chunks leave the split buffer");
   Conv1Args a;
   a.fa = frames_a; a.fb = frames_b; a.Ba = Ba; a.N = Ba + Bb; a.H = H; a.W = W; a.mean = mean;
   a.wimg = static_cast<const __bf16*>(wimg); a.bias = bias; a.slope = slope;
@@ -226,11 +231,23 @@
   if (!raised[dev].load(std::memory_order_acquire)) {
     hipError_t e = ufr::ensure_dynamic_lds(reinterpret_cast<const void*>(conv1_direct_kernel<true>), 2 * BUF_B);
     if (e == hipSuccess) e = ufr::ensure_dynamic_lds(reinterpret_cast<const void*>(conv1_direct_kernel<false>), 2 * BUF_B);
+    if (e == hipSuccess) e = ufr::ensure_dynamic_lds(reinterpret_cast<const void*>(conv1_direct_kernel<true, true>), 2 * BUF_B);
+    if (e == hipSuccess) e = ufr::ensure_dynamic_lds(reinterpret_cast<const void*>(conv1_direct_kernel<false, true>), 2 * BUF_B);
     if (e != hipSuccess) return ufr::fail(UFR_ELAUNCH, "conv1 direct: %s", hipGetErrorString(e));
     raised[dev].store(true, std::memory_order_release);
   }
   const int grid = (int)(tiles < ufr::kNumCU ? tiles : ufr::kNumCU);
-  if (6L * plane_stride < 0x7fffffffL) conv1_direct_kernel<true><<<grid, 512, 2 * BUF_B, ufr::as_stream(stream)>>>(a);
+  const bool buf = 6L * plane_stride < 0x7fffffffL;
+  if (out_parity) {
+    if (buf) conv1_direct_kernel<true, true><<<grid, 512, 2 * BUF_B, ufr::as_stream(stream)>>>(a);
+    else conv1_direct_kernel<false, true><<<grid, 512, 2 * BUF_B, ufr::as_stream(stream)>>>(a);
+  } else if (buf) conv1_direct_kernel<true><<<grid, 512, 2 * BUF_B, ufr::as_stream(stream)>>>(a);
   else conv1_direct_kernel<false><<<grid, 512, 2 * BUF_B, ufr::as_stream(stream)>>>(a);
   return ufr::launched("conv1_direct_kernel");
 }
+
+extern "C" int ufr_conv1_direct(const float* frames_a, const float* frames_b, int Ba, int Bb, int H, int W, const double* mean,
+                                const void* wimg, const float* bias, float slope, void* out_planes, long plane_stride,
+                                int out_chunk0, ufr_stream_t stream) {
+  return ufr_conv1_direct_parity(frames_a, frames_b, Ba, Bb, H, W, mean, wimg, bias, slope, out_planes, plane_stride, out_chunk0, 0, stream);
+}
diff --git a/understanding_flow_robustness_amd/csrc/igemm.hip b/understanding_flow_robustness_amd/csrc/igemm.hip
--- a/understanding_flow_robustness_amd/csrc/igemm.hip
+++ b/understanding_flow_robustness_amd/csrc/igemm.hip
@@ -1,6 +1,7 @@
 #include <atomic>
 #include <cstdlib>
 
+#include "parity_layout.h"
 #include "ufr_common.h"
 
 namespace {
@@ -184,7 +185,22 @@
   int skip_out;
   int tl_S, tl_full, tl_nt, tl_rt0, tl_row0, tl_rows, tl_per_k;
   Phase ph[4];
+  struct Par {
+    long in_img;
+    int in_par, in_pitch, out_par, oHp, oWp;
+    int off[UFR_IGEMM_MAX_TAPS], lim[UFR_IGEMM_MAX_TAPS];
+  } par;
 };
+template <bool PAR_>
+__device__ __forceinline__ long out_pixel_of(const Args& a, int pm, int oy0, int ox0) {
+  if constexpr (PAR_) {
+    if (a.par.out_par) {
+      const GridCell c = grid_cell(a.g, pm);
+      return ufr::parity::pixel(a.par.oHp, a.par.oWp, c.b, c.yr * a.g.out_sy + oy0, (c.xr + band_x0(a.g, c.b)) * a.g.out_sx + ox0);
+    }
+  }
+  return out_pixel(a.g, pm, oy0, ox0);
+}
 
 __device__ __forceinline__ int xcd_before(int m, int x) { return (m >> 3) * x + min(m & 7, x); }
 __device__ __forceinline__ bool tail_tile(const Args& a, int& bx, int& by, int& bz) {
@@ -254,7 +270,7 @@
   }
 }
 
-template <int NPL, int MT, int WGR, int BNT>
+template <int NPL, int MT, int WGR, int BNT, bool PAR_ = false>
 __device__ __forceinline__ void igemm_write_out(const Args& a, const Phase& ph, f32x4 (&acc)[MT][4], float* lds_f32, int* flag, int z, int phase,
                                                 int tile_id, int bm0, int bm, int bn0, int bn, int wrow, int wcol, int lane, int wave,
                                                 bool tail_slice = false) {
@@ -305,7 +321,7 @@
       if (row >= a.g.M || n0 >= a.e.Nchunks32 * 32) continue;
       float v[8];
       sum_slabs(base + (long)row * a.Npad + n0, sstride, S, v);
-      epilogue_store8(a.e, out_pixel(a.g, row, ph.oy0, ph.ox0), n0, v);
+      epilogue_store8(a.e, out_pixel_of<PAR_>(a, row, ph.oy0, ph.ox0), n0, v);
     }
     return;
   }
@@ -330,7 +346,7 @@
         if (row < a.g.M) {
           const float4 lo = *reinterpret_cast<const float4*>(tw + r * TS + g8 * 8), hi = *reinterpret_cast<const float4*>(tw + r * TS + g8 * 8 + 4);
           float v[8] = {lo.x, lo.y, lo.z, lo.w, hi.x, hi.y, hi.z, hi.w};
-          epilogue_store8(a.e, out_pixel(a.g, row, ph.oy0, ph.ox0), bn + wcol + g8 * 8, v);
+          epilogue_store8(a.e, out_pixel_of<PAR_>(a, row, ph.oy0, ph.ox0), bn + wcol + g8 * 8, v);
         }
       }
     }
@@ -369,6 +385,7 @@
   int yb, xb, xlo, xhi;
   long ibase;
 };
+template <bool PAR_ = false>
 __device__ __forceinline__ Cell cell_geometry(const Args& a, long cell, int xr_override) {
   const bool live = cell >= 0 && cell < a.g.M;
   const GridCell c = grid_cell(a.g, live ? (int)cell : 0);
@@ -376,7 +393,7 @@
   Cell o;
   o.yb = live ? c.yr * a.in_sy : -(1 << 20);
   o.xb = xg * a.in_sx;
-  o.ibase = (long)c.b * a.Hi * a.Wi;
+  o.ibase = PAR_ ? (long)c.b * a.par.in_img : (long)c.b * a.Hi * a.Wi;
   o.xlo = a.in_x0 ? a.in_x0[c.b * a.in_x0_stride] / a.in_x0_div : 0;
   o.xhi = a.in_x0 ? min(a.Wi, o.xlo + a.in_xw) : a.Wi;
   o.xlo = max(o.xlo, 0);
@@ -388,7 +405,7 @@
   return (unsigned)yi < (unsigned)a.Hi && xi >= c.xlo && xi < c.xhi;
 }
 
-template <int APT, int NPL, int IMG_ROWS, bool BUF_>
+template <int APT, int NPL, int IMG_ROWS, bool BUF_, bool PAR_ = false>
 struct ActStager {
   Cell cell[APT];
   bool ok[APT];
@@ -400,10 +417,10 @@
   int tap, kc;
 
   __device__ __forceinline__ void init(const Args& a, const Phase& ph, int bm, int srow0, int csw, int kt0) {
-    cstride = (long)a.g.B * a.Hi * a.Wi * 32;
+    cstride = PAR_ ? (long)a.g.B * a.par.in_img * 32 : (long)a.g.B * a.Hi * a.Wi * 32;
 #pragma unroll
     for (int i = 0; i < APT; ++i) {
-      cell[i] = cell_geometry(a, bm + srow0 + 64 * i, -1);
+      cell[i] = cell_geometry<PAR_>(a, bm + srow0 + 64 * i, -1);
       rowbase[i] = (unsigned)(cell[i].ibase * 64 + csw * 16);
     }
     gx = a.x + (long)a.in_chunk0 * cstride + csw * 8;
@@ -415,10 +432,23 @@
   }
   __device__ __forceinline__ void set_tap(const Args& a, const Phase& ph, int t) {
     const int dyx = ph.dyx[t], dyo = (int)(short)(dyx & 0xffff), dxo = dyx >> 16;
+    bool par = false;
+    int poff = 0, plim = 0;
+    if constexpr (PAR_) {
+      par = a.par.in_par;
+      poff = par ? a.par.off[t] : 0;
+      plim = par ? a.par.lim[t] : 0;
+    }
 #pragma unroll
     for (int i = 0; i < APT; ++i) {
       int pix;
-      ok[i] = tap_pixel(a, cell[i], dyo, dxo, pix);
+      if (PAR_ && par) {
+        const int yi = cell[i].yb + dyo, xi = cell[i].xb + dxo;
+        pix = poff + yi * a.par.in_pitch + xi;
+        ok[i] = (unsigned)yi < (unsigned)(plim & 0xffff) && (unsigned)xi < (unsigned)(plim >> 16);
+      } else {
+        ok[i] = tap_pixel(a, cell[i], dyo, dxo, pix);
+      }
       if (BUF_) voff[i] = ok[i] ? rowbase[i] + (unsigned)pix * 64u : 0x80000000u;
       else aoff[i] = ok[i] ? (cell[i].ibase + (long)pix) * 32 : 0;
     }
@@ -487,7 +517,7 @@
         acc[m][n] = __builtin_amdgcn_mfma_f32_16x16x32_bf16(fa[PROD_A[t]][m], fb[n][PROD_B[t]], acc[m][n], 0, 0, 0);
 }
 
-template <int BM_, int BN_, bool PIPE_ = false, bool BUF_ = false, int NP_ = 6>
+template <int BM_, int BN_, bool PIPE_ = false, bool BUF_ = false, int NP_ = 6, bool PAR_ = false>
 __global__ __launch_bounds__(256) __attribute__((amdgpu_waves_per_eu(PIPE_ ? 2 : (BM_ == 64 ? 4 : 3), PIPE_ ? 2 : (BM_ == 64 ? 4 : 3)))) void igemm_glds_kernel(const Args a) {
   static_assert(!(PIPE_ && BUF_), "the buffer-resource form exists for the single-stage kernel");
   static_assert(NP_ == 6 || NP_ == 3 || NP_ == 1, "six, three or one product");
@@ -509,7 +539,7 @@
 
   const int srow0 = tid >> 2, sch = tid & 3;
   const int csw = sch ^ ((srow0 >> 1) & 3);
-  ActStager<APT, NPL, BM_, BUF_> act;
+  ActStager<APT, NPL, BM_, BUF_, PAR_> act;
   act.init(a, ph, bm, srow0, csw, kt0);
   const __bf16* wp = a.w + ph.w_off + ((long)kt0 * a.Npad + bn + srow0) * BK + csw * 8;
   const long wstep = (long)a.Npad * BK;
@@ -578,7 +608,7 @@
     }
   }
   static_assert(PIPE_ ? 4 * 32 * 68 * 4 <= STAGE * 2 : true, "epilogue staging does not fit");
-  igemm_write_out<NPL, MT, BM_, BN_>(a, ph, acc, reinterpret_cast<float*>(lds_all), reinterpret_cast<int*>(lds_all), wk.z, wk.phase,
+  igemm_write_out<NPL, MT, BM_, BN_, PAR_>(a, ph, acc, reinterpret_cast<float*>(lds_all), reinterpret_cast<int*>(lds_all), wk.z, wk.phase,
                                      wk.tile_id(), bm, bm, bn, bn, wrow, wcol, lane, wave);
 }
 constexpr int PIPE_LDS_BYTES = (3 * (128 + 128) * BK + 3 * 128 * BK) * 2;
@@ -586,7 +616,7 @@
 constexpr int PP_IMG = 3 * 128 * BK;
 constexpr int pp_lds_bytes(int bn) { return (4 * PP_IMG + 2 * 3 * bn * BK) * 2; }
 
-template <int BN_, bool BUF_ = false, int NP_ = 6>
+template <int BN_, bool BUF_ = false, int NP_ = 6, bool PAR_ = false>
 __global__ __launch_bounds__(512) __attribute__((amdgpu_waves_per_eu(2, 2))) void igemm_pp_kernel(const Args a) {
   static_assert(NP_ == 6 || NP_ == 3 || NP_ == 1, "six, three or one product");
   constexpr int NPL = NP_ == 6 ? 3 : (NP_ == 3 ? 2 : 1), FIRST = 6 - NP_;
@@ -606,7 +636,7 @@
 
   const int srow0 = tid >> 2, sch = tid & 3;
   const int csw = sch ^ ((srow0 >> 1) & 3);
-  ActStager<2, NPL, 128, BUF_> act;
+  ActStager<2, NPL, 128, BUF_, PAR_> act;
   act.init(a, ph, bm, srow0, csw, wk.kt0);
   const __bf16* wp = a.w + ph.w_off + ((long)wk.kt0 * a.Npad + bn + srow0) * BK + csw * 8;
   const long wstep = (long)a.Npad * BK;
@@ -658,8 +688,8 @@
   if (grp == 0) __builtin_amdgcn_s_barrier();
   const unsigned long long probe_c3 = probe ? __builtin_amdgcn_s_memtime() : 0;
   static_assert(4 * 32 * 68 * 4 <= 2 * PP_IMG * 2, "epilogue staging does not fit a group's activation images");
-  igemm_write_out<NPL, MT, 256, BN_>(a, ph, acc, reinterpret_cast<float*>(lds_pp + imgA0), reinterpret_cast<int*>(lds_pp), wk.z, wk.phase,
-                                     wk.tile_id(), wk.ty * 256, bm, bn, bn, wrow, wcol, lane, wave, wk.tail_slice);
+  igemm_write_out<NPL, MT, 256, BN_, PAR_>(a, ph, acc, reinterpret_cast<float*>(lds_pp + imgA0), reinterpret_cast<int*>(lds_pp), wk.z, wk.phase,
+                                           wk.tile_id(), wk.ty * 256, bm, bn, bn, wrow, wcol, lane, wave, wk.tail_slice);
   if (probe && threadIdx.x == 0) {
     const int wg = (blockIdx.z * gridDim.y + blockIdx.y) * gridDim.x + blockIdx.x;
     if (wg < ufr_clock_probe_cap) {
@@ -892,6 +922,7 @@
   return stage > epi ? stage : epi;
 }
 
+template <bool PAR_ = false>
 __global__ __launch_bounds__(256) void igemm_reduce_kernel(const Args a) {
   const int n8 = a.Npad / 8;
   const int rows = a.tl_S ? a.tl_rows : a.g.M, row0 = a.tl_S ? a.tl_row0 : 0;
@@ -903,7 +934,7 @@
     if (n0 >= a.e.Nchunks32 * 32) continue;
     float v[8];
     sum_slabs(a.ws + ((long)a.zoff[phase] * rows + r) * a.Npad + n0, (long)rows * a.Npad, a.tl_S ? a.tl_S : a.sk[phase], v);
-    epilogue_store8(a.e, out_pixel(a.g, row, a.ph[phase].oy0, a.ph[phase].ox0), n0, v);
+    epilogue_store8(a.e, out_pixel_of<PAR_>(a, row, a.ph[phase].oy0, a.ph[phase].ox0), n0, v);
   }
 }
 
@@ -924,12 +955,24 @@
 
 namespace {
 template <int BM_, int BN_, int NP_>
-void launch_glds(const Args& a, dim3 grid, bool use_buf, hipStream_t st) {
+void launch_glds(const Args& a, dim3 grid, bool use_buf, hipStream_t st, bool par) {
+  if constexpr (NP_ == 6) {
+    if (par) {
+      igemm_glds_kernel<BM_, BN_, false, true, 6, true><<<grid, 256, 0, st>>>(a);
+      return;
+    }
+  }
   if (use_buf) igemm_glds_kernel<BM_, BN_, false, true, NP_><<<grid, 256, 0, st>>>(a);
   else if constexpr (NP_ == 6) igemm_glds_kernel<BM_, BN_><<<grid, 256, 0, st>>>(a);
 }
 template <int NP_>
-void launch_pp(const Args& a, dim3 grid, bool use_buf, hipStream_t st) {
+void launch_pp(const Args& a, dim3 grid, bool use_buf, hipStream_t st, bool par) {
+  if constexpr (NP_ == 6) {
+    if (par) {
+      igemm_pp_kernel<128, true, 6, true><<<grid, 512, pp_lds_bytes(128), st>>>(a);
+      return;
+    }
+  }
   if (use_buf) igemm_pp_kernel<128, true, NP_><<<grid, 512, pp_lds_bytes(128), st>>>(a);
   else if constexpr (NP_ == 6) igemm_pp_kernel<128><<<grid, 512, pp_lds_bytes(128), st>>>(a);
 }
@@ -937,6 +980,7 @@
 template <int NP_>
 int launch_tiles(const Args& a, const ufr_igemm_desc* d, const ufr_igemm_tail_plan_t* tp, int variant, int nz, bool use_buf, hipStream_t st) {
   const long M = a.g.M;
+  const bool par = a.par.in_par || a.par.out_par;
   const int bn = d->Npad % BN == 0 ? BN : 64;
   const dim3 grid(d->Npad / bn, (unsigned)((M + BM - 1) / BM), nz);
   if constexpr (NP_ != 6) UFR_REQUIRE(use_buf, "igemm: the reduced-product forms need activation planes below 2 GB");
@@ -945,24 +989,62 @@
     if (bn == BN) igemm_pp3_kernel<128><<<gpp, 512, pp3_lds_bytes(128), st>>>(a);
     else igemm_pp3_kernel<64><<<gpp, 512, pp3_lds_bytes(64), st>>>(a);
   } else if (variant == 4 && bn == BN) {
-    launch_glds<64, 128, NP_>(a, dim3(d->Npad / BN, (unsigned)((M + 63) / 64), nz), use_buf, st);
+    launch_glds<64, 128, NP_>(a, dim3(d->Npad / BN, (unsigned)((M + 63) / 64), nz), use_buf, st, par);
   } else if ((variant == 6 || variant == 7 || (NP_ != 6 && variant == 5)) && bn == BN) {
     if constexpr (NP_ != 6) {
       const hipError_t e = ufr::ensure_dynamic_lds(reinterpret_cast<const void*>(igemm_pp_kernel<128, true, NP_>), pp_lds_bytes(128));
       if (e != hipSuccess) return ufr::fail(UFR_ELAUNCH, "igemm: %s", hipGetErrorString(e));
     }
-    launch_pp<NP_>(a, tp ? dim3(tp->workgroups) : dim3(d->Npad / BN, (unsigned)((M + 255) / 256), nz), use_buf, st);
+    launch_pp<NP_>(a, tp ? dim3(tp->workgroups) : dim3(d->Npad / BN, (unsigned)((M + 255) / 256), nz), use_buf, st, par);
   } else if (NP_ == 6 && variant == 5 && bn == BN) {
     igemm_glds_kernel<128, 128, true><<<grid, 256, PIPE_LDS_BYTES, st>>>(a);
   } else if (bn == BN) {
-    launch_glds<128, 128, NP_>(a, grid, use_buf, st);
+    launch_glds<128, 128, NP_>(a, grid, use_buf, st, par);
   } else {
-    launch_glds<128, 64, NP_>(a, grid, use_buf, st);
+    launch_glds<128, 64, NP_>(a, grid, use_buf, st, par);
   }
   return UFR_OK;
 }
 
-int igemm_run(const ufr_igemm_desc* d, const ufr_igemm_tail_plan_t* tp, float* tws, ufr_stream_t stream) {
+int parity_plan(const ufr_igemm_desc* d, int in_parity, int out_parity, ufr_igemm_parity_plan_t* plan) {
+  UFR_REQUIRE(d && plan, "igemm parity: null argument");
+  UFR_REQUIRE((in_parity == 0 || in_parity == 1) && (out_parity == 0 || out_parity == 1), "igemm parity: the flags are 0 or 1");
+  UFR_REQUIRE(d->B > 0 && d->Hi > 0 && d->Wi > 0 && d->Ho > 0 && d->Wo > 0 && d->Hi < 32768 && d->Wi < 32768 && d->Ho < 32768 && d->Wo < 32768,
+              "igemm parity: bad grid");
+  UFR_REQUIRE(d->nphase >= 1 && d->nphase <= 4 && d->phase[0].ntaps >= 1 && d->phase[0].ntaps <= UFR_IGEMM_MAX_TAPS, "igemm parity: bad phase");
+  *plan = ufr_igemm_parity_plan_t{};
+  if (in_parity) {
+    UFR_REQUIRE(d->nphase == 1 && d->in_sy == 2 && d->in_sx == 2, "igemm parity: a parity-split input is read by one phase at stride 2");
+    UFR_REQUIRE(!d->in_x0, "igemm parity: a parity-split input takes no input band (in_x0)");
+    UFR_REQUIRE(!d->row_x0, "igemm parity: a parity-split input takes no row band (row_x0)");
+    plan->in_hp = ufr::parity::half_up(d->Hi);
+    plan->in_wp = ufr::parity::half_up(d->Wi);
+    plan->in_pixels = 4L * d->B * plan->in_hp * plan->in_wp;
+    plan->ntaps = d->phase[0].ntaps;
+    for (int t = 0; t < plan->ntaps; ++t) {
+      const ufr::parity::Split sy = ufr::parity::split(d->phase[0].dy[t]), sx = ufr::parity::split(d->phase[0].dx[t]);
+      plan->q[t] = sy.par * 2 + sx.par;
+      plan->dy[t] = sy.step;
+      plan->dx[t] = sx.step;
+      plan->rows[t] = ufr::parity::extent(d->Hi, sy.par);
+      plan->cols[t] = ufr::parity::extent(d->Wi, sx.par);
+    }
+  }
+  if (out_parity) {
+    UFR_REQUIRE(d->out_planes, "igemm parity: a parity-split output is a planes output (out_planes)");
+    UFR_REQUIRE(!d->out_f32, "igemm parity: a parity-split output takes no fp32 output (out_f32)");
+    UFR_REQUIRE(!d->out_rowmajor, "igemm parity: a parity-split output takes no row-major output (out_rowmajor)");
+    UFR_REQUIRE(!d->tail, "igemm parity: a parity-split output takes no tail columns (tail)");
+    UFR_REQUIRE(!d->add && !d->mask, "igemm parity: a parity-split output takes no addend or mask (they are read in the plain pixel order)");
+    plan->out_hp = ufr::parity::half_up(d->Ho);
+    plan->out_wp = ufr::parity::half_up(d->Wo);
+    plan->out_pixels = 4L * d->B * plan->out_hp * plan->out_wp;
+  }
+  UFR_REQUIRE(plan->in_pixels < (1L << 30) && plan->out_pixels < (1L << 30), "igemm parity: too many pixels");
+  return UFR_OK;
+}
+
+int igemm_run(const ufr_igemm_desc* d, const ufr_igemm_tail_plan_t* tp, float* tws, ufr_stream_t stream, int in_par = 0, int out_par = 0) {
   UFR_REQUIRE(d, "igemm: null descriptor");
   UFR_REQUIRE(d->x && d->w, "igemm: null operand");
   UFR_REQUIRE(d->B > 0 && d->Hi > 0 && d->Wi > 0 && d->Hr > 0 && d->Wr > 0 && d->Ho > 0 && d->Wo > 0, "igemm: bad grid");
@@ -985,9 +1067,24 @@
               "igemm: too many pixels");
   UFR_REQUIRE((d->Hr - 1) * d->out_sy + 1 <= d->Ho && (d->row_x0 || (d->Wr - 1) * d->out_sx + 1 <= d->Wo),
               "igemm: the row grid does not fit the output grid");
+  ufr_igemm_parity_plan_t pp{};
+  if (in_par || out_par) {
+    const int prc = parity_plan(d, in_par, out_par, &pp);
+    if (prc != UFR_OK) return prc;
+    UFR_REQUIRE(!in_par || (long)(d->in_chunk0 + d->KC) * pp.in_pixels * 32 <= d->x_plane_stride, "igemm parity: the input chunks leave the split buffer");
+    UFR_REQUIRE(!out_par || (long)(d->out_chunk0 + (d->N + 31) / 32) * pp.out_pixels * 32 <= d->out_plane_stride,
+                "igemm parity: the output chunks leave the split buffer");
+  }
   Args a;
   a.x = static_cast<const __bf16*>(d->x); a.x_plane_stride = d->x_plane_stride; a.in_chunk0 = d->in_chunk0; a.KC = d->KC;
-  a.Hi = d->Hi; a.Wi = d->Wi; a.in_sy = d->in_sy; a.in_sx = d->in_sx;
+  a.Hi = d->Hi; a.Wi = d->Wi; a.in_sy = in_par ? 1 : d->in_sy; a.in_sx = in_par ? 1 : d->in_sx;
+  a.par.in_par = in_par; a.par.in_pitch = in_par ? pp.in_wp : d->Wi;
+  a.par.in_img = in_par ? 4L * pp.in_hp * pp.in_wp : (long)d->Hi * d->Wi;
+  a.par.out_par = out_par; a.par.oHp = pp.out_hp; a.par.oWp = pp.out_wp;
+  for (int t = 0; t < UFR_IGEMM_MAX_TAPS; ++t) {
+    a.par.off[t] = in_par && t < pp.ntaps ? pp.q[t] * pp.in_hp * pp.in_wp : 0;
+    a.par.lim[t] = in_par && t < pp.ntaps ? (pp.rows[t] | (pp.cols[t] << 16)) : 0;
+  }
   a.in_x0 = d->in_x0; a.in_x0_stride = d->in_x0_stride; a.in_x0_div = d->in_x0_div; a.in_xw = d->in_xw;
   a.w = static_cast<const __bf16*>(d->w); a.w_plane_stride = d->w_plane_stride; a.Npad = d->Npad;
   a.g.B = d->B; a.g.Hr = d->Hr; a.g.Wr = d->Wr; a.g.M = (int)M;
@@ -1001,7 +1098,7 @@
   a.e.out_rm = d->out_rowmajor; a.e.out_ld = d->out_ld;
   a.e.planes_chunks = d->planes_chunks > 0 ? d->planes_chunks : (1 << 30); a.e.f32_first_chunk = d->f32_first_chunk;
   a.e.tail = d->tail; a.e.tail_n0 = d->tail_n0; a.e.tail_acc = d->tail_accumulate;
-  a.e.Mout = (long)d->B * d->Ho * d->Wo; a.e.N = d->N; a.e.Nchunks32 = (d->N + 31) / 32;
+  a.e.Mout = out_par ? pp.out_pixels : (long)d->B * d->Ho * d->Wo; a.e.N = d->N; a.e.Nchunks32 = (d->N + 31) / 32;
   a.nphase = d->nphase; a.splitk = d->splitk; a.ws = d->ws;
   a.tickets = (d->splitk > 1 && !d->no_reduce) ? d->tickets : nullptr;
   static const int skip_out = [] { const char* e = getenv("UFR_IGEMM_DEBUG_SKIP_EPILOGUE"); return e ? atoi(e) : 0; }();
@@ -1022,7 +1119,8 @@
     UFR_REQUIRE(p.w_off + (long)p.ntaps * d->KC * d->Npad * BK <= d->w_plane_stride, "igemm: phase %d weights out of range", z);
     a.ph[z].ntaps = p.ntaps; a.ph[z].oy0 = p.oy0; a.ph[z].ox0 = p.ox0; a.ph[z].w_off = p.w_off;
     for (int t = 0; t < UFR_IGEMM_MAX_TAPS; ++t)
-      a.ph[z].dyx[t] = t < p.ntaps ? (int)(((unsigned)(int)p.dy[t] & 0xffffu) | ((unsigned)(int)p.dx[t] << 16)) : 0;
+      a.ph[z].dyx[t] = t >= p.ntaps ? 0 : in_par ? (int)(((unsigned)pp.dy[t] & 0xffffu) | ((unsigned)pp.dx[t] << 16))
+                                                 : (int)(((unsigned)(int)p.dy[t] & 0xffffu) | ((unsigned)(int)p.dx[t] << 16));
     for (int t = 0; t < UFR_IGEMM_MAX_TAPS; ++t) a.ph[z].run[t] = 1 << 4;
     for (int t = 0; t < p.ntaps;) {
       int len = 1, dir = 0;
@@ -1047,16 +1145,19 @@
     nz += a.sk[z];
   }
   hipStream_t st = ufr::as_stream(stream);
-  const int variant = d->variant ? d->variant : 2;
+  const bool par = in_par || out_par;
+  const int variant = par && (d->variant == 5 || d->variant == 7) ? 6 : (par && d->variant == 8 ? 2 : (d->variant ? d->variant : 2));
   UFR_REQUIRE(variant == 2 || variant == 4 || variant == 5 || variant == 6 || variant == 7 || variant == 8, "igemm: unknown kernel variant %d",
               d->variant);
   const bool use_buf = 6L * d->x_plane_stride < 0x7fffffffL;
+  UFR_REQUIRE(!par || (use_buf && d->products == 6), "igemm parity: six products and activation planes below 2 GB only");
   int dev = 0;
   if (hipGetDevice(&dev) != hipSuccess || dev < 0 || dev >= 64) return ufr::fail(UFR_ELAUNCH, "igemm: no current device");
   static std::atomic<bool> raised[64] = {};
   if (!raised[dev].load(std::memory_order_acquire)) {
     hipError_t e = ufr::ensure_dynamic_lds(reinterpret_cast<const void*>(igemm_pp_kernel<128>), pp_lds_bytes(128));
     if (e == hipSuccess) e = ufr::ensure_dynamic_lds(reinterpret_cast<const void*>(igemm_pp_kernel<128, true>), pp_lds_bytes(128));
+    if (e == hipSuccess) e = ufr::ensure_dynamic_lds(reinterpret_cast<const void*>(igemm_pp_kernel<128, true, 6, true>), pp_lds_bytes(128));
     if (e == hipSuccess) e = ufr::ensure_dynamic_lds(reinterpret_cast<const void*>(igemm_glds_kernel<128, 128, true>), PIPE_LDS_BYTES);
     if (e == hipSuccess) e = ufr::ensure_dynamic_lds(reinterpret_cast<const void*>(igemm_pp3_kernel<128>), pp3_lds_bytes(128));
     if (e == hipSuccess) e = ufr::ensure_dynamic_lds(reinterpret_cast<const void*>(igemm_pp3_kernel<64>), pp3_lds_bytes(64));
@@ -1068,6 +1169,7 @@
              !d->out_rowmajor && d->k_order && d->N <= 64 && d->products == 6;
   for (int t = 0; d33 && t < 9; ++t)
     d33 = d->phase[0].dy[t] >= -1 && d->phase[0].dy[t] <= 1 && d->phase[0].dx[t] >= -1 && d->phase[0].dx[t] <= 1;
+  if (par && (d->variant == 7 || d->variant == 8)) g_variant_fallbacks.fetch_add(1);
   if ((variant == 8 && !d33) || (variant == 7 && !(d->k_order && (d->in_sx == 1 || d->in_sx == 2) && d->Wr >= 22 && d->products == 6)))
     g_variant_fallbacks.fetch_add(1);
   if (d33) {
@@ -1087,12 +1189,33 @@
   if (rc == UFR_OK) rc = ufr::launched("igemm_kernel");
   if (rc != UFR_OK || (!tp && (d->splitk == 1 || d->no_reduce || a.tickets))) return rc;
   const long total = tp ? (long)tp->tail_rows * (d->Npad / 8) : (long)d->nphase * M * (d->Npad / 8);
-  igemm_reduce_kernel<<<ufr::stream_grid(total, 256), 256, 0, st>>>(a);
+  if (par) igemm_reduce_kernel<true><<<ufr::stream_grid(total, 256), 256, 0, st>>>(a);
+  else igemm_reduce_kernel<<<ufr::stream_grid(total, 256), 256, 0, st>>>(a);
   return ufr::launched("igemm_reduce_kernel");
 }
 }
 
 extern "C" int ufr_igemm(const ufr_igemm_desc* d, ufr_stream_t stream) { return igemm_run(d, nullptr, nullptr, stream); }
+
+extern "C" int ufr_igemm_parity(const ufr_igemm_desc* d, int in_parity, int out_parity, ufr_stream_t stream) {
+  UFR_REQUIRE(d, "igemm: null descriptor");
+  UFR_REQUIRE((in_parity == 0 || in_parity == 1) && (out_parity == 0 || out_parity == 1), "igemm parity: the flags are 0 or 1");
+  return igemm_run(d, nullptr, nullptr, stream, in_parity, out_parity);
+}
+extern "C" int ufr_igemm_parity_plan(const ufr_igemm_desc* d, int in_parity, int out_parity, ufr_igemm_parity_plan_t* plan) {
+  return parity_plan(d, in_parity, out_parity, plan);
+}
+extern "C" long ufr_parity_pixel(int H, int W, int b, int y, int x) {
+  if (H <= 0 || W <= 0 || b < 0 || y < 0 || y >= H || x < 0 || x >= W) return -1;
+  return ufr::parity::pixel(ufr::parity::half_up(H), ufr::parity::half_up(W), b, y, x);
+}
+extern "C" int ufr_igemm_parity_tap(const ufr_igemm_parity_plan_t* plan, int tap, int b, int y, int x, long* pixel) {
+  UFR_REQUIRE(plan && pixel && tap >= 0 && tap < plan->ntaps && b >= 0 && y >= 0 && x >= 0, "igemm parity tap: bad argument");
+  const int yi = y + plan->dy[tap], xi = x + plan->dx[tap];
+  const bool ok = (unsigned)yi < (unsigned)plan->rows[tap] && (unsigned)xi < (unsigned)plan->cols[tap];
+  *pixel = ok ? (long)b * 4 * plan->in_hp * plan->in_wp + (long)plan->q[tap] * plan->in_hp * plan->in_wp + (long)yi * plan->in_wp + xi : -1;
+  return ok ? 1 : 0;
+}
 
 extern "C" int ufr_igemm_tail_plan(const ufr_igemm_desc* d, int resident_workgroups, ufr_igemm_tail_plan_t* plan) {
   UFR_REQUIRE(d && plan, "igemm tail plan: null argument");
diff --git a/understanding_flow_robustness_amd/csrc/parity_layout.h b/understanding_flow_robustness_amd/csrc/parity_layout.h
--- /dev/null
+++ b/understanding_flow_robustness_amd/csrc/parity_layout.h
@@ -0,0 +1,30 @@
+#ifndef UFR_PARITY_LAYOUT_H_
+#define UFR_PARITY_LAYOUT_H_
+
+#if defined(__HIPCC__) || defined(__CUDACC__)
+#define UFR_PARITY_HD __host__ __device__ inline __attribute__((always_inline))
+#else
+#define UFR_PARITY_HD inline
+#endif
+
+namespace ufr {
+namespace parity {
+
+UFR_PARITY_HD int half_up(int n) { return (n + 1) >> 1; }
+
+UFR_PARITY_HD long pixel(int Hp, int Wp, int b, int y, int x) {
+  return (((long)b * 4 + (y & 1) * 2 + (x & 1)) * Hp + (y >> 1)) * Wp + (x >> 1);
+}
+
+struct Split { int par, step; };
+UFR_PARITY_HD Split split(int d) {
+  const int par = d & 1;
+  return {par, (d - par) / 2};
+}
+
+UFR_PARITY_HD int extent(int n, int par) { return (n - par + 1) >> 1; }
+
+}
+}
+
+#endif
diff --git a/understanding_flow_robustness_amd/flownetc_engine.py b/understanding_flow_robustness_amd/flownetc_engine.py
--- a/understanding_flow_robustness_amd/flownetc_engine.py
+++ b/understanding_flow_robustness_amd/flownetc_engine.py
@@ -52,7 +52,8 @@
 
 
 class FlowNetCHeadEngine:
-    def __init__(self, net, B: int, H: int, W: int, device):
+    def __init__(self, net, B: int, H: int, W: int, device, prefix_parity: bool = True):
+        self.prefix_parity = bool(prefix_parity)
         if H % 64 or W % 64:
             raise ValueError("FlowNetC head engine: frame sides must be multiples of 64")
         L.lib()
@@ -205,10 +206,11 @@
         layers = self._stem_layers()
         wis = [None] + [ig.conv_forward_weights(conv.weight, conv.stride[0], conv.padding[0]) for _, conv, _ in layers[1:]]
         scratch = {}
+        split = self.prefix_parity and len(layers) == 3 and all(conv.stride[0] == 2 and conv.kernel_size[0] % 2 for _, conv, _ in layers[1:])
 
         def level_buffer(lvl, slot, chunks):
             if (lvl, slot) not in scratch:
-                scratch[(lvl, slot)] = ig.Planes(B, H >> lvl, W >> lvl, chunks, dev)
+                scratch[(lvl, slot)] = ig.Planes(B, H >> lvl, W >> lvl, chunks, dev, parity=split)
             return scratch[(lvl, slot)]
         halves = {}
         for h, taps in (("a", {2: self.cat2, 3: self.c3a_p}), ("b", {3: self.c3b_p})):
@@ -219,8 +221,12 @@
             chain = []
             for i in range(1, len(layers)):
                 name, conv, lvl = layers[i]
-                launch = ig.make_launch(wis[i], outs[i - 1], 0, (H >> lvl, W >> lvl), (H >> lvl, W >> lvl), out_planes=outs[i],
-                                        out_chunk0=0, bias=self._bias(conv), variant=self._variant_for(wis[i]))
+                rows = (H >> lvl, W >> lvl)
+                kw = dict(out_planes=outs[i], out_chunk0=0, bias=self._bias(conv), variant=self._variant_for(wis[i]))
+                if outs[i - 1].parity or outs[i].parity:
+                    kw["variant"] = ig.tuned(wis[i], B * rows[0] * rows[1], ig.parity_signature_kw(outs[i - 1], kw), kw["variant"], 1,
+                                             rows=rows)[0]
+                launch = ig.make_launch(wis[i], outs[i - 1], 0, rows, rows, **kw)
                 chain.append((name, launch, wis[i]))
             conv1 = layers[0][1]
             P = dict(c1=outs[0], layers=chain, b1=self._bias(conv1), w1=conv1.weight.detach())
@@ -249,9 +255,10 @@
         D = P.get("direct")
         if D is not None:
             c1 = D["c1"]
-            L.check(L.lib().ufr_conv1_direct(L.ptr(a), L.ptr(b.contiguous()) if b is not None else None, int(a.shape[0]), nb,
-                                             int(a.shape[2]), int(a.shape[3]), L.ptr(mean), L.ptr(D["wimg"]), L.ptr(D["bias"]),
-                                             float(ig.LEAKY), L.ptr(c1.t), c1.plane_stride, 0, L.stream()), "conv1 direct")
+            L.check(L.lib().ufr_conv1_direct_parity(L.ptr(a), L.ptr(b.contiguous()) if b is not None else None, int(a.shape[0]), nb,
+                                                    int(a.shape[2]), int(a.shape[3]), L.ptr(mean), L.ptr(D["wimg"]), L.ptr(D["bias"]),
+                                                    float(ig.LEAKY), L.ptr(c1.t), c1.plane_stride, 0, int(c1.parity), L.stream()),
+                    "conv1 direct")
             return
         pk = P["packed"]
         L.check(L.lib().ufr_conv1_pack_planes(L.ptr(a), L.ptr(b.contiguous()) if b is not None else None, L.ptr(pk.t),
@@ -868,13 +875,13 @@
     return tuple((p.data_ptr(), p._version) for p in net.parameters())
 
 
-def get_engine(net, B: int, H: int, W: int, device) -> FlowNetCHeadEngine:
-    key = (int(B), int(H), int(W), str(torch.device(device)))
+def get_engine(net, B: int, H: int, W: int, device, prefix_parity: bool = True) -> FlowNetCHeadEngine:
+    key = (int(B), int(H), int(W), str(torch.device(device))) + (() if prefix_parity else ("plain prefix",))
     cache = _engine_cache(net, "_ufr_head_engines")
     stamp = _weights_stamp(net)
     eng = cache.get(key)
     if eng is None or eng.weights_stamp != stamp:
-        eng = cache[key] = FlowNetCHeadEngine(net, B, H, W, device)
+        eng = cache[key] = FlowNetCHeadEngine(net, B, H, W, device, prefix_parity=prefix_parity)
         eng.weights_stamp = stamp
     return eng
 
diff --git a/understanding_flow_robustness_amd/igemm.py b/understanding_flow_robustness_amd/igemm.py
--- a/understanding_flow_robustness_amd/igemm.py
+++ b/understanding_flow_robustness_amd/igemm.py
@@ -27,13 +27,26 @@
 
 class Planes:
 
-    def __init__(self, B, H, W, chunks, device):
+    def __init__(self, B, H, W, chunks, device, parity: bool = False):
         self.B, self.H, self.W, self.chunks = int(B), int(H), int(W), int(chunks)
-        self.M = self.B * self.H * self.W
+        self.parity = bool(parity)
+        self.Hp, self.Wp = (self.H + 1) // 2, (self.W + 1) // 2
+        self.M = 4 * self.B * self.Hp * self.Wp if self.parity else self.B * self.H * self.W
         self.t = torch.zeros(3, self.chunks, self.M, 32, dtype=torch.bfloat16, device=device)
         self.plane_stride = self.chunks * self.M * 32
 
+    def parity_index(self) -> torch.Tensor:
+        b = torch.arange(self.B).view(-1, 1, 1)
+        y = torch.arange(self.H).view(1, -1, 1)
+        x = torch.arange(self.W).view(1, 1, -1)
+        return ((b * 4 + (y & 1) * 2 + (x & 1)) * self.Hp + (y >> 1)) * self.Wp + (x >> 1)
+
+    def _plain_only(self, what: str):
+        if self.parity:
+            raise RuntimeError(f"Planes.{what}: a parity-split buffer is read by its one stride-2 launch only")
+
     def load_nchw(self, x: torch.Tensor, chunk0: int = 0, scale: float = 1.0, slope: float = 1.0, bias: torch.Tensor | None = None):
+        self._plain_only("load_nchw")
         L.require_hip(x, "x")
         B, Cn, H, W = x.shape
         if (B, H, W) != (self.B, self.H, self.W) or chunk0 + pad32(Cn) // 32 > self.chunks or x.dtype != torch.float32:
@@ -44,6 +57,7 @@
         return self
 
     def load_rowmajor(self, src: torch.Tensor, chunk0: int = 0, scale: float = 1.0):
+        self._plain_only("load_rowmajor")
         L.require_hip(src, "src", contiguous=False)
         if src.dim() != 2 or (src.stride(1) != 1 and src.shape[1] != 1) or src.dtype != torch.float32 or src.shape[0] != self.M or chunk0 + pad32(src.shape[1]) // 32 > self.chunks:
             raise RuntimeError("Planes.load_rowmajor: shape mismatch")
@@ -52,6 +66,7 @@
         return self
 
     def to_nchw(self, Cn: int, chunk0: int = 0, out: torch.Tensor | None = None) -> torch.Tensor:
+        self._plain_only("to_nchw")
         if out is None:
             out = torch.empty(self.B, Cn, self.H, self.W, dtype=torch.float32, device=self.t.device)
         L.check(L.lib().ufr_chunks_to_nchw(L.ptr(self.t), self.plane_stride, None, int(chunk0), None, 0, L.ptr(out), self.B, Cn,
@@ -252,14 +267,18 @@
 
 class Launch:
 
-    def __init__(self, desc, keep, tail_plan=None, resident=0, tail_ws=None):
+    def __init__(self, desc, keep, tail_plan=None, resident=0, tail_ws=None, in_parity=False, out_parity=False):
         self.desc, self._keep = desc, keep
+        self.in_parity, self.out_parity = bool(in_parity), bool(out_parity)
         self.tail_plan, self._resident, self._tail_ws = tail_plan, int(resident), tail_ws
 
     def __call__(self):
         if self.tail_plan is not None:
             L.check(L.lib().ufr_igemm_balanced(C.byref(self.desc), self._resident, L.ptr(self._tail_ws), self._tail_ws.numel(), L.stream()),
                     "igemm (balanced)")
+            return
+        if self.in_parity or self.out_parity:
+            L.check(L.lib().ufr_igemm_parity(C.byref(self.desc), int(self.in_parity), int(self.out_parity), L.stream()), "igemm (parity)")
             return
         L.check(L.lib().ufr_igemm(C.byref(self.desc), L.stream()), "igemm")
 
@@ -313,6 +332,7 @@
     out = ("slabs" if kw.get("no_reduce") else "rowmajor" if kw.get("out_rowmajor") is not None else
            ("planes" if kw.get("out_planes") is not None else "") + ("f32" if kw.get("out_f32") is not None else ""))
     out += ("+add" if kw.get("add") is not None else "") + ("+mask" if kw.get("mask") is not None else "") + ("+tail" if kw.get("tail") is not None else "")
+    out += ("+pin" if kw.get("in_parity") else "") + ("+pout" if kw.get("out_parity") else "")
     taps = "-".join(str(len(t)) for _, _, t in wi.phases)
     grid = f"_g{int(rows[0])}x{int(rows[1])}" if rows is not None else ""
     return f"M{M}_N{wi.Npad}_KC{wi.KC}_t{taps}_s{wi.geometry['in_s']}{wi.geometry['out_s']}_{out}{grid}"
@@ -330,6 +350,11 @@
             if raw.get("_arch", "gfx950") == "gfx950":
                 _TUNING = {k: tuple(v) for k, v in raw.items() if not k.startswith("_")}
     return _TUNING
+
+
+def parity_signature_kw(x: "Planes", kw: dict) -> dict:
+    out = kw.get("out_planes")
+    return dict(kw, in_parity=bool(x.parity), out_parity=bool(out is not None and out.parity))
 
 
 def variant_fallbacks() -> int:
@@ -384,7 +409,15 @@
         ph.ntaps, ph.oy0, ph.ox0, ph.w_off = len(taps), oy0, ox0, off
         for t, (dy, dx) in enumerate(taps):
             ph.dy[t], ph.dx[t] = dy, dx
-    Mout = x.B * d.Ho * d.Wo
+    in_par, out_par = bool(x.parity), bool(out_planes is not None and out_planes.parity)
+    if in_par and (int(wi.geometry["in_s"]) != 2 or len(wi.phases) != 1 or in_band is not None or row_band is not None):
+        raise RuntimeError("igemm: a parity-split input is read by a stride-2 forward launch without bands")
+    if out_par and (out_f32 is not None or out_rowmajor is not None or tail is not None or add is not None or mask is not None or
+                    (out_planes.H, out_planes.W) != (d.Ho, d.Wo)):
+        raise RuntimeError("igemm: a parity-split output is a planes output of the launch's output grid, without addend or mask")
+    if (in_par or out_par) and balance:
+        raise RuntimeError("igemm: a parity-split launch has no balanced form")
+    Mout = out_planes.M if out_par else x.B * d.Ho * d.Wo
     nch = pad32(wi.N) // 32
     if tail is not None:
         if tail_n0 % 32 or not 0 < tail_n0 < wi.N or tail.M != Mout or tail_chunk0 + (wi.N - tail_n0 + 31) // 32 > tail.chunks:
@@ -443,7 +476,7 @@
             tws = ws if (ws is not None and ws.dtype == torch.float32 and ws.numel() >= plan.ws_floats) else \
                 torch.empty(plan.ws_floats, dtype=torch.float32, device=x.t.device)
             return Launch(d, keep + [tws], tail_plan=plan, resident=R, tail_ws=tws)
-    return Launch(d, keep)
+    return Launch(d, keep, in_parity=in_par, out_parity=out_par)
 
 
 def resident_workgroups(device) -> int:
diff --git a/understanding_flow_robustness_amd/patch_attack.py b/understanding_flow_robustness_amd/patch_attack.py
--- a/understanding_flow_robustness_amd/patch_attack.py
+++ b/understanding_flow_robustness_amd/patch_attack.py
@@ -42,12 +42,13 @@
 
     def __init__(self, flow_net, args, batch, height, width, device="cuda:0", shared_patch=True,
                  exchange: ShardedExchange | None = None, use_graph=True, warmup=3, use_cone=None, patch_hw=None,
-                 sum_groups=1, skip_unread=True, corr_changed=True, tail_split=True, tail_resident=None):
+                 sum_groups=1, skip_unread=True, corr_changed=True, tail_split=True, tail_resident=None, prefix_parity=True):
         L.lib()
         self.net, self.args = flow_net, args
         self.skip_unread = bool(skip_unread)
         self.corr_changed = bool(corr_changed)
         self.tail_split, self.tail_resident = bool(tail_split), tail_resident
+        self.prefix_parity = bool(prefix_parity)
         self.B, self.H, self.W = batch, height, width
         self.dev = torch.device(device)
         self.shared = shared_patch
@@ -205,7 +206,8 @@
                 from .pwc_engine import get_engine
             else:
                 from .flownetc_engine import get_engine
-            self.eng = get_engine(self.net, B, H, W, self.dev)
+            self.eng = get_engine(self.net, B, H, W, self.dev) if self.eng_kind == "pwc" else \
+                get_engine(self.net, B, H, W, self.dev, prefix_parity=self.prefix_parity)
             self.eng.flow_out.requires_grad_(True)
             self._wp_hold = self.eng.window_prefix(wh, ww)
         self.taps = []
```

Measured after the change: 1566 (median of 6 runs). No clear change (+0.4%).
